# hpgmg/hpgmg

Measured on AMD Instinct MI355X. Metric: DOF/s (fine-grid) for FMG F-cycle, higher is better.
Workload: dtype f64

## Files before the change

### hpgmg_amd/csrc/host/operators_hip.c

```c
#include "plugin_internal.h"

void hp_do_restriction(level_type *Lc, int id_c, level_type *Lf, int id_f, int type) {
  TICK(Lf, restriction_total, "restriction");
  communicator_type *S = &Lf->restriction[type], *R = &Lc->restriction[type];
  backend_t *Bc = hp_backend_of(Lc), *Bf = hp_backend_of(Lf);
  HIP_OK(hpgmg_hip_restrict_blocks(&Bc->dev, id_c, &Bf->dev, id_f, hp_mirror(Lf, S->blocks[0], S->num_blocks[0]), S->num_blocks[0], type));
  hp_transport_phase(R, S, (Lf->tag << 4) | 0x5);
  HIP_OK(hpgmg_hip_restrict_blocks(&Bc->dev, id_c, &Bf->dev, id_f, hp_mirror(Lf, S->blocks[1], S->num_blocks[1]), S->num_blocks[1], type));
  HIP_OK(hpgmg_hip_copy_blocks(&Bc->dev, id_c, hp_mirror(Lc, R->blocks[2], R->num_blocks[2]), R->num_blocks[2]));
  TOCK();
}

int hpgmg_restrict_zero_fused(level_type *Lc, int id_c, level_type *Lf, int id_f, int zero_id) {
  communicator_type *S = &Lf->restriction[RESTRICT_CELL], *R = &Lc->restriction[RESTRICT_CELL];
  if (!Lf->active || !Lc->active || Lc->num_my_boxes < 1 || zero_id == id_c) return 0;
  if (S->num_sends || R->num_recvs || S->num_blocks[0] || R->num_blocks[2] || S->num_blocks[1] < 1) return 0;
  TICK(Lf, restriction_total, "restriction + zero_vector");
  backend_t *Bc = hp_backend_of(Lc), *Bf = hp_backend_of(Lf);
  HIP_OK(hpgmg_hip_restrict_cell_and_zero(&Bc->dev, id_c, &Bf->dev, id_f, hp_mirror(Lf, S->blocks[1], S->num_blocks[1]), S->num_blocks[1], zero_id));
  TOCK();
  return 1;
}

static const int *restrict_map_of(level_type *Lf, backend_t *Bf);
const int *hp_restrict_map_of(level_type *Lf, backend_t *Bf) { return restrict_map_of(Lf, Bf); }
static const int *restrict_map_of(level_type *Lf, backend_t *Bf) {
  communicator_type *S = &Lf->restriction[RESTRICT_CELL];
  if (!Bf->d_restrict_map) {
    int *map = (int *)malloc((size_t)Lf->num_my_boxes * 4 * sizeof(int)), n, b;
    for (b = 0; b < 4 * Lf->num_my_boxes; b++) map[b] = -1;
    for (n = 0; n < S->num_blocks[1]; n++) {
      const blockCopy_type *e = &S->blocks[1][n];
      if (e->read.box < 0 || e->write.box < 0 || map[4 * e->read.box] >= 0) continue;
      map[4 * e->read.box] = e->write.box;
      map[4 * e->read.box + 1] = e->write.i - e->read.i / 2; map[4 * e->read.box + 2] = e->write.j - e->read.j / 2; map[4 * e->read.box + 3] = e->write.k - e->read.k / 2;
    }
    for (b = 0; b < Lf->num_my_boxes; b++) if (map[4 * b] < 0) { free(map); return NULL; }
    Bf->d_restrict_map = (int *)hpgmg_hip_malloc((size_t)Lf->num_my_boxes * 4 * sizeof(int));
    if (!Bf->d_restrict_map) { fprintf(stderr, "hpgmg: device allocation failed: %s\n", hpgmg_hip_last_error()); abort(); }
    HIP_OK(hpgmg_hip_memcpy_h2d(Bf->d_restrict_map, map, (size_t)Lf->num_my_boxes * 4 * sizeof(int)));
    free(map);
  }
  return Bf->d_restrict_map;
}
static long long fused_residuals_remote = 0;
long long hpgmg_fused_residuals_remote(void) { return fused_residuals_remote; }
static int fused_residual_on(void) {
  return (int)hp_switch(SW_FUSED_RESIDUAL);
}
#define FUSED_LAUNCH(READY, CALL) do {                                                                          \
    if ((READY) == 2) {                                                                                          \
      hpgmg_hip_set_tile_part(1); HIP_OK(CALL); hp_overlap_end(); hpgmg_hip_set_tile_part(2); HIP_OK(CALL); hpgmg_hip_set_tile_part(0); \
    } else HIP_OK(CALL); } while (0)
static int fused_residual_operand_form(level_type *L, backend_t *B, int x_id, int restrict_form);
static int fused_residual_operand(level_type *L, backend_t *B, int x_id) { return fused_residual_operand_form(L, B, x_id, 0); }
static int fused_residual_operand_form(level_type *L, backend_t *B, int x_id, int restrict_form) {
// ... 72 lines not shown
  const int many = (T && T->size > 1);
  if (!fused_residual_on() || !hp_switch(SW_DEFER_NORM) || !L->active || !Lc->active || F_id == R_id) return 0;
  if (many) {
    const int nb = L->boxes_in.i * L->boxes_in.j * L->boxes_in.k;
    int q;
    if (Lc->boxes_in.i != L->boxes_in.i || Lc->boxes_in.j != L->boxes_in.j || Lc->boxes_in.k != L->boxes_in.k) return 0;
    for (q = 0; q < nb; q++) if (L->rank_of_box[q] != Lc->rank_of_box[q]) return 0;
  }
  int local_ok = (L->num_my_boxes >= 1 && Lc->num_my_boxes >= 1 && !S->num_sends && !R->num_recvs && !S->num_blocks[0] && !R->num_blocks[2] && S->num_blocks[1] >= 1);
  backend_t *Bc = Lc->num_my_boxes >= 1 ? hp_backend_of(Lc) : NULL, *B = L->num_my_boxes >= 1 ? hp_backend_of(L) : NULL;
  if (local_ok && ((L->box_dim & 1) || !(B->dev.flags & 1) || (L->box_jStride & 1) || (L->box_kStride & 1) || (L->box_volume & 1) || L->box_dim < 16 || !restrict_map_of(L, B))) local_ok = 0;
  if (!local_ok && !many) return 0;
  if (local_ok) {
    TICK(L, blas1, "norm(F) + R = F + restriction (fused, norm deferred)");
    HIP_OK(hpgmg_hip_norm_copy_restrict_deferred(&B->dev, F_id, R_id, &Bc->dev, R_id, B->d_restrict_map));
    TOCK();
    deferred_on_device = 1;
  } else {
    double v = 0.0;
    if (B) { TICK(L, blas1, "norm(F), this rank's part (reduction deferred)"); HIP_OK(hpgmg_hip_norm_max(&B->dev, F_id, &v)); TOCK(); }
    hp_do_scale_vector(L, R_id, 1.0, F_id);
    hp_do_restriction(Lc, R_id, L, R_id, RESTRICT_CELL);
    deferred_host_value = v; deferred_on_device = 0;
  }
  deferred_norm_level = L;
  return 1;
}
double hpgmg_norm_deferred_fetch(level_type *L) {
  double v = deferred_host_value;
  if (deferred_norm_level != L) { fprintf(stderr, "hpgmg: no deferred norm is pending on this level\n"); abort(); }
  deferred_norm_level = NULL;
  if (deferred_on_device) HIP_OK(hpgmg_hip_deferred_fetch(&v));
  return hp_allreduce_scalar(L, v, HPGMG_REDUCE_MAX);
}
int hpgmg_residual_norm_fused(level_type *L, int res_id, int x_id, int rhs_id, double a, double b, double *norm_out) {
  hpgmg_config cfg;
  hpgmg_get_config(&cfg);
  if (cfg.op != HPGMG_OP_7PT && res_id >= 0) return 0;
  if (!L->active || L->num_my_boxes < 1) return 0;
  backend_t *B = hp_backend_of(L);
  const int ready = fused_residual_operand(L, B, x_id);
  if (!ready) return 0;
  double v = 0.0;
  { TICK(L, residual, "residual + norm (fused)");
    FUSED_LAUNCH(ready, hpgmg_hip_residual_norm(hp_stencil_dev(B), hp_variant(), res_id, x_id, rhs_id, a, b, 1.0 / (L->h * L->h), &v));
    TOCK(); }
  *norm_out = hp_allreduce_scalar(L, v, HPGMG_REDUCE_MAX);
  return 1;
}


static void interpolation_lists(level_type *Lf, int id_f, double prescale, level_type *Lc, int id_c, int order, int tagbits) {
  TICK(Lf, interpolation_total, "interpolation");
  communicator_type *S = &Lc->interpolation, *R = &Lf->interpolation;
  backend_t *Bc = hp_backend_of(Lc), *Bf = hp_backend_of(Lf);
  HIP_OK(hpgmg_hip_interpolate_blocks(&Bf->dev, id_f, 0.0, &Bc->dev, id_c, hp_mirror(Lc, S->blocks[0], S->num_blocks[0]), S->num_blocks[0], order));
  hp_transport_phase(R, S, (Lf->tag << 4) | tagbits);
  HIP_OK(hpgmg_hip_interpolate_blocks(&Bf->dev, id_f, prescale, &Bc->dev, id_c, hp_mirror(Lc, S->blocks[1], S->num_blocks[1]), S->num_blocks[1], order));
  HIP_OK(hpgmg_hip_increment_blocks(&Bf->dev, id_f, prescale, hp_mirror(Lf, R->blocks[2], R->num_blocks[2]), R->num_blocks[2]));
  TOCK();
}
void hp_do_interpolation_vcycle(level_type *Lf, int id_f, double prescale, level_type *Lc, int id_c) {
  hpgmg_config c; hpgmg_get_config(&c);
  if (c.op == HPGMG_OP_27PT) {
    if (!hp_exchange_and_bcs_one_launch(Lc, id_c, STENCIL_SHAPE_BOX, 12, 1)) { exchange_boundary(Lc, id_c, STENCIL_SHAPE_BOX); apply_BCs_p2(Lc, id_c, STENCIL_SHAPE_BOX); }
    interpolation_lists(Lf, id_f, prescale, Lc, id_c, 2, 0x7);
    return;
  }
  if (c.op == HPGMG_OP_FV2 || c.op == HPGMG_OP_FV4) {
    if (!hp_exchange_and_bcs_one_launch(Lc, id_c, STENCIL_SHAPE_BOX, 2, 1)) { exchange_boundary(Lc, id_c, STENCIL_SHAPE_BOX); apply_BCs_v2(Lc, id_c, STENCIL_SHAPE_BOX); }
    interpolation_lists(Lf, id_f, prescale, Lc, id_c, 3, 0x7);
    return;
  }
  if (c.op != HPGMG_OP_7PT) hp_no_kernel("interpolation_vcycle for this operator");
  interpolation_lists(Lf, id_f, prescale, Lc, id_c, 0, 0x6);
}
static int interp_all_local(level_type *Lf, level_type *Lc) {
  communicator_type *S = &Lc->interpolation, *R = &Lf->interpolation;
  int n;
  if (Lc->num_my_boxes < 1 || S->num_sends || R->num_recvs || S->num_blocks[0] || R->num_blocks[2] || S->num_blocks[1] < 1) return 0;
  for (n = 0; n < S->num_blocks[1]; n++) if (S->blocks[1][n].read.box < 0 || S->blocks[1][n].write.box < 0) return 0;
  return 1;
}
static long long zero_interp_fused = 0;
long long hpgmg_zero_interp_fused(void) { return zero_interp_fused; }
int hpgmg_zero_interpolation_fcycle_fused(level_type *Lf, int id_f, level_type *Lc, int id_c) {
  hpgmg_config c; hpgmg_get_config(&c);
  if (!hp_switch(SW_FUSED_RESIDUAL) || !hp_ghost_free_mode() || !Lf->active || !Lc->active || Lf->num_my_boxes < 1) return 0;
  if (!interp_all_local(Lf, Lc) || !hp_backend_of(Lf)->all_faces_local) return 0;
  zero_interp_fused++;
  if (c.op == HPGMG_OP_7PT) {
    if (!hp_exchange_and_bcs_one_launch(Lc, id_c, STENCIL_SHAPE_BOX, 1, 1)) { exchange_boundary(Lc, id_c, STENCIL_SHAPE_BOX); apply_BCs_p1(Lc, id_c, STENCIL_SHAPE_BOX); }
    interpolation_lists(Lf, id_f, 0.0, Lc, id_c, 17, 0x7);
  } else if (c.op == HPGMG_OP_27PT) {
    if (!hp_exchange_and_bcs_one_launch(Lc, id_c, STENCIL_SHAPE_BOX, 12, 1)) { exchange_boundary(Lc, id_c, STENCIL_SHAPE_BOX); apply_BCs_p2(Lc, id_c, STENCIL_SHAPE_BOX); }
    interpolation_lists(Lf, id_f, 0.0, Lc, id_c, 18, 0x7);
  } else if (c.op == HPGMG_OP_FV2) {
    if (!hp_exchange_and_bcs_one_launch(Lc, id_c, STENCIL_SHAPE_BOX, 2, 1)) { exchange_boundary(Lc, id_c, STENCIL_SHAPE_BOX); apply_BCs_v2(Lc, id_c, STENCIL_SHAPE_BOX); }
    interpolation_lists(Lf, id_f, 0.0, Lc, id_c, 19, 0x7);
  } else {
    if (!hp_exchange_and_bcs_one_launch(Lc, id_c, STENCIL_SHAPE_BOX, 4, 1)) { exchange_boundary(Lc, id_c, STENCIL_SHAPE_BOX); apply_BCs_v4(Lc, id_c, STENCIL_SHAPE_BOX); }
    interpolation_lists(Lf, id_f, 0.0, Lc, id_c, 20, 0x7);
  }
  return 1;
}
void interpolation_fcycle(level_type *Lf, int id_f, double prescale, level_type *Lc, int id_c) {
  hpgmg_config c; hpgmg_get_config(&c);
  if (c.op == HPGMG_OP_27PT || c.op == HPGMG_OP_FV2) { hp_do_interpolation_vcycle(Lf, id_f, prescale, Lc, id_c); return; }
  if (c.op == HPGMG_OP_FV4) {
    if (!hp_exchange_and_bcs_one_launch(Lc, id_c, STENCIL_SHAPE_BOX, 4, 1)) { exchange_boundary(Lc, id_c, STENCIL_SHAPE_BOX); apply_BCs_v4(Lc, id_c, STENCIL_SHAPE_BOX); }
    interpolation_lists(Lf, id_f, prescale, Lc, id_c, 4, 0x7);
    return;
  }
  if (c.op != HPGMG_OP_7PT) hp_no_kernel("interpolation_fcycle for this operator");
  if (!hp_exchange_and_bcs_one_launch(Lc, id_c, STENCIL_SHAPE_BOX, 1, 1)) { exchange_boundary(Lc, id_c, STENCIL_SHAPE_BOX); apply_BCs_p1(Lc, id_c, STENCIL_SHAPE_BOX); }
  interpolation_lists(Lf, id_f, prescale, Lc, id_c, 1, 0x7);
}

void hp_do_zero_vector(level_type *L, int id) { BLAS1(hpgmg_hip_fill(&hp_backend_of(L)->dev, id, 0.0)); }
void init_vector(level_type *L, int id, double s) { BLAS1(hpgmg_hip_fill(&hp_backend_of(L)->dev, id, s)); }
void hp_do_add_vectors(level_type *L, int c, double sa, int a, double sb, int b) { BLAS1(hpgmg_hip_axpby(&hp_backend_of(L)->dev, c, sa, a, sb, b)); }
void hp_do_mul_vectors(level_type *L, int c, double s, int a, int b) { BLAS1(hpgmg_hip_mul(&hp_backend_of(L)->dev, c, s, a, b)); }
void invert_vector(level_type *L, int c, double s, int a) { BLAS1(hpgmg_hip_invert(&hp_backend_of(L)->dev, c, s, a)); }
void hp_do_scale_vector(level_type *L, int c, double s, int a) { BLAS1(hpgmg_hip_scale(&hp_backend_of(L)->dev, c, s, a)); }
void shift_vector(level_type *L, int c, int a, double shift) { BLAS1(hpgmg_hip_shift(&hp_backend_of(L)->dev, c, a, shift)); }
void color_vector(level_type *L, int id, int colors, int ic, int jc, int kc) { BLAS1(hpgmg_hip_color(&hp_backend_of(L)->dev, id, colors, ic, jc, kc)); }
void random_vector(level_type *L, int id) { BLAS1(hpgmg_hip_random(&hp_backend_of(L)->dev, id)); }

static int attempt_open = 0, attempt_failed = 0;
static long long brick_failures = 0;
long long hpgmg_brick_failures(void) { return brick_failures; }
static const char *brick_failure_text = "hpgmg: an exchange inside a brick launch gave up after 2 s -- not all its workgroups were running (other processes' launches of this kind on "
                                        "the same GPU?).  Results since then are void.";
void hpgmg_solve_attempt_begin(void) {
  const hpgmg_transport *T = hpgmg_get_transport();
  attempt_open = !(T && T->size > 1);
  attempt_failed = 0;
}
static void brick_failure_noted(void) {
  attempt_failed = 1;
  brick_failures++;
  hp_switch_set(SW_BRICK_VISITS, 0);
  if (hpgmg_hip_brick_visit_error_clear()) { fprintf(stderr, "hpgmg: %s\n", hpgmg_hip_last_error()); abort(); }
}
int hpgmg_solve_attempt_end(void) {
  hp_lazy_flush();
  if (attempt_open && !attempt_failed && hpgmg_hip_brick_visit_error()) { if (hpgmg_hip_sync()) abort(); brick_failure_noted(); }
  attempt_open = 0;
  if (attempt_failed) {
    fprintf(stderr, "%s  Brick launches are off from here on (HPGMG_BRICK_VISITS=0); the solve is repeated launch by launch.\n", brick_failure_text);
    attempt_failed = 0;
    return 1;
  }
  return 0;
}
double hp_allreduce_scalar(level_type *L, double v, int op) { hp_allreduce_values(L, &v, 1, op); return v; }
void hp_allreduce_values(level_type *L, double *v, int n, int op) {
  const hpgmg_transport *T = hpgmg_get_transport();
  if (hpgmg_hip_brick_visit_error()) {
    if (!attempt_open) { fprintf(stderr, "%s  HPGMG_BRICK_VISITS=0 runs these levels launch by launch.\n", brick_failure_text); abort(); }
    if (!attempt_failed) brick_failure_noted();
  }
  if (T && T->size > 1) {
    hpgmg_level_ext *X = hpgmg_level_ext_get(L);
    if (X->num_active_ranks > 1) { const double t0 = hp_now(); T->allreduce(T->ctx, v, n, op, X->active_ranks, X->num_active_ranks); L->timers.collectives += hp_now() - t0; }
  }
}
double hp_do_dot(level_type *L, int a, int b) { double v; BLAS1(hpgmg_hip_dot(&hp_backend_of(L)->dev, a, b, &v)); return hp_allreduce_scalar(L, v, HPGMG_REDUCE_SUM); }
double hp_do_norm(level_type *L, int a) {
  double v; BLAS1(hpgmg_hip_norm_max(&hp_backend_of(L)->dev, a, &v)); return hp_allreduce_scalar(L, v, HPGMG_REDUCE_MAX); }
double mean(level_type *L, int a) {
  double v; BLAS1(hpgmg_hip_sum(&hp_backend_of(L)->dev, a, &v));
  v = hp_allreduce_scalar(L, v, HPGMG_REDUCE_SUM);
  return v / (double)((double)L->dim.i * (double)L->dim.j * (double)L->dim.k);
}
double error(level_type *L, int a, int b) { add_vectors(L, VECTOR_TEMP, 1.0, a, -1.0, b); return norm(L, VECTOR_TEMP); }
```

### hpgmg_amd/csrc/host/plugin_dense.c

```c
#include "plugin_internal.h"
#include "hpgmg_boundary_math.h"

static double *dense_stage(backend_t *B, size_t n) {
  if (B->dense_stage_len < n) {
    if (B->dense_stage) hpgmg_hip_free(B->dense_stage);
    B->dense_stage = (double *)hpgmg_hip_malloc(n * sizeof(double));
    B->dense_stage_len = B->dense_stage ? n : 0;
    if (!B->dense_stage) { fprintf(stderr, "hpgmg: dense arrays: no device memory for a %zu-double staging buffer\n", n); abort(); }
  }
  return B->dense_stage;
}
static const double *dense_source(level_type *L, int id, const double *src, int where, size_t len) {
  if (L->num_ranks != 1 || id < 0 || id >= L->numVectors || !src) return NULL;
  if (where == HPGMG_WHERE_PLUGIN) return src;
  if (where != HPGMG_WHERE_HOST) return NULL;
  double *stage = dense_stage(hp_backend_of(L), len);
  HIP_OK(hpgmg_hip_memcpy_h2d(stage, src, len * sizeof(double)));
  return stage;
}
static void dense_extents(const level_type *L, int layout, size_t n[3]) {
  const int high = L->boundary_condition.type == BC_DIRICHLET;
  n[0] = (size_t)dense_extent(L->dim.i, high && layout == HPGMG_DENSE_FACE_I);
  n[1] = (size_t)dense_extent(L->dim.j, high && layout == HPGMG_DENSE_FACE_J);
  n[2] = (size_t)dense_extent(L->dim.k, high && layout == HPGMG_DENSE_FACE_K);
}

int hpgmg_dense_pack(level_type *L, int id, const double *src, int where, int layout, int check) {
  size_t n[3];
  int status = 0;
  if (layout < HPGMG_DENSE_CELL || layout > HPGMG_DENSE_FACE_K) return -1;
  dense_extents(L, layout, n);
  if (!(src = dense_source(L, id, src, where, n[0] * n[1] * n[2]))) return -1;
  HIP_OK(hpgmg_hip_dense_pack(&hp_backend_of(L)->dev, id, src, (int)n[0], (int)n[1], (int)n[2], check, &status));
  return status;
}

int hpgmg_dense_unpack(level_type *L, int id, double *dst, int where) {
  if (L->num_ranks != 1 || id < 0 || id >= L->numVectors || !dst) return -1;
  if (where != HPGMG_WHERE_HOST && where != HPGMG_WHERE_PLUGIN) return -1;
  backend_t *B = hp_backend_of(L);
  const size_t n = (size_t)L->dim.i * L->dim.j * L->dim.k;
  if (where == HPGMG_WHERE_PLUGIN) { HIP_OK(hpgmg_hip_dense_unpack(&B->dev, id, dst)); return 0; }
  double *stage = dense_stage(B, n);
  HIP_OK(hpgmg_hip_dense_unpack(&B->dev, id, stage));
  HIP_OK(hpgmg_hip_memcpy_d2h(dst, stage, n * sizeof(double)));
  return 0;
}

int hpgmg_dense_unpack_flux(level_type *L, int x_id, const double *g, double b, int mask, const double *wall, const double *kappa,
                            double *flux_i, double *flux_j, double *flux_k, int where) {
  int status = 0;
  if (L->num_ranks != 1 || x_id < 0 || x_id >= L->numVectors || !flux_i || !flux_j || !flux_k) return -1;
  if (where != HPGMG_WHERE_HOST && where != HPGMG_WHERE_PLUGIN) return -1;
  if (mask < 0 || mask > 63 || (mask && !wall) || L->dim.i != L->dim.j || L->dim.i != L->dim.k || L->box_ghosts < 1) return -1;
  if (L->boundary_condition.type != BC_DIRICHLET && (g || mask)) return -1;
  backend_t *B = hp_backend_of(L);
  const double wq = bnd_weight_neumann(b, L->h);
  if (where == HPGMG_WHERE_PLUGIN) {
    HIP_OK(hpgmg_hip_dense_unpack_flux(&B->dev, x_id, g, b, wq, L->h, mask, wall, mask ? kappa : NULL, flux_i, flux_j, flux_k, &status));
    return status;
  }
  size_t n[3];
  dense_extents(L, HPGMG_DENSE_FACE_I, n);
  const size_t len = n[0] * n[1] * n[2];
  double *stage = dense_stage(B, 3 * len);
  HIP_OK(hpgmg_hip_dense_unpack_flux(&B->dev, x_id, g, b, wq, L->h, mask, wall, mask ? kappa : NULL, stage, stage + len, stage + 2 * len, &status));
  HIP_OK(hpgmg_hip_memcpy_d2h(flux_i, stage, len * sizeof(double)));
  HIP_OK(hpgmg_hip_memcpy_d2h(flux_j, stage + len, len * sizeof(double)));
  HIP_OK(hpgmg_hip_memcpy_d2h(flux_k, stage + 2 * len, len * sizeof(double)));
  return status;
}

int hpgmg_dense_pack_walls(level_type *L, int id, const double *src, int where, int layout, int check, int mask, double *wall) {
  size_t n[3];
  int status = 0;
  if (layout < HPGMG_DENSE_FACE_I || layout > HPGMG_DENSE_FACE_K || !wall) return -1;
  if (mask < 0 || mask > 63 || L->boundary_condition.type != BC_DIRICHLET || L->dim.i != L->dim.j || L->dim.i != L->dim.k) return -1;
  dense_extents(L, layout, n);
  if (!(src = dense_source(L, id, src, where, n[0] * n[1] * n[2]))) return -1;
  HIP_OK(hpgmg_hip_dense_pack_walls(&hp_backend_of(L)->dev, id, src, layout - HPGMG_DENSE_FACE_I, check, mask, wall, &status));
  return status;
}

int hpgmg_dense_pack_lifted_robin(level_type *L, int id, const double *f, int where, const double *g, double b, int mask, const double *wall, const double *kappa) {
  int status = 0;
  if (!g || L->boundary_condition.type != BC_DIRICHLET || mask < 0 || mask > 63 || (mask && !wall)) return -1;
  if (!(f = dense_source(L, id, f, where, (size_t)L->dim.i * L->dim.j * L->dim.k))) return -1;
  HIP_OK(hpgmg_hip_dense_pack_lifted_robin(&hp_backend_of(L)->dev, id, f, g, bnd_weight(b, L->h), mask, wall, bnd_weight_neumann(b, L->h),
                                           mask ? kappa : NULL, L->h, &status));
  return status;
}
int hpgmg_dense_pack_lifted_faces(level_type *L, int id, const double *f, int where, const double *g, double b, int mask, const double *wall) {
  return hpgmg_dense_pack_lifted_robin(L, id, f, where, g, b, mask, wall, NULL);
}
int hpgmg_dense_pack_lifted(level_type *L, int id, const double *f, int where, const double *g, double b) {
  return hpgmg_dense_pack_lifted_faces(L, id, f, where, g, b, 0, NULL);
}

int hpgmg_boundary_flux_robin(level_type *L, double *phi, const double *g, double b, int mask, const double *wall, const double *kappa) {
  int status = 0;
  if (mask < 0 || mask > 63 || (mask && !wall)) return -1;
  HIP_OK(hpgmg_hip_boundary_flux_robin(&hp_backend_of(L)->dev, phi, g, bnd_weight(b, L->h), mask, wall, bnd_weight_neumann(b, L->h), mask ? kappa : NULL, L->h,
                                       &status));
  return status;
}
int hpgmg_boundary_flux_faces(level_type *L, double *phi, const double *g, double b, int mask, const double *wall) {
  return hpgmg_boundary_flux_robin(L, phi, g, b, mask, wall, NULL);
}
int hpgmg_boundary_flux(level_type *L, double *phi, const double *g, double b) { return hpgmg_boundary_flux_faces(L, phi, g, b, 0, NULL); }

void hpgmg_boundary_restrict(level_type *Lc, double *g_c, level_type *Lf, const double *g_f) {
  (void)Lf;
  HIP_OK(hpgmg_hip_boundary_restrict(g_c, g_f, Lc->dim.i));
}

void hpgmg_boundary_lift(level_type *L, int id, const double *phi, const double *phi_fine, double sign) {
  HIP_OK(hpgmg_hip_boundary_lift(&hp_backend_of(L)->dev, id, phi, phi_fine, sign));
}

void hpgmg_boundary_interp(level_type *Lf, int id, level_type *Lc, const double *g_c) {
  HIP_OK(hpgmg_hip_boundary_interp(&hp_backend_of(Lf)->dev, id, g_c, Lc->dim.i));
}

void hpgmg_boundary_interp_robin(level_type *Lf, int id, level_type *Lc, const double *g_c, int mask, const double *kappa_c) {
  int nb = Lc->dim.i / Lc->box_dim, bx;
  if (Lc->num_my_boxes != nb * nb * nb) nb = 0;
  for (bx = 0; nb && bx < Lc->num_my_boxes; bx++) {
    const box_type *X = &Lc->my_boxes[bx];
    if (X->low.i != (bx % nb) * Lc->box_dim || X->low.j != ((bx / nb) % nb) * Lc->box_dim || X->low.k != (bx / (nb * nb)) * Lc->box_dim) nb = 0;
  }
  HIP_OK(hpgmg_hip_boundary_interp_robin(&hp_backend_of(Lf)->dev, id, &hp_backend_of(Lc)->dev, nb, g_c, Lc->h, mask, mask ? kappa_c : NULL));
}
void hpgmg_boundary_interp_faces(level_type *Lf, int id, level_type *Lc, const double *g_c, int mask) {
  hpgmg_boundary_interp_robin(Lf, id, Lc, g_c, mask, NULL);
}

int hpgmg_boundary_check_kappa(level_type *L, const double *kappa, int where, int robin_mask, int *any_positive) {
  int status = 0;
  if (any_positive) *any_positive = 0;
  if (robin_mask < 0 || robin_mask > 63 || L->dim.i != L->dim.j || L->dim.i != L->dim.k) return -1;
  if (!(kappa = dense_source(L, 0, kappa, where, (size_t)6 * L->dim.i * L->dim.i))) return -1;
  HIP_OK(hpgmg_hip_boundary_check_kappa(kappa, L->dim.i, robin_mask, &status));
  if (any_positive) *any_positive = (status & BND_KAPPA_POSITIVE) != 0;
  return status & (HPGMG_DENSE_NOT_FINITE | HPGMG_DENSE_OUT_OF_RANGE);
}
void hpgmg_boundary_store_walls(level_type *L, const double *wall, const double *kappa, int mask) {
  if (!mask || !wall) return;
  HIP_OK(hpgmg_hip_boundary_store_walls(&hp_backend_of(L)->dev, wall, kappa, L->h, mask));
}
```

### hpgmg_amd/csrc/host/plugin_ghosts.c

```c
#include "plugin_internal.h"

void hp_transport_phase(const communicator_type *recv_side, const communicator_type *send_side, int tag) {
  const hpgmg_transport *T = hpgmg_get_transport();
  int nr = recv_side ? recv_side->num_recvs : 0, ns = send_side ? send_side->num_sends : 0;
  if (nr + ns == 0) return;
  if (!T) { fprintf(stderr, "hpgmg: level needs %d messages but no transport is set\n", nr + ns); abort(); }
  T->sendrecv(T->ctx, nr, nr ? recv_side->recv_buffers : NULL, nr ? recv_side->recv_sizes : NULL, nr ? recv_side->recv_ranks : NULL,
              ns, ns ? send_side->send_buffers : NULL, ns ? send_side->send_sizes : NULL, ns ? send_side->send_ranks : NULL, tag);
}

void exchange_boundary(level_type *L, int id, int shape) {
  TICK(L, ghostZone_total, "exchange_boundary");
  if (shape >= STENCIL_MAX_SHAPES) shape = STENCIL_SHAPE_BOX;
  communicator_type *C = &L->exchange_ghosts[shape];
  backend_t *B = hp_backend_of(L);
  HIP_OK(hpgmg_hip_copy_blocks(&B->dev, id, hp_mirror(L, C->blocks[0], C->num_blocks[0]), C->num_blocks[0]));
  hp_transport_phase(C, C, (L->tag << 4) | shape);
  HIP_OK(hpgmg_hip_copy_blocks(&B->dev, id, hp_mirror(L, C->blocks[1], C->num_blocks[1]), C->num_blocks[1]));
  HIP_OK(hpgmg_hip_copy_blocks(&B->dev, id, hp_mirror(L, C->blocks[2], C->num_blocks[2]), C->num_blocks[2]));
  TOCK();
}

int hp_ghost_free_mode(void) { return (int)hp_switch(SW_GHOST_FREE); }
void hpgmg_set_ghost_free(int on) { hp_switch_set(SW_GHOST_FREE, on ? 1 : 0); hpgmg_hip_set_ghost_free(on ? 1 : 0); }
int hp_exchange_and_bcs_one_launch(level_type *L, int id, int shape, int order, int with_copies) {
  if (!hp_switch(SW_ONE_LAUNCH_GHOSTS) || !hp_ghost_free_mode() || L->num_my_boxes < 1 || L->boundary_condition.type == BC_PERIODIC) return 0;
  if (order == 1 && L->box_ghosts != 1) return 0;
  if (order == 12 && !(L->box_dim >= 2 && L->box_ghosts == 1)) return 0;
  if (order == 2 && !(L->box_dim >= 2)) return 0;
  if (order == 4 && !(L->box_dim >= 4)) return 0;
  communicator_type *C = &L->exchange_ghosts[shape];
  if (C->num_sends + C->num_recvs > 0 || C->num_blocks[0] || C->num_blocks[2]) return 0;
  backend_t *B = hp_backend_of(L);
  int n = 0;
  const hpgmg_hip_bc_entry *e = hp_bc_entries(L, shape, &n);
  if (!B->bc_sources_local[shape]) return 0;
  TICK(L, ghostZone_total, "exchange_boundary + apply_BCs (one launch)");
  HIP_OK(hpgmg_hip_exchange_and_bc(&B->dev, id, with_copies ? hp_mirror(L, C->blocks[1], C->num_blocks[1]) : NULL, with_copies ? C->num_blocks[1] : 0, e, n, order));
  TOCK();
  return 1;
}
int hp_ghosts_for_stencil(level_type *L, int id, int out_id) {
  const int shape = stencil_get_shape();
  hpgmg_config c;
  hpgmg_get_config(&c);
  const int fuse = hp_ghost_free_mode() && c.op == HPGMG_OP_7PT && shape == STENCIL_SHAPE_STAR;
  hpgmg_hip_set_ghost_free(fuse);
  hpgmg_hip_set_tile_ghost_free(0);
  if (fuse) {
    communicator_type *C = &L->exchange_ghosts[shape];
    if (C->num_sends + C->num_recvs > 0) {
      TICK(L, ghostZone_total, "exchange_boundary (remote faces)");
      backend_t *B = hp_backend_of(L);
      HIP_OK(hpgmg_hip_copy_blocks(&B->dev, id, hp_mirror(L, C->blocks[0], C->num_blocks[0]), C->num_blocks[0]));
      hp_transport_phase(C, C, (L->tag << 4) | shape);
      HIP_OK(hpgmg_hip_copy_blocks(&B->dev, id, hp_mirror(L, C->blocks[2], C->num_blocks[2]), C->num_blocks[2]));
      TOCK();
    }
    return 0;
  }
  if (hp_ghost_free_mode() && (c.op == HPGMG_OP_27PT || c.op == HPGMG_OP_FV4) && L->num_my_boxes > 0) {
    backend_t *B = hp_backend_of(L);
    if (B->all_faces_local && hpgmg_hip_tile_kernel_applies(&B->dev, hp_variant(), id != out_id)) {
      hpgmg_hip_set_tile_ghost_free(1);
      if (!hp_exchange_and_bcs_one_launch(L, id, shape, c.op == HPGMG_OP_27PT ? 12 : 4, 0)) apply_BCs(L, id, shape);
// ... 6 lines not shown
  }
  {
    int order = 0;
    if (c.op == HPGMG_OP_27PT) order = 12; else if (c.op == HPGMG_OP_FV2) order = 2; else if (c.op == HPGMG_OP_FV4) order = 4;
    if (order && hp_exchange_and_bcs_one_launch(L, id, shape, order, 1)) return 0;
  }
  exchange_boundary(L, id, shape);
  apply_BCs(L, id, shape);
  return 0;
}

void *hp_comm_stream = NULL, *hp_ev_packed = NULL, *hp_ev_landed = NULL;
long long hp_overlap_count = 0;
long long hpgmg_overlap_count(void) { return hp_overlap_count; }
void hpgmg_set_overlap(int on) { hp_switch_set(SW_OVERLAP, on ? 1 : 0); }
int hp_overlap_enabled(void) { return (int)hp_switch(SW_OVERLAP); }
void hp_overlap_counted(void) { hp_overlap_count++; }
int hp_overlap_begin(level_type *L, int id) {
  const int shape = stencil_get_shape();
  const hpgmg_transport *T = hpgmg_get_transport();
  hpgmg_config c;
  if (!hp_overlap_enabled() || !T || T->size < 2) return 0;
  hpgmg_get_config(&c);
  if (!(hp_ghost_free_mode() && c.op == HPGMG_OP_7PT && shape == STENCIL_SHAPE_STAR) || L->box_dim < 8) return 0;
  communicator_type *C = &L->exchange_ghosts[shape];
  if (C->num_sends + C->num_recvs == 0 || L->num_my_boxes < 1) return 0;
  if (!hp_comm_stream) {
    hp_comm_stream = hpgmg_hip_stream_create(); hp_ev_packed = hpgmg_hip_event_create(); hp_ev_landed = hpgmg_hip_event_create();
    if (!hp_comm_stream || !hp_ev_packed || !hp_ev_landed) { fprintf(stderr, "hpgmg: cannot create the exchange stream\n"); abort(); }
  }
  const double t0 = (hpgmg_get_timer_mode() == TIMERS_DEVICE) ? 0.0 : hp_now();
  backend_t *B = hp_backend_of(L);
  void *launch_stream = hpgmg_hip_get_stream();
  hpgmg_hip_set_ghost_free(1);
  HIP_OK(hpgmg_hip_copy_blocks(&B->dev, id, hp_mirror(L, C->blocks[0], C->num_blocks[0]), C->num_blocks[0]));
  const blockCopy_type *unpack = hp_mirror(L, C->blocks[2], C->num_blocks[2]);
  HIP_OK(hpgmg_hip_event_record(hp_ev_packed));
  hpgmg_hip_set_stream(hp_comm_stream);
  HIP_OK(hpgmg_hip_stream_wait_event(hp_ev_packed));
  hp_transport_phase(C, C, (L->tag << 4) | shape);
  HIP_OK(hpgmg_hip_copy_blocks(&B->dev, id, unpack, C->num_blocks[2]));
  HIP_OK(hpgmg_hip_event_record(hp_ev_landed));
  hpgmg_hip_set_stream(launch_stream);
  if (hpgmg_get_timer_mode() != TIMERS_DEVICE) L->timers.ghostZone_total += hp_now() - t0;
  hp_overlap_count++;
  return 1;
}
void hp_overlap_end(void) { HIP_OK(hpgmg_hip_stream_wait_event(hp_ev_landed)); }

void apply_BCs_p1(level_type *L, int x_id, int shape) {
  if (shape >= STENCIL_MAX_SHAPES) shape = STENCIL_SHAPE_BOX;
  if (L->boundary_condition.type == BC_PERIODIC) return;
  TICK(L, boundary_conditions, "apply_BCs_p1");
  backend_t *B = hp_backend_of(L);
  const int n = L->boundary_condition.num_blocks[shape];
  HIP_OK(hpgmg_hip_apply_bc_p1(&B->dev, x_id, hp_mirror(L, L->boundary_condition.blocks[shape], n), n));
  TOCK();
}
void hp_no_kernel(const char *what) { fprintf(stderr, "hpgmg: %s has no HIP kernel yet\n", what); abort(); }
void apply_BCs_p2(level_type *L, int x_id, int shape) {
  if (shape >= STENCIL_MAX_SHAPES) shape = STENCIL_SHAPE_BOX;
  if (L->boundary_condition.type == BC_PERIODIC) return;
  if (L->box_dim < 2) { apply_BCs_p1(L, x_id, shape); return; }
  TICK(L, boundary_conditions, "apply_BCs_p2");
  backend_t *B = hp_backend_of(L);
  int n = L->boundary_condition.num_blocks[shape];
  if (L->box_ghosts == 1) { const hpgmg_hip_bc_entry *e = hp_bc_entries(L, shape, &n); HIP_OK(hpgmg_hip_apply_bc_fv(&B->dev, x_id, e, n, 12)); }
  else HIP_OK(hpgmg_hip_apply_bc_p2(&B->dev, x_id, hp_mirror(L, L->boundary_condition.blocks[shape], n), n));
  TOCK();
}
void apply_BCs_v1(level_type *L, int x_id, int shape) { apply_BCs_p1(L, x_id, shape); }
int hp_bc_entry_from_block(const level_type *L, int box, const int bpos[3], const int lo[3], const int len[3], int subtype,
                           int (*find)(void *, int), void *ctx, hpgmg_hip_bc_entry *o) {
  const int strides[3] = {1, L->box_jStride, L->box_kStride};
  const int d[3] = {subtype % 3 - 1, (subtype % 9) / 3 - 1, subtype / 9 - 1};
  int ax, nf = 0, local = 1;
  o->box = box; o->nn = 0; o->base = 0; o->len0 = o->len1 = 1; o->fs0 = o->fs1 = 0;
  o->zbase = lo[0] * strides[0] + lo[1] * strides[1] + lo[2] * strides[2]; o->zi = len[0]; o->zj = len[1]; o->zk = len[2];
  int nbr[3] = {0, 0, 0};
  for (ax = 0; ax < 3; ax++) {
    if (d[ax]) { o->base += (d[ax] < 0 ? -1 : L->box_dim) * strides[ax]; o->step[o->nn++] = -d[ax] * strides[ax]; }
    else {
      if (nf == 0) { o->base += lo[ax] * strides[ax]; o->len0 = len[ax]; o->fs0 = strides[ax]; nf++; }
      else if (nf == 1) { o->base += lo[ax] * strides[ax]; o->len1 = len[ax]; o->fs1 = strides[ax]; nf++; }
      if (lo[ax] < 0) nbr[ax] = -1; else if (lo[ax] >= L->box_dim) nbr[ax] = 1;
    }
  }
  o->src_box = o->box; o->src_base = o->base;
  if (nbr[0] || nbr[1] || nbr[2]) {
    const int ni = bpos[0] + nbr[0], nj = bpos[1] + nbr[1], nk = bpos[2] + nbr[2];
    int src = -1;
    if (ni >= 0 && nj >= 0 && nk >= 0 && ni < L->boxes_in.i && nj < L->boxes_in.j && nk < L->boxes_in.k) src = find(ctx, ni + L->boxes_in.i * (nj + L->boxes_in.j * nk));
    if (src >= 0) { o->src_box = src; for (ax = 0; ax < 3; ax++) o->src_base -= nbr[ax] * L->box_dim * strides[ax]; }
    else local = 0;
  }
  return local;
}
static int find_own_box(void *ctx, int gid) {
  const level_type *L = (const level_type *)ctx;
  int q;
  if (L->rank_of_box[gid] != L->my_rank) return -1;
  for (q = 0; q < L->num_my_boxes; q++) if (L->my_boxes[q].global_box_id == gid) return q;
  return -1;
}
static hpgmg_hip_bc_entry *bc_entries_host(level_type *L, int shape, int k_only, int *n_out, int *all_local_out) {
  const int n = L->boundary_condition.num_blocks[shape];
// ... 18 lines not shown
  hpgmg_hip_bc_entry *d = (hpgmg_hip_bc_entry *)hpgmg_hip_malloc((size_t)(n > 0 ? n : 1) * sizeof *h);
  if (!d) { fprintf(stderr, "hpgmg: device allocation failed: %s\n", hpgmg_hip_last_error()); abort(); }
  if (n > 0) HIP_OK(hpgmg_hip_memcpy_h2d(d, h, (size_t)n * sizeof *h));
  free(h);
  return d;
}
const hpgmg_hip_bc_entry *hp_bc_entries(level_type *L, int shape, int *n_out) {
  backend_t *B = hp_backend_of(L);
  const int n = L->boundary_condition.num_blocks[shape];
  *n_out = n;
  if (n <= 0) return NULL;
  if (B->d_bc[shape] && B->n_bc[shape] == n) return B->d_bc[shape];
  if (B->d_bc[shape]) hpgmg_hip_free(B->d_bc[shape]);
  int m = 0, all_local = 1;
  hpgmg_hip_bc_entry *h = bc_entries_host(L, shape, 0, &m, &all_local);
  B->bc_sources_local[shape] = all_local;
  B->d_bc[shape] = bc_entries_upload(h, n);
  B->n_bc[shape] = n;
  return B->d_bc[shape];
}
const hpgmg_hip_bc_entry *hp_bc_entries_k(level_type *L, int *n_out, int *all_local_out) {
  backend_t *B = hp_backend_of(L);
  if (B->n_bc_k < 0) {
    int m = 0;
    hpgmg_hip_bc_entry *h = bc_entries_host(L, stencil_get_shape(), 1, &m, &B->bc_k_local);
    B->d_bc_k = bc_entries_upload(h, m);
    B->n_bc_k = m;
  }
  *n_out = B->n_bc_k; *all_local_out = B->bc_k_local;
  return B->d_bc_k;
}
void apply_BCs_v2(level_type *L, int x_id, int shape) {
  if (shape >= STENCIL_MAX_SHAPES) shape = STENCIL_SHAPE_BOX;
  if (L->boundary_condition.type == BC_PERIODIC) return;
  if (L->box_dim < 2) { apply_BCs_v1(L, x_id, shape); return; }
  TICK(L, boundary_conditions, "apply_BCs_v2");
  int n = L->boundary_condition.num_blocks[shape];
  { const hpgmg_hip_bc_entry *e = hp_bc_entries(L, shape, &n); HIP_OK(hpgmg_hip_apply_bc_fv(&hp_backend_of(L)->dev, x_id, e, n, 2)); }
  TOCK();
}
void apply_BCs_v4(level_type *L, int x_id, int shape) {
  if (shape >= STENCIL_MAX_SHAPES) shape = STENCIL_SHAPE_BOX;
  if (L->boundary_condition.type == BC_PERIODIC) return;
  if (L->box_ghosts < 2) { fprintf(stderr, "called quartic BC's with only 1 ghost zone!!!\n"); abort(); }
  if (L->box_dim < 4) { apply_BCs_v2(L, x_id, shape); return; }
  TICK(L, boundary_conditions, "apply_BCs_v4");
  int n = L->boundary_condition.num_blocks[shape];
  { const hpgmg_hip_bc_entry *e = hp_bc_entries(L, shape, &n); HIP_OK(hpgmg_hip_apply_bc_fv(&hp_backend_of(L)->dev, x_id, e, n, 4)); }
  TOCK();
}
void extrapolate_betas(level_type *L) {
  if (L->boundary_condition.type == BC_PERIODIC) return;
  TICK(L, boundary_conditions, "extrapolate_betas");
  const int n = L->boundary_condition.num_blocks[STENCIL_SHAPE_BOX];
  HIP_OK(hpgmg_hip_extrapolate_betas(&hp_backend_of(L)->dev, hp_mirror(L, L->boundary_condition.blocks[STENCIL_SHAPE_BOX], n), n));
  TOCK();
}
void rebuild_operator_blackbox(level_type *L, double a, double b, int colors) {
  hp_coef32_invalidate(L);
  if (L->dim.i < colors) colors = L->dim.i;
  if (L->dim.j < colors) colors = L->dim.j;
  if (L->dim.k < colors) colors = L->dim.k;
  if (L->my_rank == 0 && hpgmg_verbose) { fprintf(stdout, "  calculating D^{-1} exactly for level h=%e using %3d colors...  ", L->h, colors * colors * colors); fflush(stdout); }
  const int x_id = VECTOR_TEMP, Aii_id = VECTOR_DINV, sum_id = (hpgmg_vectors_reserved() > VECTOR_L1INV) ? VECTOR_L1INV : VECTOR_E;
  const double h2inv = 1.0 / (L->h * L->h);
  int ic, jc, kc;
  hp_do_zero_vector(L, Aii_id);
  hp_do_zero_vector(L, sum_id);
  for (kc = 0; kc < colors; kc++) for (jc = 0; jc < colors; jc++) for (ic = 0; ic < colors; ic++) {
    color_vector(L, x_id, colors, ic, jc, kc);
    exchange_boundary(L, x_id, stencil_get_shape());
    apply_BCs(L, x_id, stencil_get_shape());
    HIP_OK(hpgmg_hip_blackbox_accumulate(&hp_backend_of(L)->dev, hp_variant(), x_id, Aii_id, sum_id, a, b, h2inv));
  }
  double lambda = -1e9;
  HIP_OK(hpgmg_hip_blackbox_finalize(&hp_backend_of(L)->dev, Aii_id, sum_id, a, b, h2inv, &lambda));
  if (L->my_rank == 0 && hpgmg_verbose) fprintf(stdout, "done\n");
  { const hpgmg_transport *T = hpgmg_get_transport();
    if (T && T->size > 1) { int r, *all = (int *)malloc((size_t)T->size * sizeof(int)); for (r = 0; r < T->size; r++) all[r] = r;
      T->allreduce(T->ctx, &lambda, 1, HPGMG_REDUCE_MAX, all, T->size); free(all); } }
  { hpgmg_config cfg; hpgmg_get_config(&cfg);
    if (cfg.smoother == HPGMG_SMOOTH_CHEBY && L->my_rank == 0 && hpgmg_verbose) { fprintf(stdout, "  estimating  lambda_max... <%1.15e\n", lambda); fflush(stdout); } }
  L->dominant_eigenvalue_of_DinvA = lambda;
}
void apply_BCs(level_type *L, int x_id, int shape) {
  hpgmg_config c;
  hpgmg_get_config(&c);
  switch (c.op) {
    case HPGMG_OP_7PT:  apply_BCs_p1(L, x_id, shape); break;
    case HPGMG_OP_27PT: apply_BCs_p2(L, x_id, shape); break;
    case HPGMG_OP_FV2:  apply_BCs_v2(L, x_id, shape); break;
    default:            apply_BCs_v4(L, x_id, shape); break;
  }
}
```

### hpgmg_amd/csrc/host/plugin_internal.h

```cpp
#ifndef HPGMG_PLUGIN_INTERNAL_H
#define HPGMG_PLUGIN_INTERNAL_H
#include <stdio.h>
#include <stdlib.h>
#include <string.h>
#include <math.h>
#include <time.h>
#include <stdint.h>
#include "hpgmg_level.h"
#include "hpgmg_operators.h"
#include "hpgmg_mg.h"
#include "hpgmg_hip.h"

int hpgmg_smooth_sweeps(void);
int hpgmg_gsrb_out_of_place(void);

#define HP_INTERNAL __attribute__((visibility("hidden")))

enum { TIMERS_HOST = 0, TIMERS_DEVICE = 1, TIMERS_SYNC = 2 };
#define TICK(L, FIELD, WHAT) const hpgmg_tick tick_ = hpgmg_tick_begin((L), &(L)->timers.FIELD, WHAT)
#define TOCK() hpgmg_tick_end(tick_)
HP_INTERNAL void hp_lazy_flush(void);
#define HIP_OK(call) do { hp_lazy_flush(); int e_ = (call); if (e_) { fprintf(stderr, "hpgmg: %s failed (%d): %s\n", #call, e_, hpgmg_hip_last_error()); abort(); } } while (0)

#define MAX_LISTS 32
typedef struct {
  hpgmg_hip_level dev;
  double **d_box_base;  int *d_box_low;  int *d_box_nbr;  int all_faces_local;
  double  *seen_v0;     int seen_nv, seen_boxes;
  struct { const blockCopy_type *host; int n; blockCopy_type *dev; } lists[MAX_LISTS];
  int num_lists;
  hpgmg_hip_bc_entry *d_bc[STENCIL_MAX_SHAPES]; int n_bc[STENCIL_MAX_SHAPES];
  int *d_fv4_special; int n_fv4_special;
  hpgmg_hip_bc_entry *d_bc_k; int n_bc_k, bc_k_local;
  int bc_sources_local[STENCIL_MAX_SHAPES];
  int *krylov_pinned;
  double *dense_stage; size_t dense_stage_len;
  double *pair_scratch; double **d_pair_base;
  float *coef32; float **d_coef32_base; int coef32_valid;
  int lexicographic;
  int *d_restrict_map;
  struct pair_halo *halo;
  int halo_state;
  struct halo_images *img;
  int img_state;
  int img_active;
} backend_t;

enum { HALO_FIRST = 0, HALO_NEXT = 1, HALO_COEF = 2, HALO_PLANS = 3 };
typedef struct {
  int n_send, n_recv;
  hpgmg_hip_halo_entry *d_send, *d_recv;
  int n_sp, n_rp;
  int *sp_rank, *rp_rank, *sp_size, *rp_size;
  double **sp_ptr, **rp_ptr;
} halo_plan;
typedef struct pair_halo {
  int brick[3], rem[6];
  halo_plan plan[HALO_PLANS];
  double *sendbuf, *recvbuf, *deep, *deep_beta;
  int coef_valid;
} pair_halo;

enum { IMG_PLAN_COEF = 6, IMG_PLANS = 7 };
typedef struct {
  int n_send, n_recv;
  hpgmg_hip_halo_entry *d_send, *d_recv;
  int n_sp, n_rp;
  int *sp_rank, *rp_rank, *sp_size, *rp_size;
  long long *sp_off, *rp_off;
  int built;
} image_plan;
typedef struct halo_images {
  int n_real, n_img, n_all;
  int *gid;
  int *h_nbr;
  int lo[3], n[3];
  int *brick_lo, *brick_n;
  int depth_max;
  double *storage, *scratch;
  double **d_box_base, **d_pair_base; int *d_box_low, *d_box_nbr;
  hpgmg_hip_level dev, dev_all;
  image_plan plan[IMG_PLANS];
  double *sendbuf, *recvbuf; size_t send_cap, recv_cap;
  double **ptr_tmp; int ptr_cap;
  hpgmg_hip_bc_entry *d_bc; int n_bc, n_bc_own;
  hpgmg_hip_bc_entry *d_bc_k; int n_bc_k;
  int *d_special; int n_special;
  int coef_valid, shape;
  double *seen_v0; int seen_nv;
} halo_images;

typedef enum { SW_GHOST_FREE = 0, SW_ONE_LAUNCH_GHOSTS, SW_OVERLAP, SW_PAIR_REMOTE, SW_IMAGES, SW_FUSED_SWEEPS, SW_PAIR_MIN_CELLS, SW_FUSED_RESIDUAL, SW_FUSED_TAIL,
               SW_FUSED_FTAIL, SW_FUSED_BOTTOM, SW_SMALL_FUSED, SW_SMALL_VTAIL, SW_SMALL_27PT_GSRB, SW_SMALL_OPS, SW_LAZY, SW_LAZY_REPORT, SW_TEMP_SCRATCH,
               SW_FV4_NO_EXACT_RB, SW_GRAPH, SW_SMOOTHER_PRECISION, SW_DEFER_NORM, SW_BRICK_VISITS, SW_BRICK_SIZE, SW_BRICK_MIN_DIM, SW_BRICK_FSTEP, SW_BRICK_CHAIN, SW_BRICK_WIDE, SW_BRICK_WIDE_MAX_DIM, SW_BRICK_WIDE_TAIL_DIM, SW_FTAIL_MAX_DIM, SW_COUNT } hp_switch_id;
HP_INTERNAL long long hp_switch(hp_switch_id id);
HP_INTERNAL void hp_switch_set(hp_switch_id id, long long value);

HP_INTERNAL backend_t *hp_backend_of(level_type *L);
HP_INTERNAL const blockCopy_type *hp_mirror(level_type *owner, const blockCopy_type *host, int n);
HP_INTERNAL int  hp_variant(void);
HP_INTERNAL int  hp_ghost_free_mode(void);
HP_INTERNAL int  hp_box_rank_at(const level_type *L, int bi, int bj, int bk);
HP_INTERNAL void hp_ensure_pair_scratch(level_type *L, backend_t *B);
HP_INTERNAL int  hp_bc_entry_from_block(const level_type *L, int box, const int bpos[3], const int lo[3], const int len[3], int subtype,
                                        int (*find)(void *, int), void *ctx, hpgmg_hip_bc_entry *o);
HP_INTERNAL int  hp_images_ready(level_type *L, backend_t *B);
HP_INTERNAL void hp_images_refresh(level_type *L, backend_t *B, int scr, int id, int depth, int rhs_id, int bc_order);
HP_INTERNAL int  hp_images_refresh_begin(level_type *L, backend_t *B, int scr, int id, int depth, int rhs_id, int bc_order);
HP_INTERNAL void hp_images_refresh_end(void);
HP_INTERNAL int  hp_overlap_enabled(void);
HP_INTERNAL void hp_overlap_counted(void);
HP_INTERNAL void hp_images_bcs(level_type *L, backend_t *B, int scr, int id, int bc_order, int part);
HP_INTERNAL const int *hp_images_fv4_special(level_type *L, backend_t *B, int *n_out);
HP_INTERNAL const hpgmg_hip_bc_entry *hp_images_bc_k(level_type *L, backend_t *B, int *n_out);
HP_INTERNAL void hp_images_release(backend_t *B);
HP_INTERNAL void hp_images_invalidate_coefficients(backend_t *B);
extern HP_INTERNAL long long hp_images_exchanges;
static inline const hpgmg_hip_level *hp_stencil_dev(backend_t *B) { return (B->img && B->img_active) ? &B->img->dev : &B->dev; }


extern HP_INTERNAL void *hp_comm_stream, *hp_ev_packed, *hp_ev_landed;
extern HP_INTERNAL long long hp_overlap_count;
HP_INTERNAL double hp_now(void);
HP_INTERNAL void hp_transport_phase(const communicator_type *recv_side, const communicator_type *send_side, int tag);
HP_INTERNAL int hp_exchange_and_bcs_one_launch(level_type *L, int id, int shape, int order, int with_copies);
HP_INTERNAL int hp_ghosts_for_stencil(level_type *L, int id, int out_id);
HP_INTERNAL int hp_overlap_begin(level_type *L, int id);
HP_INTERNAL void hp_overlap_end(void);
HP_INTERNAL void hp_no_kernel(const char *what);
HP_INTERNAL const hpgmg_hip_bc_entry *hp_bc_entries(level_type *L, int shape, int *n_out);
HP_INTERNAL const hpgmg_hip_bc_entry *hp_bc_entries_k(level_type *L, int *n_out, int *all_local_out);
HP_INTERNAL int hp_vcycle_legs_fused(level_type **levels, int n, int e_id, int R_id, double a, double b, int leg);
HP_INTERNAL void hp_coef32_invalidate(level_type *L);
HP_INTERNAL int hp_interp_smooth_fused(level_type *Lf, int e_id, int R_id, level_type *Lc, double a, double b, int exact_state);
HP_INTERNAL void hp_do_smooth(level_type *L, int x_id, int rhs_id, double a, double b, int temp_dead);
HP_INTERNAL void hp_do_residual(level_type *L, int res_id, int x_id, int rhs_id, double a, double b);
HP_INTERNAL void hp_do_apply_op(level_type *L, int Ax_id, int x_id, double a, double b);
HP_INTERNAL int hp_pair_halo_ready(level_type *L, backend_t *B);
HP_INTERNAL int hp_pair_halo_begin(level_type *L, backend_t *B, int first, int x0_scr, int x0_id, int xm1_scr, int xm1_id, int rhs_id);
HP_INTERNAL void hp_do_restriction(level_type *Lc, int id_c, level_type *Lf, int id_f, int type);
HP_INTERNAL int hp_residual_restrict_zero_fused(level_type *Lc, int id_c, level_type *Lf, int res_id, int x_id, int rhs_id, double a, double b, int zero_id);
HP_INTERNAL int hp_norm_scale_restrict_fused(level_type *L, int F_id, int R_id, level_type *Lc, double *norm_out);
HP_INTERNAL void hp_do_interpolation_vcycle(level_type *Lf, int id_f, double prescale, level_type *Lc, int id_c);
HP_INTERNAL void hp_do_zero_vector(level_type *L, int id);
HP_INTERNAL void hp_do_add_vectors(level_type *L, int c, double sa, int a, double sb, int b);
HP_INTERNAL void hp_do_mul_vectors(level_type *L, int c, double s, int a, int b);
HP_INTERNAL void hp_do_scale_vector(level_type *L, int c, double s, int a);
HP_INTERNAL double hp_allreduce_scalar(level_type *L, double v, int op);
HP_INTERNAL void hp_allreduce_values(level_type *L, double *v, int n, int op);
HP_INTERNAL double hp_do_dot(level_type *L, int a, int b);
HP_INTERNAL double hp_do_norm(level_type *L, int a);
HP_INTERNAL void hp_small_ops_forget(void);
HP_INTERNAL const int *hp_restrict_map_of(level_type *Lf, backend_t *Bf);

#define BLAS1(call) do { TICK(L, blas1, "BLAS1"); HIP_OK(call); TOCK(); } while (0)
#define STENCIL_WITH_GHOSTS(L, id, out_id, TIMER, CALL) do {                                                     \
    hp_backend_of(L)->img_active = 0;                                                                    \
    if (hp_overlap_begin(L, id)) {                                                                          \
      TICK(L, TIMER, #TIMER " (overlapped with the halo exchange)");                                     \
      hpgmg_hip_set_defer_mode(1); HIP_OK(CALL);                                                         \
      hp_overlap_end();                                                                                     \
      hpgmg_hip_set_defer_mode(2); HIP_OK(CALL); hpgmg_hip_set_defer_mode(0);                            \
      TOCK();                                                                                            \
    } else {                                                                                             \
      const int two_parts_ = hp_ghosts_for_stencil(L, id, out_id);    \
      TICK(L, TIMER, #TIMER);                                                                            \
      if (two_parts_) {                                                                                  \
        hpgmg_hip_set_tile_part(1); HIP_OK(CALL);                                                        \
        hp_images_refresh_end();                                                                         \
        hpgmg_hip_set_tile_part(2); HIP_OK(CALL); hpgmg_hip_set_tile_part(0);                            \
      } else HIP_OK(CALL);                                                                               \
      TOCK();                                                                                            \
    } } while (0)
#define PAIR_REMOTE_LAUNCH(OVERLAPPED, DISCARD_X1, CALL) do {                                                   \
    pair_halo *H_ = B->halo;                                                                                   \
    if (OVERLAPPED) {                                                                                          \
      hpgmg_hip_pair_set_halo(H_->brick, H_->rem, H_->deep, H_->deep_beta); hpgmg_hip_set_tile_part(1);        \
      if (DISCARD_X1) hpgmg_hip_pair_discard_x1();                                                             \
      HIP_OK(CALL);                                                                                            \
      hp_overlap_end();                                                                                           \
      hpgmg_hip_pair_set_halo(H_->brick, H_->rem, H_->deep, H_->deep_beta); hpgmg_hip_set_tile_part(2);        \
      if (DISCARD_X1) hpgmg_hip_pair_discard_x1();                                                             \
      HIP_OK(CALL);                                                                                            \
      hpgmg_hip_set_tile_part(0);                                                                              \
    } else {                                                                                                   \
      hpgmg_hip_pair_set_halo(H_->brick, H_->rem, H_->deep, H_->deep_beta);                                    \
// ... 6 lines not shown
```

### hpgmg_amd/csrc/host/plugin_problem.c

```c
#include "plugin_internal.h"

static void eval_beta(double x, double y, double z, double *B, double *Bx, double *By, double *Bz) {
  const double Bmin = 1.0, Bmax = 10.0, c2 = (Bmax - Bmin) / 2, c1 = (Bmax + Bmin) / 2, c3 = 10.0;
  const double xc = 0.50, yc = 0.50, zc = 0.50;
  double r2 = pow((x - xc), 2) + pow((y - yc), 2) + pow((z - zc), 2);
  double r2x = 2.0 * (x - xc), r2y = 2.0 * (y - yc), r2z = 2.0 * (z - zc);
  double r = pow(r2, 0.5);
  double rx = 0.5 * r2x * pow(r2, -0.5), ry = 0.5 * r2y * pow(r2, -0.5), rz = 0.5 * r2z * pow(r2, -0.5);
  *B  = c1 + c2 * tanh(c3 * (r - 0.25));
  *Bx = c2 * c3 * rx * (1 - pow(tanh(c3 * (r - 0.25)), 2));
  *By = c2 * c3 * ry * (1 - pow(tanh(c3 * (r - 0.25)), 2));
  *Bz = c2 * c3 * rz * (1 - pow(tanh(c3 * (r - 0.25)), 2));
}
static void eval_poly(double t, double shift, double *P, double *Pt, double *Ptt) {
  *P   =  2.0 * pow(t, 6) -   6.0 * pow(t, 5) +  5.0 * pow(t, 4) - 1.0 * pow(t, 2) + shift;
  *Pt  = 12.0 * pow(t, 5) -  30.0 * pow(t, 4) + 20.0 * pow(t, 3) - 2.0 * t;
  *Ptt = 60.0 * pow(t, 4) - 120.0 * pow(t, 3) + 60.0 * pow(t, 2) - 2.0;
}
#ifndef M_PI
#define M_PI 3.14159265358979323846
#endif
static double fv_beta(double x, double y, double z, double h, int add_Bxx, int add_Byy, int add_Bzz) {
  const double b = 0.25, a = 2.0 * M_PI;
  double B   = 1.0 + b * sin(a * x) * sin(a * y) * sin(a * z);
// ... 80 lines not shown
    }
    hpgmg_vector_upload(B->vectors[VECTOR_BETA_I], stage + 0 * vol, vol);
    hpgmg_vector_upload(B->vectors[VECTOR_BETA_J], stage + 1 * vol, vol);
    hpgmg_vector_upload(B->vectors[VECTOR_BETA_K], stage + 2 * vol, vol);
    if (cfg.helmholtz) hpgmg_vector_upload(B->vectors[VECTOR_ALPHA], stage + 3 * vol, vol);
    hpgmg_vector_upload(B->vectors[VECTOR_F], stage + 4 * vol, vol);
  }
  free(stage);
}

void rebuild_operator(level_type *L, level_type *from, double a, double b) {
  hp_coef32_invalidate(L);
  hpgmg_config cfg;
  hpgmg_get_config(&cfg);
  if (cfg.op != HPGMG_OP_7PT) {
    if (from) {
      if (cfg.helmholtz) hp_do_restriction(L, VECTOR_ALPHA, from, VECTOR_ALPHA, RESTRICT_CELL);
      hp_do_restriction(L, VECTOR_BETA_I, from, VECTOR_BETA_I, RESTRICT_FACE_I);
      hp_do_restriction(L, VECTOR_BETA_J, from, VECTOR_BETA_J, RESTRICT_FACE_J);
      hp_do_restriction(L, VECTOR_BETA_K, from, VECTOR_BETA_K, RESTRICT_FACE_K);
    }
    if (cfg.op == HPGMG_OP_FV4) extrapolate_betas(L);
    if (cfg.helmholtz) exchange_boundary(L, VECTOR_ALPHA, STENCIL_SHAPE_BOX);
    exchange_boundary(L, VECTOR_BETA_I, STENCIL_SHAPE_BOX);
    exchange_boundary(L, VECTOR_BETA_J, STENCIL_SHAPE_BOX);
    exchange_boundary(L, VECTOR_BETA_K, STENCIL_SHAPE_BOX);
    rebuild_operator_blackbox(L, a, b, cfg.op == HPGMG_OP_FV4 ? 4 : 2);
    exchange_boundary(L, VECTOR_DINV, STENCIL_SHAPE_BOX);
    return;
  }
  if (cfg.op != HPGMG_OP_7PT) hp_no_kernel("rebuild_operator for this operator");
  if (L->my_rank == 0 && hpgmg_verbose) { fprintf(stdout, "  rebuilding operator for level...  h=%e  ", L->h); fflush(stdout); }
  if (from) {
    if (cfg.helmholtz) hp_do_restriction(L, VECTOR_ALPHA, from, VECTOR_ALPHA, RESTRICT_CELL);
    hp_do_restriction(L, VECTOR_BETA_I, from, VECTOR_BETA_I, RESTRICT_FACE_I);
    hp_do_restriction(L, VECTOR_BETA_J, from, VECTOR_BETA_J, RESTRICT_FACE_J);
    hp_do_restriction(L, VECTOR_BETA_K, from, VECTOR_BETA_K, RESTRICT_FACE_K);
  }
  if (cfg.helmholtz) exchange_boundary(L, VECTOR_ALPHA, STENCIL_SHAPE_BOX);
  exchange_boundary(L, VECTOR_BETA_I, STENCIL_SHAPE_BOX);
  exchange_boundary(L, VECTOR_BETA_J, STENCIL_SHAPE_BOX);
  exchange_boundary(L, VECTOR_BETA_K, STENCIL_SHAPE_BOX);

  double lambda = -1e9;
  BLAS1(hpgmg_hip_rebuild_7pt(&hp_backend_of(L)->dev, cfg.variable_coeff, cfg.helmholtz ? VECTOR_ALPHA : -1,
                              cfg.helmholtz ? VECTOR_L1INV : -1, a, b, 1.0 / (L->h * L->h), &lambda));
  { const hpgmg_transport *T = hpgmg_get_transport();
    if (T && T->size > 1) { int r, *all = (int *)malloc((size_t)T->size * sizeof(int)); for (r = 0; r < T->size; r++) all[r] = r;
      T->allreduce(T->ctx, &lambda, 1, HPGMG_REDUCE_MAX, all, T->size); free(all); } }
  if (L->my_rank == 0 && hpgmg_verbose) fprintf(stdout, "eigenvalue_max<%e\n", lambda);
  L->dominant_eigenvalue_of_DinvA = lambda;
  exchange_boundary(L, VECTOR_DINV, STENCIL_SHAPE_BOX);
  if (cfg.helmholtz) exchange_boundary(L, VECTOR_L1INV, STENCIL_SHAPE_BOX);
}
```

### hpgmg_amd/csrc/host/plugin_runtime.c

```c
#include "plugin_internal.h"

static int timer_mode = -1;
void hpgmg_set_timer_mode(int mode) { timer_mode = (mode >= 0 && mode <= 2) ? mode : 0; }
void hpgmg_set_sync_timers(int on) { timer_mode = on ? TIMERS_SYNC : TIMERS_HOST; }
int hpgmg_get_timer_mode(void) {
  if (timer_mode < 0) {
    const char *e = getenv("HPGMG_TIMERS"), *s = getenv("HPGMG_SYNC_TIMERS");
    timer_mode = TIMERS_HOST;
    if (e && !strcmp(e, "device")) timer_mode = TIMERS_DEVICE;
    if ((e && !strcmp(e, "sync")) || (s && s[0] == '1')) timer_mode = TIMERS_SYNC;
  }
  return timer_mode;
}
double hp_now(void) {
  struct timespec ts;
  if (hpgmg_get_timer_mode() == TIMERS_SYNC) hpgmg_hip_sync();
  clock_gettime(CLOCK_MONOTONIC, &ts);
  return (double)ts.tv_sec + 1e-9 * (double)ts.tv_nsec;
}
hpgmg_tick hpgmg_tick_begin(level_type *L, double *acc, const char *what) {
  hpgmg_tick t;
  t.acc = acc; t.slot = -1; t.t0 = 0.0; t.range = 0;
  if (hpgmg_hip_range_enabled()) {
    char label[96];
    snprintf(label, sizeof label, "%d^3 %s", L ? L->dim.i : 0, what);
    hpgmg_hip_range_push(label);
    t.range = 1;
  }
  if (hpgmg_get_timer_mode() == TIMERS_DEVICE) { t.slot = hpgmg_hip_timer_begin(acc); if (t.slot < 0) t.acc = NULL; }
  else t.t0 = hp_now();
  return t;
}
void hpgmg_tick_end(hpgmg_tick t) {
  if (hpgmg_get_timer_mode() == TIMERS_DEVICE) hpgmg_hip_timer_end(t.slot);
  else if (t.acc) *t.acc += hp_now() - t.t0;
  if (t.range) hpgmg_hip_range_pop();
}
void hpgmg_timers_settle(void) { hpgmg_hip_timer_flush(); }

const char *hpgmg_backend_name(void) { return "hip"; }
double *hpgmg_vector_alloc(size_t n) {
  double *p = (double *)hpgmg_hip_malloc(n * sizeof(double));
  if (!p) { fprintf(stderr, "hpgmg: device allocation of %zu doubles failed: %s\n", n, hpgmg_hip_last_error()); abort(); }
  return p;
}
void hpgmg_vector_free(double *p) { hp_lazy_flush(); hpgmg_hip_graph_reset(); hpgmg_hip_free(p); }
void hpgmg_vector_copy(double *d, const double *s, size_t n) { HIP_OK(hpgmg_hip_memcpy_d2d(d, s, n * sizeof(double))); }
void hpgmg_vector_upload(double *d, const double *s, size_t n) { HIP_OK(hpgmg_hip_memcpy_h2d(d, s, n * sizeof(double))); }
void hpgmg_vector_download(double *d, const double *s, size_t n) { HIP_OK(hpgmg_hip_memcpy_d2h(d, s, n * sizeof(double))); }

int hpgmg_transport_init_rccl(const char *id128, int rank, int size) {
  hpgmg_transport t;
  int e = hpgmg_hip_rccl_init(id128, rank, size);
  if (e) return e;
  t.rank = rank; t.size = size; t.ctx = NULL;
  t.sendrecv = hpgmg_hip_rccl_sendrecv;
  t.allreduce = hpgmg_hip_rccl_allreduce;
  t.prepare_subset = hpgmg_hip_rccl_prepare_subset;
  hpgmg_set_transport(&t);
  return 0;
}
void hpgmg_transport_finalize_rccl(void) { hpgmg_set_transport(NULL); hpgmg_hip_rccl_finalize(); }
int hpgmg_transport_init_ipc(const char *name, int rank, int size) {
  hpgmg_transport t;
  int e = hpgmg_hip_ipc_init(name, rank, size);
  if (e) return e;
  t.rank = rank; t.size = size; t.ctx = NULL;
  t.sendrecv = hpgmg_hip_ipc_sendrecv;
  t.allreduce = hpgmg_hip_ipc_allreduce;
  t.prepare_subset = NULL;
  hpgmg_set_transport(&t);
  return 0;
}
void hpgmg_transport_finalize_ipc(void) { hpgmg_set_transport(NULL); hpgmg_hip_ipc_finalize(); }

void hpgmg_set_graphs(int on) { hp_switch_set(SW_GRAPH, on ? 1 : 0); }
void hpgmg_segment_begin(long long key) {
  hp_lazy_flush();
  if (!hp_switch(SW_GRAPH) || hpgmg_get_timer_mode() == TIMERS_SYNC) return;
  { extern int hpgmg_gather_dim; const hpgmg_transport *T = hpgmg_get_transport(); if (T && T->size > 1 && hpgmg_gather_dim < 64) return; }
  if (hpgmg_hip_graph_begin(key) < 0) { fprintf(stderr, "hpgmg: graph segment failed: %s\n", hpgmg_hip_last_error()); abort(); }
}
void hpgmg_segment_end(void) { HIP_OK(hpgmg_hip_graph_end()); }


backend_t *hp_backend_of(level_type *L) {
  hpgmg_level_ext *X = hpgmg_level_ext_get(L);
  backend_t *B = (backend_t *)X->backend;
  if (!B) { B = (backend_t *)calloc(1, sizeof(*B)); X->backend = B; B->lexicographic = -1; B->n_bc_k = -1; B->n_fv4_special = -1; }
  double *v0 = L->num_my_boxes ? L->my_boxes[0].vectors[0] : NULL;
  if (B->seen_v0 != v0 || B->seen_nv != L->numVectors || B->seen_boxes != L->num_my_boxes || !B->d_box_low) {
    int b, n = L->num_my_boxes > 0 ? L->num_my_boxes : 1;
    double **base = (double **)calloc((size_t)n, sizeof(double *));
    int *low = (int *)calloc((size_t)n * 3, sizeof(int));
    for (b = 0; b < L->num_my_boxes; b++) {
      base[b] = L->my_boxes[b].vectors[0];
      low[3 * b] = L->my_boxes[b].low.i; low[3 * b + 1] = L->my_boxes[b].low.j; low[3 * b + 2] = L->my_boxes[b].low.k;
    }
    int *nbr = (int *)calloc((size_t)n * 6, sizeof(int));
    B->all_faces_local = 1;
    for (b = 0; b < L->num_my_boxes; b++) {
// ... 22 lines not shown
    B->d_box_low = (int *)hpgmg_hip_malloc((size_t)n * 3 * sizeof(int));
    B->d_box_nbr = (int *)hpgmg_hip_malloc((size_t)n * 6 * sizeof(int));
    if (!B->d_box_base || !B->d_box_low || !B->d_box_nbr) { fprintf(stderr, "hpgmg: device allocation failed: %s\n", hpgmg_hip_last_error()); abort(); }
    HIP_OK(hpgmg_hip_memcpy_h2d(B->d_box_base, base, (size_t)n * sizeof(double *)));
    HIP_OK(hpgmg_hip_memcpy_h2d(B->d_box_low, low, (size_t)n * 3 * sizeof(int)));
    HIP_OK(hpgmg_hip_memcpy_h2d(B->d_box_nbr, nbr, (size_t)n * 6 * sizeof(int)));
    free(base); free(low); free(nbr);
    B->seen_v0 = v0; B->seen_nv = L->numVectors; B->seen_boxes = L->num_my_boxes;
  }
  B->dev.box_base = (double *const *)B->d_box_base;
  B->dev.box_low = B->d_box_low;
  B->dev.num_boxes = L->num_my_boxes;
  B->dev.dim = L->box_dim;       B->dev.ghosts = L->box_ghosts;
  B->dev.jStride = L->box_jStride; B->dev.kStride = L->box_kStride; B->dev.volume = L->box_volume;
  B->dev.dim_i = L->dim.i; B->dev.dim_j = L->dim.j; B->dev.dim_k = L->dim.k;
  B->dev.periodic = (L->boundary_condition.type == BC_PERIODIC);
  B->dev.box_nbr = B->d_box_nbr;
  {
    int b, ok = (L->box_jStride % 2 == 0) && (L->box_kStride % 2 == 0) && (L->box_volume % 2 == 0);
    const size_t first = (size_t)L->box_ghosts * (size_t)(1 + L->box_jStride + L->box_kStride);
    for (b = 0; ok && b < L->num_my_boxes; b++) if (((uintptr_t)(L->my_boxes[b].vectors[0] + first)) % 16) ok = 0;
    B->dev.flags = ok ? 1 : 0;
    B->dev.box_stride = 0;
    if (L->num_my_boxes > 1) {
      const long long d = (long long)(L->my_boxes[1].vectors[0] - L->my_boxes[0].vectors[0]);
      for (b = 1; b < L->num_my_boxes && (long long)(L->my_boxes[b].vectors[0] - L->my_boxes[b - 1].vectors[0]) == d; b++) ;
      if (b == L->num_my_boxes && d > 0) B->dev.box_stride = d;
    } }
  return B;
}

const blockCopy_type *hp_mirror(level_type *owner, const blockCopy_type *host, int n) {
  int s;
  if (n <= 0 || !host) return NULL;
  backend_t *B = hp_backend_of(owner);
  for (s = 0; s < B->num_lists; s++) if (B->lists[s].host == host && B->lists[s].n == n) return B->lists[s].dev;
  if (B->num_lists == MAX_LISTS) { fprintf(stderr, "hpgmg: too many block lists on one level\n"); abort(); }
  blockCopy_type *d = (blockCopy_type *)hpgmg_hip_malloc((size_t)n * sizeof(blockCopy_type));
  if (!d) { fprintf(stderr, "hpgmg: device allocation failed: %s\n", hpgmg_hip_last_error()); abort(); }
  HIP_OK(hpgmg_hip_memcpy_h2d(d, host, (size_t)n * sizeof(blockCopy_type)));
  B->lists[B->num_lists].host = host; B->lists[B->num_lists].n = n; B->lists[B->num_lists].dev = d;
  B->num_lists++;
  return d;
}

void hpgmg_level_release(level_type *L) {
  hp_lazy_flush();
  hp_small_ops_forget();
  hpgmg_hip_graph_reset();
  hpgmg_hip_timer_forget(&L->timers, &L->timers + 1);
  hpgmg_level_ext *X = hpgmg_level_ext_get(L);
  backend_t *B = (backend_t *)X->backend;
  int s;
  if (!B) return;
  hpgmg_hip_pair_packed_forget(&B->dev);
  hp_images_release(B);
  for (s = 0; s < B->num_lists; s++) hpgmg_hip_free(B->lists[s].dev);
  for (s = 0; s < STENCIL_MAX_SHAPES; s++) if (B->d_bc[s]) hpgmg_hip_free(B->d_bc[s]);
  if (B->d_bc_k) hpgmg_hip_free(B->d_bc_k);
  if (B->d_fv4_special) hpgmg_hip_free(B->d_fv4_special);
  if (B->d_box_base) hpgmg_hip_free(B->d_box_base);
  if (B->d_box_low) hpgmg_hip_free(B->d_box_low);
  if (B->d_box_nbr) hpgmg_hip_free(B->d_box_nbr);
  if (B->krylov_pinned) hpgmg_hip_host_free(B->krylov_pinned);
  if (B->dense_stage) hpgmg_hip_free(B->dense_stage);
  if (B->pair_scratch) hpgmg_hip_free(B->pair_scratch);
  if (B->coef32) hpgmg_hip_free(B->coef32);
  if (B->d_coef32_base) hpgmg_hip_free(B->d_coef32_base);
  if (B->d_pair_base) hpgmg_hip_free(B->d_pair_base);
  if (B->d_restrict_map) hpgmg_hip_free(B->d_restrict_map);
  if (B->halo) {
    int q;
    for (q = 0; q < HALO_PLANS; q++) {
      halo_plan *P = &B->halo->plan[q];
      if (P->d_send) hpgmg_hip_free(P->d_send);
      if (P->d_recv) hpgmg_hip_free(P->d_recv);
      free(P->sp_rank); free(P->rp_rank); free(P->sp_size); free(P->rp_size); free(P->sp_ptr); free(P->rp_ptr);
    }
    if (B->halo->sendbuf) hpgmg_hip_free(B->halo->sendbuf);
    if (B->halo->recvbuf) hpgmg_hip_free(B->halo->recvbuf);
    if (B->halo->deep) hpgmg_hip_free(B->halo->deep);
    if (B->halo->deep_beta) hpgmg_hip_free(B->halo->deep_beta);
    free(B->halo);
  }
  free(B);
  X->backend = NULL;
}

int hp_variant(void) {
  hpgmg_config c;
  hpgmg_get_config(&c);
  if (c.op == HPGMG_OP_7PT || c.op == HPGMG_OP_FV2)
    return !c.variable_coeff ? HPGMG_HIP_7PT_CC : (c.helmholtz ? HPGMG_HIP_7PT_VC_HELMHOLTZ : HPGMG_HIP_7PT_VC_POISSON);
  if (c.op == HPGMG_OP_27PT) return HPGMG_HIP_27PT_CC;
  if (c.op == HPGMG_OP_FV4 && c.variable_coeff) return c.helmholtz ? HPGMG_HIP_FV4_VC_HELMHOLTZ : HPGMG_HIP_FV4_VC_POISSON;
  fprintf(stderr, "hpgmg: operator %d has no HIP kernels yet\n", c.op);
  abort();
}
```

### hpgmg_amd/csrc/host/plugin_smooth.c

```c
#include "plugin_internal.h"

static void cheby_coefficients(const level_type *L, int degree, double *c1, double *c2) {
  double beta = 1.000 * L->dominant_eigenvalue_of_DinvA, alpha = 0.125000 * beta;
  double theta = 0.5 * (beta + alpha), delta = 0.5 * (beta - alpha), sigma = theta / delta, rho_n = 1 / sigma;
  int s;
  c1[0] = 0.0; c2[0] = 1 / theta;
  for (s = 1; s < degree; s++) { double rho_nm1 = rho_n; rho_n = 1.0 / (2.0 * sigma - rho_nm1); c1[s] = rho_n * rho_nm1; c2[s] = rho_n * 2.0 / delta; }
}

void hpgmg_level_sync_counters(level_type *L) {
  hpgmg_hip_timer_flush();
  hpgmg_level_ext *X = hpgmg_level_ext_get(L);
  backend_t *B = (backend_t *)X->backend;
  if (!B || !B->krylov_pinned) return;
  HIP_OK(hpgmg_hip_sync());
  L->Krylov_iterations += *B->krylov_pinned;
  *B->krylov_pinned = 0;
}

int hpgmg_vcycle_legs_fused(level_type **levels, int n, int e_id, int R_id, double a, double b, int leg) { hp_lazy_flush(); return hp_vcycle_legs_fused(levels, n, e_id, R_id, a, b, leg); }
static int bottom_solve_fused_impl(level_type *L, int e_id, int R_id, double a, double b, double want, int ask_only);
static level_type *tail_books_on = NULL;
static int tail_follows_bricks = 0;
static long long small_vtails = 0;
// ... 219 lines not shown
        if (L->numVectors < hpgmg_vectors_reserved() + IterativeSolver_NumVectors()) return 0;
        L->must_subtract_mean = 0;
        if (!B->krylov_pinned) B->krylov_pinned = (int *)hpgmg_hip_host_malloc(64);
        if (!B->krylov_pinned) return 0;
      }
    }
    dev[l] = &B->dev;
    h2inv[l] = 1.0 / (L->h * L->h);
  }
  if (leg == HPGMG_LEG_FCYCLE_TAIL_ASK || probe) return 1;
  TICK(tail_books_on ? tail_books_on : levels[0], smooth, leg == 3 ? "bottom solve (device BiCGStab)" : (leg == 4 ? "fused F-cycle tail" : "fused V-cycle tail"));
  HIP_OK(hpgmg_hip_vcycle_tail(n, dev, h2inv, c1, c2, sweeps, hp_variant(), cfg.smoother, e_id, R_id, a, b, leg,
                               hpgmg_vectors_reserved(), MG_DEFAULT_BOTTOM_NORM, with_bottom ? hp_backend_of(levels[n - 1])->krylov_pinned : NULL));
  TOCK();
  return 1;
}

static int boxes_lexicographic(level_type *L) {
  backend_t *B = hp_backend_of(L);
  if (B->lexicographic < 0) {
    int bx, ok = (L->num_my_boxes == L->boxes_in.i * L->boxes_in.j * L->boxes_in.k);
    for (bx = 0; ok && bx < L->num_my_boxes; bx++) {
      const box_type *X = &L->my_boxes[bx];
      if (X->low.i != (bx % L->boxes_in.i) * L->box_dim || X->low.j != ((bx / L->boxes_in.i) % L->boxes_in.j) * L->box_dim ||
          X->low.k != (bx / (L->boxes_in.i * L->boxes_in.j)) * L->box_dim) ok = 0;
    }
    B->lexicographic = ok;
  }
  return B->lexicographic;
}

void hpgmg_set_smoother_precision(int bits) { hp_switch_set(SW_SMOOTHER_PRECISION, (bits == 32) ? 32 : 64); }
int hpgmg_get_smoother_precision(void) {
  return hp_switch(SW_SMOOTHER_PRECISION) == 32 ? 32 : 64;
}
static const float *const *coef32_of(level_type *L) {
  backend_t *B = hp_backend_of(L);
  if (hpgmg_get_smoother_precision() != 32) return NULL;
  if (!B->coef32) {
    int bx;
    float **base = (float **)calloc((size_t)L->num_my_boxes, sizeof(float *));
    B->coef32 = (float *)hpgmg_hip_malloc(((size_t)L->num_my_boxes * 5 * (size_t)L->box_volume + 4) * sizeof(float));
    B->d_coef32_base = (float **)hpgmg_hip_malloc((size_t)L->num_my_boxes * sizeof(float *));
    if (!B->coef32 || !B->d_coef32_base) { fprintf(stderr, "hpgmg: no memory for the fp32 coefficient copies\n"); abort(); }
    const size_t pad = ((uintptr_t)L->my_boxes[0].vectors[0] % 16) / sizeof(double);
    for (bx = 0; bx < L->num_my_boxes; bx++) base[bx] = B->coef32 + pad + (size_t)bx * 5 * (size_t)L->box_volume;
    HIP_OK(hpgmg_hip_memcpy_h2d(B->d_coef32_base, base, (size_t)L->num_my_boxes * sizeof(float *)));
    free(base);
    B->coef32_valid = 0;
  }
  if (!B->coef32_valid) { HIP_OK(hpgmg_hip_coef32_refresh(&B->dev, (float *const *)B->d_coef32_base, L->numVectors)); B->coef32_valid = 1; }
  return (const float *const *)B->d_coef32_base;
}
void hp_coef32_invalidate(level_type *L) { backend_t *B = hp_backend_of(L); B->coef32_valid = 0; if (B->halo) B->halo->coef_valid = 0; hp_images_invalidate_coefficients(B); hpgmg_hip_pair_packed_invalidate(&B->dev); }

static long long pair_remote_smooths = 0, fp32_pair_smooths = 0;
long long hpgmg_pair_remote_smooths(void) { return pair_remote_smooths; }
long long hpgmg_fp32_pair_smooths(void) { hp_lazy_flush(); return fp32_pair_smooths; }

void hp_ensure_pair_scratch(level_type *L, backend_t *B) {
  if (!B->pair_scratch) {
    int bx;
    double **base = (double **)calloc((size_t)L->num_my_boxes, sizeof(double *));
    B->pair_scratch = (double *)hpgmg_hip_malloc(((size_t)L->num_my_boxes * 2 * (size_t)L->box_volume + 2) * sizeof(double));
    B->d_pair_base = (double **)hpgmg_hip_malloc((size_t)L->num_my_boxes * sizeof(double *));
    if (!B->pair_scratch || !B->d_pair_base) { fprintf(stderr, "hpgmg: no memory for the sweep-pair scratch vectors\n"); abort(); }
    const size_t pad = ((uintptr_t)L->my_boxes[0].vectors[0] % 16) / sizeof(double);
    for (bx = 0; bx < L->num_my_boxes; bx++) base[bx] = B->pair_scratch + pad + (size_t)bx * 2 * (size_t)L->box_volume;
    HIP_OK(hpgmg_hip_memcpy_h2d(B->d_pair_base, base, (size_t)L->num_my_boxes * sizeof(double *)));
    free(base);
  }
}
void hpgmg_set_fused_sweeps(int on) { hp_switch_set(SW_FUSED_SWEEPS, on ? 1 : 0); }
void hpgmg_set_pair_min_cells(long long cells) { hp_switch_set(SW_PAIR_MIN_CELLS, cells > 0 ? cells : 2000000); }
static int pair_kernel_ready(level_type *L, int x_id, int rhs_id, int sweeps) {
  hpgmg_config cfg;
  hpgmg_get_config(&cfg);
  backend_t *B = hp_backend_of(L);
  if (!hp_switch(SW_FUSED_SWEEPS) || sweeps != 4 || cfg.op != HPGMG_OP_7PT || !hp_ghost_free_mode() || stencil_get_shape() != STENCIL_SHAPE_STAR) return 0;
  if (L->boundary_condition.type != BC_DIRICHLET || x_id == VECTOR_TEMP || rhs_id == VECTOR_TEMP) return 0;
  if (B->all_faces_local) { if (!hpgmg_hip_smooth_cheby_pair_supported(&B->dev, hp_variant()) || !boxes_lexicographic(L)) return 0; }
  else if (!hp_pair_halo_ready(L, B)) return 0;
  {
    if ((long long)L->dim.i * L->dim.j * L->dim.k < hp_switch(SW_PAIR_MIN_CELLS)) return 0;
  }
  hp_ensure_pair_scratch(L, B);
  hpgmg_hip_set_ghost_free(1);
  return 1;
}


static long long interp_folded_remote = 0;
long long hpgmg_interp_folded_remote(void) { return interp_folded_remote; }
static int first_pair_folded(const hpgmg_hip_level *fold_Lc, backend_t *B, int v, int x_id, int rhs_id, double a, double b, double h2inv, const double *c1, const double *c2) {
  hpgmg_hip_pair_fold_interpolation(fold_Lc, x_id, 1.0);
  return hpgmg_hip_smooth_cheby_pair(&B->dev, v, (double *const *)B->d_pair_base, NULL, 0, x_id, 0, VECTOR_TEMP, 1, 0, 1, 1, rhs_id, a, b, h2inv, c1[0], c2[0], c1[1], c2[1]);
}
static int smooth_cheby_pairs_fold(level_type *L, int x_id, int rhs_id, double a, double b, const double *c1, const double *c2, int sweeps, int temp_dead, const hpgmg_hip_level *fold_Lc) {
  if (!pair_kernel_ready(L, x_id, rhs_id, sweeps)) return 0;
  backend_t *B = hp_backend_of(L);
  const double h2inv = 1.0 / (L->h * L->h);
  const int v = hp_variant();
  const int remote = !B->all_faces_local;
  const float *const *c32 = remote ? NULL : coef32_of(L);
  int over = 0;
  if (c32) fp32_pair_smooths++;
  if (remote) {
    pair_remote_smooths++;
    if (fold_Lc) { hpgmg_hip_pair_halo_fold_interpolation(fold_Lc, x_id, 1.0); interp_folded_remote++; }
    over = hp_pair_halo_begin(L, B, 1, 0, x_id, 0, VECTOR_TEMP, rhs_id);
  }
  { TICK(L, smooth, "smooth (Chebyshev sweeps 1+2)");
    if (remote && fold_Lc) PAIR_REMOTE_LAUNCH(over, 0, first_pair_folded(fold_Lc, B, v, x_id, rhs_id, a, b, h2inv, c1, c2));
    else if (remote) PAIR_REMOTE_LAUNCH(over, 0, hpgmg_hip_smooth_cheby_pair(&B->dev, v, (double *const *)B->d_pair_base, c32, 0, x_id, 0, VECTOR_TEMP, 1, 0, 1, 1, rhs_id, a, b, h2inv, c1[0], c2[0], c1[1], c2[1]));
    else HIP_OK(hpgmg_hip_smooth_cheby_pair(&B->dev, v, (double *const *)B->d_pair_base, c32, 0, x_id, 0, VECTOR_TEMP, 1, 0, 1, 1, rhs_id, a, b, h2inv, c1[0], c2[0], c1[1], c2[1]));
    TOCK(); }
  if (remote) over = hp_pair_halo_begin(L, B, 0, 1, 1, 1, 0, rhs_id);
  { TICK(L, smooth, "smooth (Chebyshev sweeps 3+4)");
    if (remote) PAIR_REMOTE_LAUNCH(over, temp_dead, hpgmg_hip_smooth_cheby_pair(&B->dev, v, (double *const *)B->d_pair_base, c32, 1, 1, 1, 0, 0, VECTOR_TEMP, 0, x_id, rhs_id, a, b, h2inv, c1[2], c2[2], c1[3], c2[3]));
    else {
      if (temp_dead) hpgmg_hip_pair_discard_x1();
      HIP_OK(hpgmg_hip_smooth_cheby_pair(&B->dev, v, (double *const *)B->d_pair_base, c32, 1, 1, 1, 0, 0, VECTOR_TEMP, 0, x_id, rhs_id, a, b, h2inv, c1[2], c2[2], c1[3], c2[3]));
    }
    TOCK(); }
  return 1;
}
static int smooth_cheby_pairs(level_type *L, int x_id, int rhs_id, double a, double b, const double *c1, const double *c2, int sweeps, int temp_dead) {
  return smooth_cheby_pairs_fold(L, x_id, rhs_id, a, b, c1, c2, sweeps, temp_dead, NULL);
}
static int smooth_gsrb_pairs(level_type *L, int x_id, int rhs_id, double a, double b, int sweeps) {
  if (hpgmg_gsrb_out_of_place() || !pair_kernel_ready(L, x_id, rhs_id, sweeps)) return 0;
  backend_t *B = hp_backend_of(L);
  const double h2inv = 1.0 / (L->h * L->h);
  const int v = hp_variant();
  const int remote = !B->all_faces_local;
  int over = 0;
  if (remote) { pair_remote_smooths++; over = hp_pair_halo_begin(L, B, 1, 0, x_id, 0, x_id, rhs_id); }
  { TICK(L, smooth, "smooth (GSRB half sweeps 1+2)");
    if (remote) PAIR_REMOTE_LAUNCH(over, 0, hpgmg_hip_smooth_gsrb_pair(&B->dev, v, (double *const *)B->d_pair_base, NULL, 0, x_id, 0, 1, 1, rhs_id, a, b, h2inv, 0));
    else HIP_OK(hpgmg_hip_smooth_gsrb_pair(&B->dev, v, (double *const *)B->d_pair_base, NULL, 0, x_id, 0, 1, 1, rhs_id, a, b, h2inv, 0));
    TOCK(); }
  if (remote) over = hp_pair_halo_begin(L, B, 0, 1, 1, 1, 1, rhs_id);
  { TICK(L, smooth, "smooth (GSRB half sweeps 3+4)");
    if (remote) PAIR_REMOTE_LAUNCH(over, 0, hpgmg_hip_smooth_gsrb_pair(&B->dev, v, (double *const *)B->d_pair_base, NULL, 1, 1, 0, 0, x_id, rhs_id, a, b, h2inv, 2));
    else HIP_OK(hpgmg_hip_smooth_gsrb_pair(&B->dev, v, (double *const *)B->d_pair_base, NULL, 1, 1, 0, 0, x_id, rhs_id, a, b, h2inv, 2));
    TOCK(); }
  return 1;
}

int hpgmg_interp_smooth_fused(level_type *Lf, int e_id, int R_id, level_type *Lc, double a, double b) { hp_lazy_flush(); return hp_interp_smooth_fused(Lf, e_id, R_id, Lc, a, b, 0); }
static long long interp_folded_single = 0;
long long hpgmg_interp_folded_single(void) { return interp_folded_single; }
static int interp_smooth_fused_single(level_type *Lf, int e_id, int R_id, level_type *Lc, double a, double b) {
  hpgmg_config cfg;
  hpgmg_get_config(&cfg);
  const int sweeps = hpgmg_smooth_sweeps(), v = hp_variant();
  communicator_type *S = &Lc->interpolation, *Rv = &Lf->interpolation;
  if (!hp_switch(SW_FUSED_RESIDUAL) || cfg.op != HPGMG_OP_7PT || cfg.smoother != HPGMG_SMOOTH_CHEBY || !Lf->active || !Lc->active || sweeps < 2) return 0;
  if (Lf->num_my_boxes < 1 || Lc->num_my_boxes < 1 || !hp_ghost_free_mode() || Lf->boundary_condition.type != BC_DIRICHLET) return 0;
  if (S->num_sends || Rv->num_recvs || S->num_blocks[0] || Rv->num_blocks[2]) return 0;
  if (e_id == VECTOR_TEMP || R_id == VECTOR_TEMP || Lf->dominant_eigenvalue_of_DinvA <= 0.0) return 0;
  backend_t *B = hp_backend_of(Lf), *Bc = hp_backend_of(Lc);
  if (!B->all_faces_local || stencil_get_shape() != STENCIL_SHAPE_STAR) return 0;
  hpgmg_hip_set_ghost_free(1);
  if (!hpgmg_hip_smooth_cheby_fold_supported(&B->dev, v)) return 0;
  const int *map = hp_restrict_map_of(Lf, B);
  if (!map) return 0;
  double c1[16], c2[16];
  const double h2inv = 1.0 / (Lf->h * Lf->h);
  int s;
  cheby_coefficients(Lf, sweeps, c1, c2);
  B->img_active = 0;
  for (s = 0; s < sweeps; s++) {
    const int src = (s & 1) ? VECTOR_TEMP : e_id, dst = (s & 1) ? e_id : VECTOR_TEMP;
    TICK(Lf, smooth, s < 2 ? "smooth (Chebyshev sweep, interpolation folded in)" : "smooth");
    if (s < 2) hpgmg_hip_stencil_fold_interpolation(&Bc->dev, e_id, map, s + 1);
    HIP_OK(hpgmg_hip_smooth_cheby(&B->dev, v, src, dst, R_id, a, b, h2inv, c1[s], c2[s]));
    TOCK();
  }
  interp_folded_single++;
  return 1;
}
int hp_interp_smooth_fused(level_type *Lf, int e_id, int R_id, level_type *Lc, double a, double b, int exact_state) {
  hpgmg_config cfg;
  hpgmg_get_config(&cfg);
  const int sweeps = hpgmg_smooth_sweeps();
  communicator_type *S = &Lc->interpolation, *Rv = &Lf->interpolation;
  if (cfg.op != HPGMG_OP_7PT || !Lf->active || !Lc->active) return 0;
  if (cfg.smoother != HPGMG_SMOOTH_CHEBY && !(cfg.smoother == HPGMG_SMOOTH_GSRB && !hpgmg_gsrb_out_of_place())) return 0;
  if (S->num_sends || Rv->num_recvs || S->num_blocks[0] || Rv->num_blocks[2]) return 0;
  const int remote = !hp_backend_of(Lf)->all_faces_local;
  int parents_in_place = (Lc->num_my_boxes == Lf->num_my_boxes), bx;
  for (bx = 0; parents_in_place && bx < Lf->num_my_boxes; bx++)
    parents_in_place = (2 * Lc->my_boxes[bx].low.i == Lf->my_boxes[bx].low.i && 2 * Lc->my_boxes[bx].low.j == Lf->my_boxes[bx].low.j && 2 * Lc->my_boxes[bx].low.k == Lf->my_boxes[bx].low.k);
  if ((remote && Lf->box_dim % 128 != 0) || Lc->box_dim * 2 != Lf->box_dim || !parents_in_place ||       (!remote && !boxes_lexicographic(Lc)) ||
      (remote && (cfg.smoother != HPGMG_SMOOTH_CHEBY || !hp_switch(SW_PAIR_REMOTE))) ||
      !pair_kernel_ready(Lf, e_id, R_id, sweeps))
    return interp_smooth_fused_single(Lf, e_id, R_id, Lc, a, b);
// ... 256 lines not shown
```

### hpgmg_amd/csrc/host/plugin_switches.c

```c
#include "plugin_internal.h"

enum { K_ON = 0, K_OFF = 1, K_INT = 2, K_TRI = 3 };
static struct { const char *env; int kind; long long dflt; const char *what; long long value; int known; } table[SW_COUNT] = {
  [SW_GHOST_FREE]        = { "HPGMG_GHOST_FREE", K_ON, 1, "stencil launches read neighbouring boxes and the Dirichlet rule themselves; 0: the reference's exchange + boundary + stencil launches" },
  [SW_ONE_LAUNCH_GHOSTS] = { "HPGMG_ONE_LAUNCH_GHOSTS", K_ON, 1, "27-pt / fv2 / fv4: box-to-box ghost copies and boundary conditions as one launch" },
  [SW_OVERLAP]           = { "HPGMG_OVERLAP", K_ON, 1, "N > 1: halo exchanges on a second stream under the part of the stencil launch that does not need them" },
  [SW_PAIR_REMOTE]       = { "HPGMG_PAIR_REMOTE", K_ON, 1, "N > 1, 7-pt: sweep pairs across rank boundaries (two-deep halo, one exchange per pair); 0: one exchange per sweep" },
  [SW_IMAGES]            = { "HPGMG_IMAGES", K_ON, 1, "N > 1, 27-pt / fv4: images of the neighbouring ranks' boxes (one-pass red + black kernels keep running); 0: exchange_boundary per half sweep" },
  [SW_FUSED_SWEEPS]      = { "HPGMG_FUSED_SWEEPS", K_ON, 1, "7-pt: two smoother sweeps per pass on bandwidth-bound levels" },
  [SW_PAIR_MIN_CELLS]    = { "HPGMG_PAIR_MIN_CELLS", K_INT, 2000000, "7-pt: smallest level (cells) that takes the sweep-pair kernel (2 M: the 128^3 level too, since the kernel picks its launch shape per launch -- 16 workgroup rows of 10 waves x 16 chunks = 256 workgroups there: config 2 2.70 vs 2.74 ms; with 16 waves it lost, 3.02 vs 2.92: profiles/r06k_ab_pair_min.txt, r06n_ab_pair_min.txt)" },
  [SW_FUSED_RESIDUAL]    = { "HPGMG_FUSED_RESIDUAL", K_ON, 1, "residual + restriction (+ zero_vector), residual + norm, norm + copy + restriction as one pass each" },
  [SW_FUSED_TAIL]        = { "HPGMG_FUSED_TAIL", K_ON, 1, "7-pt: the V-cycle below the brick levels (<= 8^3; <= 16^3 without them) as one single-workgroup launch" },
  [SW_FUSED_FTAIL]       = { "HPGMG_FUSED_FTAIL", K_ON, 1, "7-pt: the F-cycle's own work below 32^3 as one launch" },
  [SW_FUSED_BOTTOM]      = { "HPGMG_FUSED_BOTTOM", K_ON, 1, "BiCGStab bottom solve on the device; 0: driven from the host (host/solvers.c) through the operators" },
  [SW_SMALL_FUSED]       = { "HPGMG_SMALL_FUSED", K_TRI, 2, "27-pt / fv2 / fv4: smooth() of a one-box level as one launch on an LDS image (2, default); 0 off" },
  [SW_SMALL_VTAIL]       = { "HPGMG_SMALL_VTAIL", K_TRI, 2, "27-pt / fv2 / fv4: the V-cycle below a one-box level as one launch: 2 on except for 27-pt GSRB (default), 1 on, 0 off" },
  [SW_SMALL_27PT_GSRB]   = { "HPGMG_TUNE_SMALL_27PT_GSRB", K_OFF, 0, "27-pt GSRB: the one-launch small-level smooth() instead of the one-workgroup-per-box red + black kernel" },
  [SW_SMALL_OPS]         = { "HPGMG_SMALL_OPS", K_ON, 1, "BLAS-1 / operator calls of a host-driven Krylov solver on a small one-box level go out with the scalar that follows them" },
  [SW_LAZY]              = { "HPGMG_LAZY", K_ON, 1, "void operators are postponed while they follow MGVCycle's call order and issued fused (the reference's own driver, INTEGRATION.md Route B)" },
  [SW_LAZY_REPORT]       = { "HPGMG_LAZY_REPORT", K_OFF, 0, "print what the operator queue did when the process ends" },
  [SW_TEMP_SCRATCH]      = { "HPGMG_TEMP_SCRATCH", K_ON, 1, "inside a cycle VECTOR_TEMP is scratch after smooth(): in-cycle smoother forms; 0: the exact state of smooth() everywhere" },
  [SW_FV4_NO_EXACT_RB]   = { "HPGMG_TUNE_FV4_NO_EXACT_RB", K_OFF, 0, "fv4: the exported smooth() as six half sweeps (no red + black passes)" },
  [SW_GRAPH]             = { "HPGMG_GRAPH", K_OFF, 0, "capture / replay the launch-bound segments as hipGraphs (measured slower with a full stream)" },
  [SW_DEFER_NORM]        = { "HPGMG_DEFER_NORM", K_ON, 1, "FMGSolve: norm(F) of the opening pass is collected at the end, where it is used, instead of waited for at the start" },
  [SW_BRICK_VISITS]     = { "HPGMG_BRICK_VISITS", K_ON, 1, "7-pt: the 64^3 / 32^3 / 16^3 levels of a V-cycle leg as one launch of 8^3 bricks that trade faces, residuals and corrections inside the launch; 0 when other processes run such launches on the same GPU" },
  [SW_BRICK_SIZE]       = { "HPGMG_TUNE_BRICK", K_INT, 8, "side of those bricks: 8 (512 lanes, one cell each) or 16 (1024 lanes, four cells each)" },
  [SW_BRICK_MIN_DIM]    = { "HPGMG_TUNE_BRICK_MIN", K_INT, 16, "smallest level (cells per side) visited as bricks; the levels below it are the single-workgroup tail's" },
  [SW_BRICK_FSTEP]      = { "HPGMG_TUNE_BRICK_FSTEP", K_ON, 1, "FMGSolve: interpolation_fcycle onto a brick level rides in the first launch of the V-cycle that follows it" },
  [SW_BRICK_CHAIN]      = { "HPGMG_TUNE_BRICK_CHAIN", K_INT, 1, "consecutive brick levels of a V-cycle leg in ONE launch (what passes between the levels passes inside it); 0: one launch per level visit" },
  [SW_BRICK_WIDE]       = { "HPGMG_BRICK_WIDE", K_ON, 1, "27-pt / fv4: the same for the operators with wide stencils (kernels/brick_wide.hip: halo of the stencil's radius, apply_BCs_p2 / _v4 on the LDS image)" },
  [SW_BRICK_WIDE_MAX_DIM] = { "HPGMG_TUNE_BRICK_WIDE_MAX", K_INT, 64, "largest level (cells per side) the 27-pt / fv4 plugins visit as bricks (measured: fv4 `7 64` 29.71 / 29.91 / 30.15 ms with 64 / 32 / 16, 27-pt 12.27 / 12.51 / 12.52)" },
  [SW_BRICK_WIDE_TAIL_DIM] = { "HPGMG_TUNE_BRICK_WIDE_TAIL", K_INT, 1, "27-pt / fv4: the largest one-box level left to the single-workgroup tail (1: the 8^3, 4^3 (and 27-pt: 2^3) levels are visited as ONE brick each and only the bottom solve is left; 2 / 4 / 8: the tail starts there)" },
  [SW_FTAIL_MAX_DIM]    = { "HPGMG_TUNE_FTAIL_MAX", K_INT, 8, "7-pt: the largest level (cells per side) the single-launch F-cycle tail starts from (8: the 16^3 step of the climb is a brick launch each way, eight CUs instead of one: config 1 0.320 vs 0.328 ms with 16, config 2 the same within noise; profiles/r06i_ab_ftail.txt)" },
  [SW_SMOOTHER_PRECISION]= { "HPGMG_SMOOTHER_PRECISION", K_INT, 64, "32: fp32 coefficient streams in the Chebyshev sweep pairs (BASELINE config 5: within 2e-4 of the fp64 norms, and bit-exact against the CPU oracle's fp32 mode, which rounds the same coefficients); 64: bit-exact" },
};

long long hp_switch(hp_switch_id id) {
  if (!table[id].known) {
    const char *e = getenv(table[id].env);
    long long v = table[id].dflt;
    switch (table[id].kind) {
      case K_ON:  v = !(e && e[0] == '0'); break;
      case K_OFF: v = (e && e[0] == '1'); break;
      case K_INT: if (e && *e) v = atoll(e); break;
      default:    v = (e && e[0] == '0') ? 0 : ((e && e[0] == '1') ? 1 : table[id].dflt); break;
    }
    table[id].value = v; table[id].known = 1;
  }
  return table[id].value;
}
void hp_switch_set(hp_switch_id id, long long value) { table[id].value = value; table[id].known = 1; }

void hpgmg_print_switches(void) {
  int q;
  for (q = 0; q < SW_COUNT; q++) fprintf(stderr, "  %-28s = %-8lld (default %lld)  %s\n", table[q].env, hp_switch((hp_switch_id)q), table[q].dflt, table[q].what);
}
__attribute__((constructor)) static void switches_report(void) { const char *e = getenv("HPGMG_SWITCHES"); if (e && e[0] == '1') hpgmg_print_switches(); }
```

### hpgmg_amd/csrc/kernels/cheby_pair.hpp

```cpp
#pragma once
#include "common.hpp"
#include "stencil_math.hpp"

namespace hpgmg {

struct VecRef { int scratch, id; };
struct PairArgs {
  VecRef x0, xm1, out1, out2;
  int rhs_id;
  double a, b, h2inv, c1a, c2a, c1b, c2b;
  int sweep_a;
  int keep_x1;
  hpgmg_hip_level Lc; int coarse_id; double prescale;
  double *const *scr_base;
  const float *const *c32_base;
  int nbi, nbj;
  int Di, Dj, Dk;
  int rem[6];
  const double *deep;
  const double *deep_beta;
  int tiles_i, slabs_j, chunks_k, KC, per_xcd, total_blocks;
  int edge_blocks, edge_per_xcd;
  double *edge_coef;
  const int *order;
};

__device__ __forceinline__ double *pair_vec(const hpgmg_hip_level &L, const PairArgs &A, VecRef r, int box) {
  double *base = r.scratch ? A.scr_base[box] : L.box_base[box];
  return base + (size_t)r.id * (size_t)L.volume + (size_t)L.ghosts * (size_t)(1 + L.jStride + L.kStride);
}
struct LaneShift { long long lvl, scr, c32; };
__device__ __forceinline__ long long shift_of(const LaneShift &s, VecRef r) { return r.scratch ? s.scr : s.lvl; }

struct alignas(16) p2 { double x, y; };
typedef double __attribute__((ext_vector_type(2))) d2v;
typedef const d2v __attribute__((address_space(1))) *gd2cptr;
typedef d2v __attribute__((address_space(1))) *gd2ptr;
__device__ __forceinline__ p2 pld(const double *p) { const d2v v = *(gd2cptr)as_global(p); return p2{v.x, v.y}; }
__device__ __forceinline__ void pst(double *p, p2 v) { d2v w; w.x = v.x; w.y = v.y; *(gd2ptr)as_global(p) = w; }
__device__ __forceinline__ double gld1(const double *p) { return *as_global(p); }
__device__ __forceinline__ p2 pneg(p2 v) { return p2{-v.x, -v.y}; }
__device__ __forceinline__ int uni(int v) { return __builtin_amdgcn_readfirstlane(v); }

enum { C32_DINV = 0, C32_ALPHA, C32_BETA_I, C32_BETA_J, C32_BETA_K, C32_COUNT };
template <bool C32> struct CoefStream {
  const double *p64; const float *p32;
  __device__ __forceinline__ CoefStream(const hpgmg_hip_level &L, const PairArgs &A, int box, int vec_id, int slot, const LaneShift &sh = LaneShift{0, 0, 0}) {
    const size_t first = (size_t)L.ghosts * (size_t)(1 + L.jStride + L.kStride);
    if (C32) { p32 = A.c32_base[box] + (size_t)slot * (size_t)L.volume + first + sh.c32; p64 = nullptr; }
    else     { p64 = L.box_base[box] + (size_t)vec_id * (size_t)L.volume + first + sh.lvl; p32 = nullptr; }
  }
  __device__ __forceinline__ p2 pair(int off) const {
    if (C32) { typedef float __attribute__((ext_vector_type(2))) f2v; const f2v f = *(const f2v __attribute__((address_space(1))) *)(p32 + off); return p2{(double)f.x, (double)f.y}; }
    return pld(p64 + off);
  }
  __device__ __forceinline__ double one(int off) const { return C32 ? (double)*(const float __attribute__((address_space(1))) *)(p32 + off) : gld1(p64 + off); }
};

template <int V> struct PlaneCoef { p2 rhs, dinv, al, bi, bjlo, bjhi, bk0, bk1; double bir; };

enum { PAIR_CHEBY = 0, PAIR_GSRB = 1 };
template <int V, int SM>
__device__ __forceinline__ p2 pair_update(p2 c, double left, double right, p2 jm, p2 jp, p2 km, p2 kp, p2 old,
                                          const PlaneCoef<V> &q, double a, double b, double h2inv, double c1, double c2, bool first_is_swept) {
  const double Ax0 = apply_op_7pt<V>(c.x, left, c.y, jm.x, jp.x, km.x, kp.x, q.bi.x, q.bi.y, q.bjlo.x, q.bjhi.x, q.bk0.x, q.bk1.x, q.al.x, a, b, h2inv);
  const double Ax1 = apply_op_7pt<V>(c.y, c.x, right, jm.y, jp.y, km.y, kp.y, q.bi.y, q.bir, q.bjlo.y, q.bjhi.y, q.bk0.y, q.bk1.y, q.al.y, a, b, h2inv);
  p2 o;
  if (SM == PAIR_CHEBY) {
    o.x = c.x + c1 * (c.x - old.x) + c2 * q.dinv.x * (q.rhs.x - Ax0);
    o.y = c.y + c1 * (c.y - old.y) + c2 * q.dinv.y * (q.rhs.y - Ax1);
  } else {
    const double nx = c.x + q.dinv.x * (q.rhs.x - Ax0), ny = c.y + q.dinv.y * (q.rhs.y - Ax1);
    o.x = first_is_swept ? nx : c.x;
    o.y = first_is_swept ? c.y : ny;
  }
  return o;
}

constexpr int kPairMaxBoxes = 1024;
template <int V, int NW, bool C32, int SM, bool NARROW, bool INTERP, bool REMOTE = false>
__global__ __launch_bounds__(64 * NW) void cheby_pair_kernel(const hpgmg_hip_level L_in, const PairArgs A_in) {
  static_assert(!(REMOTE && C32) && !(REMOTE && NARROW && INTERP), "the multi-rank variant is built for fp64 coefficients; with narrow boxes the interpolation is not folded in");
  constexpr bool kVC = (V != HPGMG_HIP_7PT_CC);
  constexpr bool kHelm = (V == HPGMG_HIP_7PT_VC_HELMHOLTZ);
  constexpr int NR = NW - 2;
  extern __shared__ p2 pair_lds[];
  p2 (*slabX0)[NW][64] = reinterpret_cast<p2 (*)[NW][64]>(pair_lds);
  p2 (*slabX1)[NW][64] = reinterpret_cast<p2 (*)[NW][64]>(pair_lds + 2 * NW * 64);
  p2 (*slabBJ)[NW][64] = reinterpret_cast<p2 (*)[NW][64]>(pair_lds + 4 * NW * 64);
  __shared__ double *sTabLvl[kPairMaxBoxes];
  __shared__ double *sTabScr[kPairMaxBoxes];
  __shared__ const float *sTabC32[C32 ? kPairMaxBoxes : 1];
  __shared__ double *sTabCrs[INTERP ? kPairMaxBoxes : 1];
  hpgmg_hip_level L = L_in;
  PairArgs A = A_in;
  {
    const int nt = 64 * NW, tid0 = (int)threadIdx.y * 64 + (int)threadIdx.x;
    for (int bx = tid0; bx < L_in.num_boxes; bx += nt) {
      sTabLvl[bx] = L_in.box_base[bx];
      sTabScr[bx] = A_in.scr_base ? A_in.scr_base[bx] : nullptr;
      if (C32) sTabC32[bx] = A_in.c32_base[bx];
      if (INTERP) sTabCrs[bx] = A_in.Lc.box_base[bx];
    }
    L.box_base = sTabLvl; A.scr_base = sTabScr;
    if (C32) A.c32_base = sTabC32;
    if (INTERP) A.Lc.box_base = sTabCrs;
    __syncthreads();
  }

  int logical = xcd_logical_block((int)blockIdx.x, A.per_xcd);
  if (REMOTE && A.order) logical = A.order[logical];
  if (logical >= A.total_blocks) return;
  int t = logical;
  const int ti = t % A.tiles_i; t /= A.tiles_i;
  const int sj = t % A.slabs_j; t /= A.slabs_j;
  const int ck = t;

  const int lane = (int)threadIdx.x, w = uni((int)threadIdx.y);
  const int bd = L.dim, jS = L.jStride, kS = L.kStride;
  const int gi0 = ti * 128, R = sj * NR, K0 = ck * A.KC;
  const int NRs = (R + NR <= A.Dj) ? NR : A.Dj - R;
  const int KCs = (K0 + A.KC <= A.Dk) ? A.KC : A.Dk - K0;
  const int gj = R - 1 + w;
  const int jlo = (REMOTE && A.rem[2]) ? -1 : 0, jhi = (REMOTE && A.rem[3]) ? A.Dj + 1 : A.Dj;
  const int klo = (REMOTE && A.rem[4]) ? -1 : 0, khi = (REMOTE && A.rem[5]) ? A.Dk + 1 : A.Dk;
  auto x0row = [&](int r) { return r >= ((REMOTE && A.rem[2]) ? -2 : 0) && r < ((REMOTE && A.rem[3]) ? A.Dj + 2 : A.Dj); };
  auto x0plane = [&](int g) { return g >= ((REMOTE && A.rem[4]) ? -2 : 0) && g < ((REMOTE && A.rem[5]) ? A.Dk + 2 : A.Dk); };
  const bool row_x1 = (gj >= jlo && gj < jhi && w <= NRs + 1);
  const bool row_out = (w >= 1 && w <= NRs);
  const int lanes_per_box = NARROW ? bd / 2 : 64, hop = NARROW ? lane / lanes_per_box : 0;
  const int bi_ = gi0 / bd, li = NARROW ? 2 * (lane - hop * lanes_per_box) : gi0 - bi_ * bd + 2 * lane;
  LaneShift sh = {0, 0, 0};
  if (NARROW) { sh.lvl = (long long)hop * L.box_stride; sh.scr = (long long)hop * 2 * L.volume; sh.c32 = (long long)hop * C32_COUNT * L.volume; }
  const int gjc = row_x1 ? gj : 0;
  const int nbj_ = A.Dj / bd, nbk_ = A.Dk / bd;
  auto jbox = [&](int r) { return !REMOTE ? r / bd : (r < 0 ? 0 : (r >= A.Dj ? nbj_ - 1 : r / bd)); };
  auto kbox = [&](int g) { return !REMOTE ? g / bd : (g < 0 ? 0 : (g >= A.Dk ? nbk_ - 1 : g / bd)); };
  const int bj_ = jbox(gjc), lj = gjc - bj_ * bd;
// ... 31 lines not shown
  auto x0_row = [&](int bj, int l_j, int gk) -> p2 {
    if (REMOTE && (gk < -1 || gk > A.Dk)) {
      if (l_j < 0 || l_j >= bd) return p2{0, 0};
      const int box = box_of(bi_, bj, gk) + hop;
      return pld(A.deep + (((size_t)box * 6 + (gk < 0 ? 4 : 5)) * bd + l_j) * bd + li);
    }
    return x0_pair(box_of(bi_, bj, gk), li, l_j, gk);
  };
  auto far_row = [&](int gk) -> p2 {
    if (REMOTE && far_deep) {
      if (gk < 0 || gk >= A.Dk) return p2{0, 0};
      const int box = box_of(bi_, bjf, gk) + hop;
      return pld(A.deep + (((size_t)box * 6 + (gjf < 0 ? 2 : 3)) * bd + (gk - kbox(gk) * bd)) * bd + li);
    }
    return REMOTE ? x0_row(bjf, ljf, gk) : x0_pair(box_of(bi_, bjf, gk), li, ljf, gk);
  };

  const int P0 = K0 - 1, P1 = K0 + KCs;
  auto in_dom = [&](int gk) { return gk >= klo && gk < khi; };

  p2 x0m = {0, 0}, x0c = {0, 0}, x0p = {0, 0};
  p2 x1m2 = {0, 0}, x1m1 = {0, 0}, x1c = {0, 0};
  p2 far_c = {0, 0}, far_n = {0, 0};
  p2 bj_c = {0, 0}, bj_n = {0, 0};
  PlaneCoef<V> qc = {}, qp = {};

  const int pstart = in_dom(P0) ? P0 : P0 + 1;
  if (row_x1) {
    const int box = box_of(bi_, bj_, pstart), off = row_off + plane_off(pstart);
    x0c = REMOTE ? x0_row(bj_, lj, pstart) : x0_pair(box, li, lj, pstart);
    if (kVC) bj_c = CoefStream<C32>(L, A, box, VECTOR_BETA_J, C32_BETA_J, sh).pair(off);
    if (x0plane(pstart - 1)) x0m = REMOTE ? x0_row(bj_, lj, pstart - 1) : x0_pair(box_of(bi_, bj_, pstart - 1), li, lj, pstart - 1);
    if (far_lo || far_hi) far_c = far_row(pstart);
    slabX0[pstart & 1][w][lane] = x0c;
    slabBJ[pstart & 1][w][lane] = bj_c;
  }
  __syncthreads();

#ifdef HPGMG_EXP_TIMELINE
  unsigned long long *tl = (unsigned long long *)A.deep;
  const bool probe = !REMOTE && tl && logical == 0 && w == 1 && lane == 0;
  int tl_n = 0;
#define TL_MARK() do { if (probe && tl_n < 4000) tl[tl_n++] = __builtin_amdgcn_s_memrealtime(); } while (0)
#else
#define TL_MARK() do { } while (0)
#endif
  for (int p = pstart; p <= P1 && p < khi; p++) {
    const int box = box_of(bi_, bj_, p), off = row_off + plane_off(p);
    TL_MARK();
    const bool have_next = in_dom(p + 1) && (p + 1 <= P1);
    const bool above_in = x0plane(p + 1);
    const bool ghost_plane = REMOTE && (p < 0 || p >= A.Dk);
    if (row_x1) {
      if (above_in) {
        const int bn = box_of(bi_, bj_, p + 1), offn = row_off + plane_off(p + 1);
        x0p = REMOTE ? x0_row(bj_, lj, p + 1) : x0_pair(bn, li, lj, p + 1);
        if (have_next) {
          if (kVC) bj_n = CoefStream<C32>(L, A, bn, VECTOR_BETA_J, C32_BETA_J, sh).pair(offn);
          if (far_lo || far_hi) far_n = far_row(p + 1);
        }
      }
      qc.rhs = pld(vec_origin(L, box, A.rhs_id) + sh.lvl + off);
      qc.dinv = CoefStream<C32>(L, A, box, VECTOR_DINV, C32_DINV, sh).pair(off);
      if (kHelm) qc.al = CoefStream<C32>(L, A, box, VECTOR_ALPHA, C32_ALPHA, sh).pair(off);
      if (kVC) {
        const CoefStream<C32> bis(L, A, box, VECTOR_BETA_I, C32_BETA_I, sh), bks(L, A, box, VECTOR_BETA_K, C32_BETA_K, sh);
        qc.bi = bis.pair(off);
        qc.bir = __shfl_down(qc.bi.x, 1, 64);
        if (lane == 63) qc.bir = bis.one(off + 2);
        if (p == pstart || (p % bd) == 0) qc.bk0 = bks.pair(off); else qc.bk0 = qp.bk1;
        if (REMOTE && p >= A.Dk) qc.bk1 = ghost_row ? p2{0, 0} : pld(A.deep_beta + (((size_t)(box + hop) * 3 + 2) * bd + lj) * bd + li);
        else qc.bk1 = bks.pair(off + kS);
        qc.bjlo = bj_c;
        if (REMOTE && gj >= A.Dj) qc.bjhi = ghost_plane ? p2{0, 0} : pld(A.deep_beta + (((size_t)(box + hop) * 3 + 1) * bd + (p - kbox(p) * bd)) * bd + li);
        else if (w == NRs + 1 || gj + 1 >= jhi || ((lj + 1) == bd)) qc.bjhi = CoefStream<C32>(L, A, box, VECTOR_BETA_J, C32_BETA_J, sh).pair(off + jS);
        else qc.bjhi = slabBJ[p & 1][w + 1][lane];
      }
      p2 xm1 = x0c;
      if (SM == PAIR_CHEBY && A.c1a != 0.0) xm1 = pld(pair_vec(L, A, A.xm1, box) + shift_of(sh, A.xm1) + off);
#ifdef HPGMG_EXP_TIMELINE
      if (probe) { asm volatile("s_waitcnt vmcnt(0)" ::: "memory"); }
      TL_MARK();
#endif

      p2 jm, jp;
      if (!x0row(gj - 1)) jm = pneg(x0c); else if (w == 0) jm = far_c; else jm = slabX0[p & 1][w - 1][lane];
      if (!x0row(gj + 1)) jp = pneg(x0c); else if (w == NRs + 1) jp = far_c; else jp = slabX0[p & 1][w + 1][lane];
      const p2 km = x0plane(p - 1) ? x0m : pneg(x0c);
      const p2 kp = above_in ? x0p : pneg(x0c);
      double left = __shfl_up(x0c.y, 1, 64), right = __shfl_down(x0c.x, 1, 64);
      if (lane == 0)  left  = (left_dom && !left_ghost)   ? -x0c.x : x0_one(box_of(biL, bj_, p), liL, lj, p);
      if (lane == 63) right = (right_dom && !right_ghost) ? -x0c.y : x0_one(box_of(biR, bj_, p), liR, lj, p);
      if (!(ghost_row && ghost_plane))
        x1c = pair_update<V, SM>(x0c, left, right, jm, jp, km, kp, xm1, qc, A.a, A.b, A.h2inv, A.c1a, A.c2a, ((gj ^ p ^ A.sweep_a) & 1) == 0);
    }
#ifdef HPGMG_EXP_TIMELINE
    if (probe) { asm volatile("" :: "v"(x1c.x)); }
    TL_MARK();
#endif

    const int q = p - 1;
    if (row_out && q >= K0) {
      const int boxq = box_of(bi_, bj_, q), offq = row_off + plane_off(q);
      p2 jm, jp;
      if (gj - 1 < jlo) jm = pneg(x1m1); else jm = slabX1[q & 1][w - 1][lane];
      if (gj + 1 >= jhi) jp = pneg(x1m1); else jp = slabX1[q & 1][w + 1][lane];
      const p2 km = in_dom(q - 1) ? x1m2 : pneg(x1m1);
      const p2 kp = x1c;
      double left = __shfl_up(x1m1.y, 1, 64), right = __shfl_down(x1m1.x, 1, 64);
      if (lane == 0)  left  = (left_dom && !left_ghost)   ? -x1m1.x : gld1(pair_vec(L, A, A.out1, box_of(biL, bj_, q)) + (liL + lj * jS + plane_off(q)));
      if (lane == 63) right = (right_dom && !right_ghost) ? -x1m1.y : gld1(pair_vec(L, A, A.out1, box_of(biR, bj_, q)) + (liR + lj * jS + plane_off(q)));
      const p2 x2 = pair_update<V, SM>(x1m1, left, right, jm, jp, km, kp, x0m, qp, A.a, A.b, A.h2inv, A.c1b, A.c2b, ((gj ^ q ^ (A.sweep_a + 1)) & 1) == 0);
      pst(pair_vec(L, A, A.out2, boxq) + shift_of(sh, A.out2) + offq, x2);
    }
    if (SM == PAIR_CHEBY && A.keep_x1 && row_out && p >= K0 && p < K0 + KCs) pst(pair_vec(L, A, A.out1, box) + shift_of(sh, A.out1) + off, x1c);

    TL_MARK();
    if (row_x1) {
      slabX1[p & 1][w][lane] = x1c;
      if (have_next) { slabX0[(p + 1) & 1][w][lane] = x0p; slabBJ[(p + 1) & 1][w][lane] = bj_n; }
    }
    __syncthreads();
    TL_MARK();
    x0m = x0c; x0c = x0p; x1m2 = x1m1; x1m1 = x1c; far_c = far_n; bj_c = bj_n; qp = qc;
  }
#ifdef HPGMG_EXP_TIMELINE
  if (probe) tl[4095] = (unsigned long long)tl_n;
#endif
#undef TL_MARK

  if (P1 >= khi && row_out) {
    const int q = A.Dk - 1;
// ... 98 lines not shown
```

### hpgmg_amd/csrc/kernels/pair.hip

```cpp
#include "stencil_direct.hpp"
#include "cheby_pair.hpp"

namespace hpgmg {
struct HaloRefs { VecRef x0, xm1; int rhs_id; double *const *scr_base; int fold; hpgmg_hip_level Lc; int coarse_id; double prescale; };
__device__ __forceinline__ double *halo_vec(const hpgmg_hip_level &L, const HaloRefs &R, int vec, int box) {
  const size_t first = (size_t)L.ghosts * (size_t)(1 + L.jStride + L.kStride);
  if (vec >= 16) return L.box_base[box] + (size_t)(vec - 16) * (size_t)L.volume + first;
  if (vec == 2) return L.box_base[box] + (size_t)R.rhs_id * (size_t)L.volume + first;
  const VecRef r = (vec == 0) ? R.x0 : R.xm1;
  return (r.scratch ? R.scr_base[box] : L.box_base[box]) + (size_t)r.id * (size_t)L.volume + first;
}
template <bool kUnpack>
__global__ __launch_bounds__(256) void pair_halo_kernel(const hpgmg_hip_level L, const HaloRefs R, const hpgmg_hip_halo_entry *__restrict__ list,
                                                        double *buf, double *deep, double *deep_beta) {
  const hpgmg_hip_halo_entry e = list[blockIdx.x];
  const int n = e.ni * e.nj * e.nk, jS = L.jStride, kS = L.kStride;
  double *v = halo_vec(L, R, e.vec, e.box) + e.i + e.j * jS + e.k * kS;
  double *b = buf + e.off;
  double *plane = nullptr;
  if (kUnpack && e.deep >= 8) plane = deep_beta + ((size_t)e.box * 3 + (e.deep - 8)) * (size_t)L.dim * L.dim;
  else if (kUnpack && e.deep >= 0) plane = deep + ((size_t)e.box * 6 + e.deep) * (size_t)L.dim * L.dim;
  for (int t = blockIdx.y * 256 + threadIdx.x; t < n; t += gridDim.y * 256) {
    const int ti = t % e.ni, tj = (t / e.ni) % e.nj, tk = t / (e.ni * e.nj);
    if (!kUnpack) {
      double val = v[ti + tj * jS + tk * kS];
      if (R.fold && e.vec == 0) {
        const int ci = e.i + ti, cj = e.j + tj, ck = e.k + tk;
        val = R.prescale * val + vec_origin(R.Lc, e.box, R.coarse_id)[(ci >> 1) + (cj >> 1) * R.Lc.jStride + (ck >> 1) * R.Lc.kStride];
      }
      b[t] = val;
    }
    else if (plane) plane[t] = b[t];
    else v[ti + tj * jS + tk * kS] = b[t];
  }
}
#ifdef HPGMG_EXP_TIMELINE
double *g_exp_timeline = nullptr;
#endif
}
using namespace hpgmg;

extern "C" {
int hpgmg_hip_graph_flush(void);

static int pair_supported_dims(const hpgmg_hip_level *L, int variant, int Di, int Dj, int Dk) {
  if (variant != HPGMG_HIP_7PT_VC_HELMHOLTZ && variant != HPGMG_HIP_7PT_VC_POISSON && variant != HPGMG_HIP_7PT_CC) return 0;
  if (L->num_boxes <= 0 || L->num_boxes > kPairMaxBoxes || L->periodic || !(L->flags & 1) || L->ghosts < 1 || Di % 128 != 0) return 0;
  if (L->dim % 128 != 0 && !(128 % L->dim == 0 && L->dim >= 16 && (L->box_stride > 0 || L->num_boxes == 1))) return 0;
  if (L->jStride % 2 || L->kStride % 2 || L->volume % 2) return 0;
  if (Di % L->dim || Dj % L->dim || Dk % L->dim) return 0;
  if ((long long)(Di / L->dim) * (Dj / L->dim) * (Dk / L->dim) != L->num_boxes) return 0;
  return 1;
}
int hpgmg_hip_smooth_cheby_pair_supported(const hpgmg_hip_level *L, int variant) { return pair_supported_dims(L, variant, L->dim_i, L->dim_j, L->dim_k); }
int hpgmg_hip_smooth_cheby_pair_supported_brick(const hpgmg_hip_level *L, int variant, int nbi, int nbj, int nbk) {
  return pair_supported_dims(L, variant, nbi * L->dim, nbj * L->dim, nbk * L->dim);
}
int hpgmg_hip_coef32_refresh(const hpgmg_hip_level *L, float *const *c32_base, int num_vectors) {
  HPGMG_SKIP_IF_REPLAY();
  if (L->num_boxes <= 0) return 0;
  hipLaunchKernelGGL(coef32_convert_kernel, dim3(512, L->num_boxes), dim3(256), 0, g_stream, *L, c32_base, num_vectors);
  HPGMG_LAUNCH_CHECK("coef32_convert_kernel");
  return 0;
}
static bool g_pair_halo_set = false;
static int g_pair_rem[6], g_pair_brick[3];
static const double *g_pair_deep = nullptr, *g_pair_deep_beta = nullptr;
static long long g_pair_launches = 0, g_pair_remote_launches = 0;
static int g_pair_discard_x1 = 0;
static const hpgmg_hip_level *g_pair_interp_level = nullptr;
static int g_pair_interp_id = 0;
static double g_pair_interp_prescale = 1.0;
struct EdgePack { const void *key; int variant, Di, Dj, Dk; double *buf; bool valid; };
static std::vector<EdgePack> g_edge_packs;
extern "C" void hpgmg_hip_pair_packed_invalidate(const hpgmg_hip_level *L) { for (EdgePack &e : g_edge_packs) if (!L || e.key == (const void *)L->box_base) e.valid = false; }
extern "C" void hpgmg_hip_pair_packed_forget(const hpgmg_hip_level *L) {
  for (size_t q = 0; q < g_edge_packs.size();) {
    if (!L || g_edge_packs[q].key == (const void *)L->box_base) { (void)hipStreamSynchronize(g_stream); (void)hipFree(g_edge_packs[q].buf); g_edge_packs.erase(g_edge_packs.begin() + (long)q); }
    else q++;
  }
}
static EdgePack *edge_pack_slot(const hpgmg_hip_level *L, int variant, const PairArgs &A) {
  static const int on = env_int("HPGMG_TUNE_PAIR_PACKED", 1);
  if (!on || A.tiles_i < 2 || variant == HPGMG_HIP_7PT_CC) return nullptr;
  for (EdgePack &e : g_edge_packs) if (e.key == (const void *)L->box_base && e.variant == variant && e.Di == A.Di && e.Dj == A.Dj && e.Dk == A.Dk) return &e;
  EdgePack e = { (const void *)L->box_base, variant, A.Di, A.Dj, A.Dk, nullptr, false };
  const size_t n = (size_t)2 * (A.tiles_i - 1) * A.Dk * A.Dj * 8;
  if (hipMalloc((void **)&e.buf, n * sizeof(double)) != hipSuccess) return nullptr;
  g_edge_packs.push_back(e);
  return &g_edge_packs.back();
}
struct PairOrder { int ti, sj, ck, rem[6], part; int *d_order; int grid, per_xcd, count; };
static std::vector<PairOrder> g_pair_orders;
static const PairOrder *pair_part_order(const PairArgs &A, int part) {
  for (const PairOrder &o : g_pair_orders)
    if (o.ti == A.tiles_i && o.sj == A.slabs_j && o.ck == A.chunks_k && o.part == part && memcmp(o.rem, A.rem, sizeof o.rem) == 0) return &o;
  PairOrder o = {}; o.ti = A.tiles_i; o.sj = A.slabs_j; o.ck = A.chunks_k; o.part = part; memcpy(o.rem, A.rem, sizeof o.rem);
  std::vector<int> sel;
  for (int l = 0; l < A.total_blocks; l++) {
    int t = l;
    const int ti = t % A.tiles_i; t /= A.tiles_i;
    const int sj = t % A.slabs_j; t /= A.slabs_j;
    const int ck = t;
    const bool later = (ti == 0 && A.rem[0]) || (ti == A.tiles_i - 1 && A.rem[1]) || (sj == 0 && A.rem[2]) || (sj == A.slabs_j - 1 && A.rem[3]) || (ck == 0 && A.rem[4]) || (ck == A.chunks_k - 1 && A.rem[5]);
    if (later == (part == 2)) sel.push_back(l);
  }
  o.count = (int)sel.size();
  if (o.count > 0) {
    o.per_xcd = (o.count + kXcds - 1) / kXcds; o.grid = o.per_xcd * kXcds;
    sel.resize((size_t)o.grid, A.total_blocks);
    if (hipMalloc((void **)&o.d_order, sel.size() * sizeof(int)) != hipSuccess) return nullptr;
    if (hipMemcpy(o.d_order, sel.data(), sel.size() * sizeof(int), hipMemcpyHostToDevice) != hipSuccess) { (void)hipFree(o.d_order); return nullptr; }
  }
  g_pair_orders.push_back(o);
  return &g_pair_orders.back();
}
static int smooth_pair(const hpgmg_hip_level *L, int variant, int gsrb, int sweep_a, double *const *scr_base, const float *const *c32_base,
                       int x0_scr, int x0_id, int xm1_scr, int xm1_id, int out1_scr, int out1_id, int out2_scr, int out2_id,
                       int rhs_id, double a, double b, double h2inv, double c1a, double c2a, double c1b, double c2b) {
  const bool remote = g_pair_halo_set;
  const int discard_x1 = g_pair_discard_x1;
  const hpgmg_hip_level *const interp_level = g_pair_interp_level;
  g_pair_halo_set = false; g_pair_discard_x1 = 0; g_pair_interp_level = nullptr;
  HPGMG_SKIP_IF_REPLAY();
  const int Di = remote ? g_pair_brick[0] * L->dim : L->dim_i, Dj = remote ? g_pair_brick[1] * L->dim : L->dim_j, Dk = remote ? g_pair_brick[2] * L->dim : L->dim_k;
  if (!pair_supported_dims(L, variant, Di, Dj, Dk)) return record_error(hipErrorInvalidValue, "smooth_cheby_pair: level not supported");
  if (remote && c32_base) return record_error(hipErrorInvalidValue, "smooth_cheby_pair: remote faces need fp64 coefficients");
  static const int tune_kc = env_int("HPGMG_TUNE_PAIR_KC", 0);
  static const int tune_nw = env_int("HPGMG_TUNE_PAIR_NW", 0);
  int nw = 16, kc = tune_kc;
  {
    const int slots = 256, cand[3] = {10, 12, 16}, step_cost[3] = {46, 51, 75};
    long long best_cost = -1;
    for (int ci = 0; ci < 3; ci++) {
      const int w = cand[ci];
      if (tune_nw > 0 && w != tune_nw) continue;
      if (tune_nw <= 0 && c32_base && w == 10) continue;
      const int per_plane = (Di / 128) * ((Dj + (w - 2) - 1) / (w - 2));
      auto steps = [&](int c) { const long long wgs = (long long)per_plane * ((Dk + c - 1) / c); return ((wgs + slots - 1) / slots) * (c + 2); };
      int k = tune_kc;
      if (k <= 0) {
        long long best = -1;
        for (int c = 8; c <= 64 && c <= Dk; c++) { const long long cost = steps(c); if (best < 0 || cost < best) { best = cost; k = c; } }
        for (int c = k + 1; c <= 64 && c <= Dk; c++) if (steps(c) * 100 <= best * 103) k = c;
      }
      const long long cost = steps(k) * step_cost[ci];
      if (best_cost < 0 || cost < best_cost) { best_cost = cost; nw = w; kc = k; }
    }
  }
  PairArgs A = {};
  A.x0 = VecRef{x0_scr, x0_id}; A.xm1 = VecRef{xm1_scr, xm1_id}; A.out1 = VecRef{out1_scr, out1_id}; A.out2 = VecRef{out2_scr, out2_id};
  A.rhs_id = rhs_id; A.a = a; A.b = b; A.h2inv = h2inv; A.c1a = c1a; A.c2a = c2a; A.c1b = c1b; A.c2b = c2b;
  A.scr_base = scr_base; A.c32_base = c32_base; A.sweep_a = sweep_a;
  A.keep_x1 = discard_x1 ? 0 : 1;
  const bool interp = (interp_level != nullptr);
  if (interp) {
    const hpgmg_hip_level *C = interp_level;
    if ((remote && L->dim % 128 != 0) || C->num_boxes != L->num_boxes || C->num_boxes > kPairMaxBoxes || 2 * C->dim != L->dim) return record_error(hipErrorInvalidValue, "smooth pair with interpolation: level pair not supported");
    A.Lc = *C; A.coarse_id = g_pair_interp_id; A.prescale = g_pair_interp_prescale;
  }
  A.nbi = Di / L->dim; A.nbj = Dj / L->dim;
  A.Di = Di; A.Dj = Dj; A.Dk = Dk;
  if (remote) { for (int d = 0; d < 6; d++) A.rem[d] = g_pair_rem[d]; A.deep = g_pair_deep; A.deep_beta = g_pair_deep_beta; }
#ifdef HPGMG_EXP_TIMELINE
  else A.deep = g_exp_timeline;
#endif
  A.tiles_i = A.Di / 128; A.slabs_j = (A.Dj + (nw - 2) - 1) / (nw - 2); A.KC = kc; A.chunks_k = (A.Dk + kc - 1) / kc;
  A.total_blocks = A.tiles_i * A.slabs_j * A.chunks_k;
  int grid = grid_for(A.total_blocks, &A.per_xcd);
  long long cells = (long long)A.Di * A.Dj * A.Dk;
  const long long whole_cells = cells;
  const int part = remote ? g_tile_part : 0;
  if (part) {
    const PairOrder *o = pair_part_order(A, part);
    if (!o) return record_error(hipErrorOutOfMemory, "smooth pair: dispatch list of a partial launch");
    if (o->count == 0) return 0;
    A.order = o->d_order; grid = o->grid; A.per_xcd = o->per_xcd;
    cells = cells * o->count / A.total_blocks;
  }
  const size_t lds = (size_t)nw * 6 * 64 * sizeof(p2);
  if (!remote && !c32_base) {
    EdgePack *pk = edge_pack_slot(L, variant, A);
    if (pk) {
      A.edge_coef = pk->buf;
      if (!pk->valid) {
        A.edge_blocks = ((A.Dj + 63) / 64) * A.Dk * 2 * (A.tiles_i - 1);
        const dim3 pgrid(grid_for(A.edge_blocks, &A.edge_per_xcd));
        if (variant == HPGMG_HIP_7PT_VC_HELMHOLTZ) hipLaunchKernelGGL((cheby_pair_edge_kernel<HPGMG_HIP_7PT_VC_HELMHOLTZ, false, PAIR_CHEBY, false, false, true>), pgrid, dim3(64), 0, g_stream, *L, A);
        else hipLaunchKernelGGL((cheby_pair_edge_kernel<HPGMG_HIP_7PT_VC_POISSON, false, PAIR_CHEBY, false, false, true>), pgrid, dim3(64), 0, g_stream, *L, A);
        HPGMG_LAUNCH_CHECK("cheby_pair_edge_kernel (packing)");
        pk->valid = true;
      }
    }
  }
  const int prof = profile_begin(whole_cells);
#define PAIR_NW_SWITCH(...) switch (nw) { case 10: { constexpr int NWC = 10; __VA_ARGS__ } break; case 12: { constexpr int NWC = 12; __VA_ARGS__ } break; default: { constexpr int NWC = 16; __VA_ARGS__ } break; }
#define PAIR_LAUNCH2(VAR, C32, SM, NARROW, INTERP) PAIR_NW_SWITCH( \
      static bool once = false; if (!once) { HPGMG_CHECK(hipFuncSetAttribute((const void *)cheby_pair_kernel<VAR, NWC, C32, SM, NARROW, INTERP>, hipFuncAttributeMaxDynamicSharedMemorySize, (int)((size_t)NWC * 6 * 64 * sizeof(p2)))); once = true; } \
      hipLaunchKernelGGL((cheby_pair_kernel<VAR, NWC, C32, SM, NARROW, INTERP>), dim3(grid), dim3(64, NWC), lds, g_stream, *L, A); )
#define PAIR_LAUNCH_REMOTE_IP(VAR, SM, NRW, IP) { \
      const int ecols = 2 * (A.tiles_i - 1) + (A.rem[0] ? 1 : 0) + (A.rem[1] ? 1 : 0); \
      A.edge_blocks = ((A.Dj + 63) / 64) * A.Dk * ecols; const int egrid_r = grid_for(A.edge_blocks, &A.edge_per_xcd); \
      if (ecols > 0) hipLaunchKernelGGL((cheby_pair_edge_kernel<VAR, false, SM, IP, true>), dim3(egrid_r), dim3(64), 0, g_stream, *L, A); \
      PAIR_NW_SWITCH( \
      static bool once = false; if (!once) { HPGMG_CHECK(hipFuncSetAttribute((const void *)cheby_pair_kernel<VAR, NWC, false, SM, NRW, IP, true>, hipFuncAttributeMaxDynamicSharedMemorySize, (int)((size_t)NWC * 6 * 64 * sizeof(p2)))); once = true; } \
      hipLaunchKernelGGL((cheby_pair_kernel<VAR, NWC, false, SM, NRW, IP, true>), dim3(grid), dim3(64, NWC), lds, g_stream, *L, A); ) }
#define PAIR_LAUNCH_REMOTE(VAR, SM) { if (L->dim % 128 != 0) PAIR_LAUNCH_REMOTE_IP(VAR, SM, true, false) else if (interp) PAIR_LAUNCH_REMOTE_IP(VAR, SM, false, true) else PAIR_LAUNCH_REMOTE_IP(VAR, SM, false, false) }
#define PAIR_LAUNCH(VAR, C32, SM) { \
      A.edge_blocks = ((A.Dj + 63) / 64) * A.Dk * 2 * (A.tiles_i - 1); const dim3 egrid(A.edge_blocks > 0 ? grid_for(A.edge_blocks, &A.edge_per_xcd) : 1); \
      if (remote) PAIR_LAUNCH_REMOTE(VAR, SM) \
      else if (interp) { \
        if (A.tiles_i > 1) hipLaunchKernelGGL((cheby_pair_edge_kernel<VAR, C32, SM, true>), egrid, dim3(64), 0, g_stream, *L, A); \
        if (L->dim % 128 == 0) PAIR_LAUNCH2(VAR, C32, SM, false, true) else PAIR_LAUNCH2(VAR, C32, SM, true, true) \
      } else { \
        if (A.tiles_i > 1) hipLaunchKernelGGL((cheby_pair_edge_kernel<VAR, C32, SM, false>), egrid, dim3(64), 0, g_stream, *L, A); \
        if (L->dim % 128 == 0) PAIR_LAUNCH2(VAR, C32, SM, false, false) else PAIR_LAUNCH2(VAR, C32, SM, true, false) \
      } }
#define PAIR_CASE(VAR) case VAR: \
    if (gsrb) { if (c32_base) PAIR_LAUNCH(VAR, true, PAIR_GSRB) else PAIR_LAUNCH(VAR, false, PAIR_GSRB) } \
    else      { if (c32_base) PAIR_LAUNCH(VAR, true, PAIR_CHEBY) else PAIR_LAUNCH(VAR, false, PAIR_CHEBY) } break;
  switch (variant) {
    PAIR_CASE(HPGMG_HIP_7PT_VC_HELMHOLTZ)
    PAIR_CASE(HPGMG_HIP_7PT_VC_POISSON)
    PAIR_CASE(HPGMG_HIP_7PT_CC)
    default: return record_error(hipErrorInvalidValue, "smooth_cheby_pair: variant");
  }
#undef PAIR_CASE
#undef PAIR_LAUNCH
#undef PAIR_LAUNCH2
#undef PAIR_NW_SWITCH
#undef PAIR_LAUNCH_REMOTE
#undef PAIR_LAUNCH_REMOTE_IP
  if (part != 1) { g_pair_launches++; if (remote) g_pair_remote_launches++; }
  profile_end(prof, 2 * cells, part == 1);
  HPGMG_LAUNCH_CHECK("cheby_pair_kernel");
  return 0;
}
int hpgmg_hip_smooth_cheby_pair(const hpgmg_hip_level *L, int variant, double *const *scr_base, const float *const *c32_base,
                                int x0_scr, int x0_id, int xm1_scr, int xm1_id, int out1_scr, int out1_id, int out2_scr, int out2_id,
                                int rhs_id, double a, double b, double h2inv, double c1a, double c2a, double c1b, double c2b) {
  return smooth_pair(L, variant, 0, 0, scr_base, c32_base, x0_scr, x0_id, xm1_scr, xm1_id, out1_scr, out1_id, out2_scr, out2_id, rhs_id, a, b, h2inv, c1a, c2a, c1b, c2b);
}
void hpgmg_hip_pair_fold_interpolation(const hpgmg_hip_level *Lc, int coarse_id, double prescale) {
  g_pair_interp_level = Lc; g_pair_interp_id = coarse_id; g_pair_interp_prescale = prescale;
}
void hpgmg_hip_pair_set_halo(const int brick_boxes[3], const int remote_face[6], const double *deep, const double *deep_beta) {
  for (int d = 0; d < 3; d++) g_pair_brick[d] = brick_boxes[d];
  for (int d = 0; d < 6; d++) g_pair_rem[d] = remote_face[d];
  g_pair_deep = deep; g_pair_deep_beta = deep_beta; g_pair_halo_set = true;
}
void hpgmg_hip_pair_discard_x1(void) { g_pair_discard_x1 = 1; }
#ifdef HPGMG_EXP_TIMELINE
void hpgmg_hip_exp_timeline(void *buf) { g_exp_timeline = (double *)buf; }
#endif
void hpgmg_hip_pair_launch_counts(long long out[2]) { out[0] = g_pair_launches; out[1] = g_pair_remote_launches; }

static const hpgmg_hip_level *g_halo_fold_level = nullptr;
static int g_halo_fold_id = 0;
static double g_halo_fold_prescale = 1.0;
static int pair_halo_move(bool unpack, const hpgmg_hip_level *L, double *const *scr_base, int x0_scr, int x0_id, int xm1_scr, int xm1_id, int rhs_id,
                          const hpgmg_hip_halo_entry *entries, int n, double *buf, double *deep, double *deep_beta) {
  const hpgmg_hip_level *fold = unpack ? nullptr : g_halo_fold_level;
  if (!unpack) g_halo_fold_level = nullptr;
  HPGMG_SKIP_IF_REPLAY();
  if (n <= 0) return 0;
  HaloRefs R = {}; R.x0 = VecRef{x0_scr, x0_id}; R.xm1 = VecRef{xm1_scr, xm1_id}; R.rhs_id = rhs_id; R.scr_base = scr_base;
  if (fold) { R.fold = 1; R.Lc = *fold; R.coarse_id = g_halo_fold_id; R.prescale = g_halo_fold_prescale; }
  const int slabs = (L->dim * L->dim + 4095) / 4096;
  if (unpack) hipLaunchKernelGGL((pair_halo_kernel<true>), dim3(n, slabs), dim3(256), 0, g_stream, *L, R, entries, buf, deep, deep_beta);
  else        hipLaunchKernelGGL((pair_halo_kernel<false>), dim3(n, slabs), dim3(256), 0, g_stream, *L, R, entries, buf, deep, deep_beta);
  HPGMG_LAUNCH_CHECK("pair_halo_kernel");
  return 0;
}
void hpgmg_hip_pair_halo_fold_interpolation(const hpgmg_hip_level *Lc, int coarse_id, double prescale) { g_halo_fold_level = Lc; g_halo_fold_id = coarse_id; g_halo_fold_prescale = prescale; }
int hpgmg_hip_pair_halo_pack(const hpgmg_hip_level *L, double *const *scr_base, int x0_scr, int x0_id, int xm1_scr, int xm1_id, int rhs_id,
                             const hpgmg_hip_halo_entry *entries, int n, double *sendbuf) {
  return pair_halo_move(false, L, scr_base, x0_scr, x0_id, xm1_scr, xm1_id, rhs_id, entries, n, sendbuf, nullptr, nullptr);
}
int hpgmg_hip_pair_halo_unpack(const hpgmg_hip_level *L, double *const *scr_base, int x0_scr, int x0_id, int xm1_scr, int xm1_id, int rhs_id,
                               const hpgmg_hip_halo_entry *entries, int n, double *recvbuf, double *deep, double *deep_beta) {
  return pair_halo_move(true, L, scr_base, x0_scr, x0_id, xm1_scr, xm1_id, rhs_id, entries, n, recvbuf, deep, deep_beta);
}

int hpgmg_hip_smooth_gsrb_pair(const hpgmg_hip_level *L, int variant, double *const *scr_base, const float *const *c32_base,
                               int x0_scr, int x0_id, int edge_scr_id, int out2_scr, int out2_id, int rhs_id,
                               double a, double b, double h2inv, int sweep) {
  return smooth_pair(L, variant, 1, sweep, scr_base, c32_base, x0_scr, x0_id, x0_scr, x0_id, 1, edge_scr_id, out2_scr, out2_id, rhs_id, a, b, h2inv, 0.0, 0.0, 0.0, 0.0);
}

}
```

### include/hpgmg_fv.h

```cpp
#ifndef HPGMG_FV_H
#define HPGMG_FV_H

#include "hpgmg_level.h"
#include "hpgmg_operators.h"
#include "hpgmg_mg.h"

#ifdef __cplusplus
extern "C" {
#endif

typedef struct hpgmg_solver {
  level_type level_h;
  mg_type    mg;
  double a, b, h;
  int boxes_in_i, box_dim;
  int my_rank, num_ranks;
} hpgmg_solver;

int hpgmg_choose_boxes_in_i(int log2_box_dim, int target_boxes_per_rank, int num_ranks);

hpgmg_solver *hpgmg_solver_create(int log2_box_dim, int target_boxes_per_rank, int bc, int my_rank, int num_ranks);
hpgmg_solver *hpgmg_solver_create_explicit(int boxes_in_i, int box_dim, int bc, int my_rank, int num_ranks);
void hpgmg_solver_destroy(hpgmg_solver *s);

// ... 29 lines not shown
int  hpgmg_user_solve(hpgmg_user_solver *s, int method, double rtol, const double *u0, int where, hpgmg_user_info *info);
int  hpgmg_user_set_max_iterations(hpgmg_user_solver *s, int n);
int  hpgmg_user_get_solution(hpgmg_user_solver *s, double *u, int where);
int  hpgmg_user_apply(hpgmg_user_solver *s, const double *x, double *y, int where);
int  hpgmg_user_set_rhs_dirichlet(hpgmg_user_solver *s, const double *f, const double *g, int where, double *mean_shift);
int  hpgmg_user_apply_dirichlet(hpgmg_user_solver *s, const double *x, const double *g, double *y, int where);
enum { HPGMG_FACE_DIRICHLET = 0, HPGMG_FACE_NEUMANN = 1, HPGMG_FACE_ROBIN = 3 };
int  hpgmg_user_create_faces(int n, int box_dim, const int face_bc[6], int op, int smoother, double a, double b, double h, hpgmg_user_solver **out);
int  hpgmg_user_set_coefficients_robin(hpgmg_user_solver *s, const double *alpha, const double *beta_i, const double *beta_j, const double *beta_k,
                                       const double *kappa, int where);
int  hpgmg_user_flux(hpgmg_user_solver *s, const double *u, const double *g, double *flux_i, double *flux_j, double *flux_k, int where);

enum { HPGMG_INFO_DIM = 0, HPGMG_INFO_BOX_DIM, HPGMG_INFO_GHOSTS, HPGMG_INFO_JSTRIDE, HPGMG_INFO_KSTRIDE,
       HPGMG_INFO_VOLUME, HPGMG_INFO_NUM_MY_BOXES, HPGMG_INFO_NUM_VECTORS, HPGMG_INFO_BOXES_IN_I,
       HPGMG_INFO_MY_RANK, HPGMG_INFO_NUM_RANKS, HPGMG_INFO_NUM_MY_BLOCKS, HPGMG_INFO_ACTIVE, HPGMG_INFO_COUNT };
void   hpgmg_level_info(const level_type *level, int out[HPGMG_INFO_COUNT]);
double hpgmg_level_h(const level_type *level);
double hpgmg_level_eigenvalue(const level_type *level);
int    hpgmg_level_must_subtract_mean(const level_type *level);
void   hpgmg_level_set_eigenvalue(level_type *level, double dominant_eigenvalue_of_DinvA);
void   hpgmg_level_box_low(const level_type *level, int box, int out[3]);
int    hpgmg_level_list_counts(const level_type *level, int which, int shape_or_type, int out[3]);
void   hpgmg_level_read_vector(level_type *level, int box, int id, double *host_out);
void   hpgmg_level_write_vector(level_type *level, int box, int id, const double *host_in);
level_type *hpgmg_level_create(int boxes_in_i, int box_dim, int ghosts, int numVectors, int bc, int my_rank, int num_ranks, double h);
void        hpgmg_level_destroy(level_type *level);
mg_type    *hpgmg_mg_create(level_type *fine, double a, double b, int minCoarseDim);
void        hpgmg_mg_destroy(mg_type *mg);
level_type *hpgmg_mg_level(mg_type *mg, int l);
int         hpgmg_mg_num_levels(const mg_type *mg);
void        hpgmg_set_verbose(int v);
int         hpgmg_transport_init_rccl(const char *id128, int rank, int size);
void        hpgmg_transport_finalize_rccl(void);
int         hpgmg_transport_init_ipc(const char *name, int rank, int size);
void        hpgmg_transport_finalize_ipc(void);
int         hpgmg_transport_selftest(char *msg, int msglen);
void        hpgmg_set_sync_timers(int on);
void        hpgmg_print_switches(void);
void        hpgmg_set_small_fused(int mode);
void        hpgmg_set_small_vtail(int on);
void        hpgmg_set_small_ops(int on);
long long   hpgmg_small_ops_groups(void);
long long   hpgmg_small_ops_prefetched(void);
void        hpgmg_set_fused_bottom(int on);
void        hpgmg_set_fused_tail(int on);
void        hpgmg_set_brick_visits(int on);
long long   hpgmg_brick_visits(void);
long long   hpgmg_brick_failures(void);
long long   hpgmg_brick_capacity_refusals(void);
void        hpgmg_set_brick_wide(int on);
void        hpgmg_set_brick_chains(int on);
long long   hpgmg_pair_remote_smooths(void);
long long   hpgmg_fp32_pair_smooths(void);
long long   hpgmg_fused_residuals_remote(void);
long long   hpgmg_fv4_rb_smooths(void);
long long   hpgmg_rb27_passes(void);
long long   hpgmg_image_exchanges(void);
void        hpgmg_level_timers(level_type *level, double out[9]);
void        hpgmg_set_gather_dim(int dim);
long long   hpgmg_overlap_count(void);
void        hpgmg_set_overlap(int on);
void        hpgmg_set_smoother_precision(int bits);
int         hpgmg_get_smoother_precision(void);
void        hpgmg_set_graphs(int on);
void        hpgmg_set_fused_sweeps(int on);
void        hpgmg_set_pair_min_cells(long long cells);
void        hpgmg_set_ghost_free(int on);
void        hpgmg_set_box_alignment(int jstride, int kstride, int volume, int base_bytes);

#ifdef __cplusplus
}
#endif
#endif
```

### include/hpgmg_hip.h

```cpp
#ifndef HPGMG_HIP_H
#define HPGMG_HIP_H

#include <stddef.h>
#include "hpgmg_level.h"

#ifdef __cplusplus
extern "C" {
#endif

typedef struct {
  double *const *box_base;
  const int *box_low;
  int num_boxes;
  int dim, ghosts, jStride, kStride, volume;
  int dim_i, dim_j, dim_k;
  int periodic;
  const int *box_nbr;
  int flags;
  long long box_stride;
} hpgmg_hip_level;

enum { HPGMG_HIP_7PT_VC_HELMHOLTZ = 0, HPGMG_HIP_7PT_VC_POISSON = 1, HPGMG_HIP_7PT_CC = 2,
       HPGMG_HIP_27PT_CC = 3, HPGMG_HIP_FV4_VC_HELMHOLTZ = 4, HPGMG_HIP_FV4_VC_POISSON = 5 };

// ... 43 lines not shown
                            double a, double b, double h2inv, double weight);
int hpgmg_hip_residual(const hpgmg_hip_level *L, int variant, int res_id, int x_id, int rhs_id,
                       double a, double b, double h2inv);
int hpgmg_hip_residual_fused_supported(const hpgmg_hip_level *L, int variant);
int  hpgmg_hip_residual_restrict_supported(const hpgmg_hip_level *L, int variant);
int hpgmg_hip_residual_restrict(const hpgmg_hip_level *L, int variant, int x_id, int rhs_id, double a, double b, double h2inv,
                                const hpgmg_hip_level *Lc, int coarse_id, const int *map, int zero_id);
int hpgmg_hip_residual_restrict_store(const hpgmg_hip_level *L, int variant, int res_id, int x_id, int rhs_id, double a, double b, double h2inv,
                                      const hpgmg_hip_level *Lc, int coarse_id, const int *map, int zero_id);
int hpgmg_hip_residual_norm(const hpgmg_hip_level *L, int variant, int res_id, int x_id, int rhs_id, double a, double b, double h2inv, double *norm_out);
int hpgmg_hip_small_level_max_cells(void);
int hpgmg_hip_small_level_op(const hpgmg_hip_level *L, int variant, int mode, int sweeps, int x_id, int rhs_id, int res_id, int out_of_place,
                             double a, double b, double h2inv, const double *c1, const double *c2,
                             const blockCopy_type *copy_list, int n_copy, const blockCopy_type *bc_list, int n_bc, int bc_kind, int zero_first);
int hpgmg_hip_bottom_bicgstab_max_cells(void);
int hpgmg_hip_bottom_bicgstab(const hpgmg_hip_level *L, int variant, int x_id, int rhs_id, int krylov_base, double a, double b, double h2inv, double want,
                              const blockCopy_type *bc_list, int n_bc, int bc_kind, int zero_first, int *krylov_iterations);
int hpgmg_hip_small_ops_max(void);
int hpgmg_hip_small_ops(const hpgmg_hip_level *L, int variant, int n, const int *kinds, const int *c, const int *a, const int *b, const double *sa, const double *sb,
                        const blockCopy_type *bc_list, int n_bc, int bc_kind, int zero_first, double op_a, double op_b, double h2inv, double *value_out, double *value2_out);
long long hpgmg_hip_small_ops_launch_count(void);
#define HPGMG_HIP_SMALL_TAIL_MAX_LEVELS 4
typedef struct {
  hpgmg_hip_level L;
  const blockCopy_type *bc_list, *ibc_list;
  int n_bc, bc_kind, zero_first, n_ibc, ibc_kind, ibc_zero_first;
  double h2inv, c1[8], c2[8];
} hpgmg_hip_small_tail_level;
typedef struct {
  int n, mode, sweeps, out_of_place, e_id, R_id, krylov_base, legs;
  double a, b, want;
  int *krylov_iterations;
  hpgmg_hip_small_tail_level lv[HPGMG_HIP_SMALL_TAIL_MAX_LEVELS];
} hpgmg_hip_small_tail_args;
long long hpgmg_hip_small_vtail_lds_doubles(const hpgmg_hip_small_tail_args *args);
long long hpgmg_hip_small_vtail_lds_limit(void);
int hpgmg_hip_small_vtail(const hpgmg_hip_small_tail_args *args, int variant);
long long hpgmg_hip_small_vtail_launch_count(void);
void hpgmg_hip_set_defer_mode(int mode);
void hpgmg_hip_set_tile_part(int part);
void hpgmg_hip_set_tile_ghost_free(int on);
void hpgmg_hip_set_27pt_tile32(int on);
int  hpgmg_hip_smooth_gsrb27_rb_supported(const hpgmg_hip_level *L);
int  hpgmg_hip_smooth_gsrb27_rb(const hpgmg_hip_level *L, int x_id, int out_id, int rhs_id, double a, double b, double h2inv, int sweep);
int  hpgmg_hip_smooth_gsrb27_rb_box_supported(const hpgmg_hip_level *L);
void hpgmg_hip_set_27pt_rb_box_maxdim(int dim);
int  hpgmg_hip_smooth_gsrb27_rb_box(const hpgmg_hip_level *L, int x_id, int out_id, int rhs_id, double a, double b, double h2inv, int sweep);
long long hpgmg_hip_rb27_launch_count(void);
int  hpgmg_hip_tile_kernel_applies(const hpgmg_hip_level *L, int variant, int out_of_place);

int hpgmg_hip_smooth_cheby_pair_supported(const hpgmg_hip_level *L, int variant);
int hpgmg_hip_smooth_cheby_pair(const hpgmg_hip_level *L, int variant, double *const *scr_base, const float *const *c32_base,
                                int x0_scr, int x0_id, int xm1_scr, int xm1_id, int out1_scr, int out1_id, int out2_scr, int out2_id,
                                int rhs_id, double a, double b, double h2inv, double c1a, double c2a, double c1b, double c2b);
int  hpgmg_hip_smooth_cheby_pair_supported_brick(const hpgmg_hip_level *L, int variant, int nbi, int nbj, int nbk);
void hpgmg_hip_pair_set_halo(const int brick_boxes[3], const int remote_face[6], const double *deep, const double *deep_beta);
void hpgmg_hip_pair_discard_x1(void);
void hpgmg_hip_pair_packed_invalidate(const hpgmg_hip_level *L);
void hpgmg_hip_pair_packed_forget(const hpgmg_hip_level *L);
void hpgmg_hip_pair_launch_counts(long long out[2]);
typedef struct { int box, vec, i, j, k, ni, nj, nk, deep, pad_; long long off; } hpgmg_hip_halo_entry;
void hpgmg_hip_pair_halo_fold_interpolation(const hpgmg_hip_level *Lc, int coarse_id, double prescale);
int  hpgmg_hip_pair_halo_pack(const hpgmg_hip_level *L, double *const *scr_base, int x0_scr, int x0_id, int xm1_scr, int xm1_id, int rhs_id,
                              const hpgmg_hip_halo_entry *entries, int n, double *sendbuf);
int  hpgmg_hip_pair_halo_unpack(const hpgmg_hip_level *L, double *const *scr_base, int x0_scr, int x0_id, int xm1_scr, int xm1_id, int rhs_id,
                                const hpgmg_hip_halo_entry *entries, int n, double *recvbuf, double *deep, double *deep_beta);
int hpgmg_hip_smooth_gsrb_pair(const hpgmg_hip_level *L, int variant, double *const *scr_base, const float *const *c32_base,
                               int x0_scr, int x0_id, int edge_scr_id, int out2_scr, int out2_id, int rhs_id,
                               double a, double b, double h2inv, int sweep);
void hpgmg_hip_pair_fold_interpolation(const hpgmg_hip_level *Lc, int coarse_id, double prescale);
int hpgmg_hip_coef32_refresh(const hpgmg_hip_level *L, float *const *c32_base, int num_vectors );

int hpgmg_hip_copy_blocks(const hpgmg_hip_level *L, int id, const blockCopy_type *blocks, int num_blocks);
int hpgmg_hip_increment_blocks(const hpgmg_hip_level *L, int id, double prescale, const blockCopy_type *blocks, int num_blocks);
int hpgmg_hip_apply_bc_p1(const hpgmg_hip_level *L, int id, const blockCopy_type *blocks, int num_blocks);
int hpgmg_hip_apply_bc_p2(const hpgmg_hip_level *L, int id, const blockCopy_type *blocks, int num_blocks);
int hpgmg_hip_apply_bc_v2(const hpgmg_hip_level *L, int id, const blockCopy_type *blocks, int num_blocks);
int hpgmg_hip_apply_bc_v4(const hpgmg_hip_level *L, int id, const blockCopy_type *blocks, int num_blocks);
int hpgmg_hip_extrapolate_betas(const hpgmg_hip_level *L, const blockCopy_type *blocks, int num_blocks);
typedef struct { int box, nn, base, len0, len1, fs0, fs1, step[3], src_box, src_base;
                 int zbase, zi, zj, zk;
} hpgmg_hip_bc_entry;
int hpgmg_hip_apply_bc_fv(const hpgmg_hip_level *L, int id, const hpgmg_hip_bc_entry *entries, int num_entries, int order);
int hpgmg_hip_exchange_and_bc(const hpgmg_hip_level *L, int id, const blockCopy_type *copies, int num_copies,
                              const hpgmg_hip_bc_entry *entries, int num_entries, int order);

int  hpgmg_hip_smooth_gsrb_fv4_rb_supported(const hpgmg_hip_level *L, int variant);
int  hpgmg_hip_fv4_rb_prepass(const hpgmg_hip_level *L, int variant, double *const *scr_base, int x_scratch, int x_id, int tg_id, int rhs_id,
                              double a, double b, double h2inv, int sweep, const hpgmg_hip_bc_entry *entries_k, int n_k,
                              const int *special_cells , int n_special);
int  hpgmg_hip_smooth_gsrb_fv4_rb(const hpgmg_hip_level *L, int variant, double *const *scr_base, int x_scratch, int x_id, int out_scratch, int out_id,
                                  int tg_id, int rhs_id, double a, double b, double h2inv, int sweep);
long long hpgmg_hip_rb_fv4_launch_count(void);
int hpgmg_hip_restrict_blocks(const hpgmg_hip_level *Lc, int id_c, const hpgmg_hip_level *Lf, int id_f,
                              const blockCopy_type *blocks, int num_blocks, int type);
int hpgmg_hip_restrict_cell_and_zero(const hpgmg_hip_level *Lc, int id_c, const hpgmg_hip_level *Lf, int id_f,
                                     const blockCopy_type *blocks, int num_blocks, int zero_id);
int hpgmg_hip_interpolate_blocks(const hpgmg_hip_level *Lf, int id_f, double prescale, const hpgmg_hip_level *Lc, int id_c,
                                 const blockCopy_type *blocks, int num_blocks, int order);

int hpgmg_hip_fill(const hpgmg_hip_level *L, int id, double interior_value);
int hpgmg_hip_axpby(const hpgmg_hip_level *L, int id_c, double sa, int id_a, double sb, int id_b);
int hpgmg_hip_mul(const hpgmg_hip_level *L, int id_c, double s, int id_a, int id_b);
int hpgmg_hip_invert(const hpgmg_hip_level *L, int id_c, double s, int id_a);
int hpgmg_hip_scale(const hpgmg_hip_level *L, int id_c, double s, int id_a);
int hpgmg_hip_shift(const hpgmg_hip_level *L, int id_c, int id_a, double shift);
int hpgmg_hip_color(const hpgmg_hip_level *L, int id, int colors, int ic, int jc, int kc);
int hpgmg_hip_random(const hpgmg_hip_level *L, int id);
int hpgmg_hip_norm_max(const hpgmg_hip_level *L, int id, double *out);
int hpgmg_hip_dot(const hpgmg_hip_level *L, int id_a, int id_b, double *out);
int hpgmg_hip_norm_copy_restrict(const hpgmg_hip_level *L, int f_id, int r_id, const hpgmg_hip_level *Lc, int rc_id, const int *map, double *norm_out);
int  hpgmg_hip_norm_copy_restrict_deferred(const hpgmg_hip_level *L, int f_id, int r_id, const hpgmg_hip_level *Lc, int rc_id, const int *restrict_map);
int  hpgmg_hip_deferred_fetch(double *out);
int hpgmg_hip_sum(const hpgmg_hip_level *L, int id, double *out);
int hpgmg_hip_gram(const hpgmg_hip_level *L, const int *id_A, int rows, const int *id_B, int cols, double *C_host);
int hpgmg_hip_pcg_supported(const hpgmg_hip_level *L, int variant);
int hpgmg_hip_pcg_apply_dot(const hpgmg_hip_level *L, int variant, int Ap_id, int p_id, double a, double b, double h2inv, double *dot);
int hpgmg_hip_pcg_update(const hpgmg_hip_level *L, int x_id, int r_id, int p_id, int Ap_id, double alpha, double *rmax);
int hpgmg_hip_pcg_dot(const hpgmg_hip_level *L, int a_id, int b_id, double *dot);
int hpgmg_hip_pcg_dot2(const hpgmg_hip_level *L, int a_id, int c_id, int b_id, double *ab, double *cb);

int hpgmg_hip_dense_pack(const hpgmg_hip_level *L, int id, const double *src, int ni, int nj, int nk, int check, int *status);
// ... 85 lines not shown
```

Measured before the change: 6.524 billion.

## Form Dinv inside the Chebyshev pair smoother instead of loading it

Adds a kernel template variant that recomputes the diagonal inverse from the beta coefficients on the fly, rather than streaming the stored Dinv vector. It applies only when Dinv is recorded as rebuilt with the same a, b and h2inv. To keep that record valid, every path that writes coefficient vectors (BLAS1 ops, exchanges, BCs, restriction, interpolation, copies, uploads) now clears it. The aim is to cut one memory stream per cell in a bandwidth-bound smoother, at the cost of extra arithmetic, more kernel instantiations and host-side bookkeeping that must catch every write. It is gated by a switch and excluded for the constant-coefficient 7pt variant, for fp32 coefficients, for remote halos and for NW=16.

Measured after the change: 6.664 billion (median of 6 runs). 2.2% higher.

```diff
diff --git a/hpgmg_amd/csrc/host/operators_hip.c b/hpgmg_amd/csrc/host/operators_hip.c
--- a/hpgmg_amd/csrc/host/operators_hip.c
+++ b/hpgmg_amd/csrc/host/operators_hip.c
@@ -2,6 +2,7 @@
 
 void hp_do_restriction(level_type *Lc, int id_c, level_type *Lf, int id_f, int type) {
   TICK(Lf, restriction_total, "restriction");
+  hp_coef_written(Lc, id_c);
   communicator_type *S = &Lf->restriction[type], *R = &Lc->restriction[type];
   backend_t *Bc = hp_backend_of(Lc), *Bf = hp_backend_of(Lf);
   HIP_OK(hpgmg_hip_restrict_blocks(&Bc->dev, id_c, &Bf->dev, id_f, hp_mirror(Lf, S->blocks[0], S->num_blocks[0]), S->num_blocks[0], type));
@@ -180,6 +181,7 @@
 
 static void interpolation_lists(level_type *Lf, int id_f, double prescale, level_type *Lc, int id_c, int order, int tagbits) {
   TICK(Lf, interpolation_total, "interpolation");
+  hp_coef_written(Lf, id_f);
   communicator_type *S = &Lc->interpolation, *R = &Lf->interpolation;
   backend_t *Bc = hp_backend_of(Lc), *Bf = hp_backend_of(Lf);
   HIP_OK(hpgmg_hip_interpolate_blocks(&Bf->dev, id_f, 0.0, &Bc->dev, id_c, hp_mirror(Lc, S->blocks[0], S->num_blocks[0]), S->num_blocks[0], order));
@@ -245,15 +247,15 @@
   interpolation_lists(Lf, id_f, prescale, Lc, id_c, 1, 0x7);
 }
 
-void hp_do_zero_vector(level_type *L, int id) { BLAS1(hpgmg_hip_fill(&hp_backend_of(L)->dev, id, 0.0)); }
-void init_vector(level_type *L, int id, double s) { BLAS1(hpgmg_hip_fill(&hp_backend_of(L)->dev, id, s)); }
-void hp_do_add_vectors(level_type *L, int c, double sa, int a, double sb, int b) { BLAS1(hpgmg_hip_axpby(&hp_backend_of(L)->dev, c, sa, a, sb, b)); }
-void hp_do_mul_vectors(level_type *L, int c, double s, int a, int b) { BLAS1(hpgmg_hip_mul(&hp_backend_of(L)->dev, c, s, a, b)); }
-void invert_vector(level_type *L, int c, double s, int a) { BLAS1(hpgmg_hip_invert(&hp_backend_of(L)->dev, c, s, a)); }
-void hp_do_scale_vector(level_type *L, int c, double s, int a) { BLAS1(hpgmg_hip_scale(&hp_backend_of(L)->dev, c, s, a)); }
-void shift_vector(level_type *L, int c, int a, double shift) { BLAS1(hpgmg_hip_shift(&hp_backend_of(L)->dev, c, a, shift)); }
-void color_vector(level_type *L, int id, int colors, int ic, int jc, int kc) { BLAS1(hpgmg_hip_color(&hp_backend_of(L)->dev, id, colors, ic, jc, kc)); }
-void random_vector(level_type *L, int id) { BLAS1(hpgmg_hip_random(&hp_backend_of(L)->dev, id)); }
+void hp_do_zero_vector(level_type *L, int id) { hp_coef_written(L, id); BLAS1(hpgmg_hip_fill(&hp_backend_of(L)->dev, id, 0.0)); }
+void init_vector(level_type *L, int id, double s) { hp_coef_written(L, id); BLAS1(hpgmg_hip_fill(&hp_backend_of(L)->dev, id, s)); }
+void hp_do_add_vectors(level_type *L, int c, double sa, int a, double sb, int b) { hp_coef_written(L, c); BLAS1(hpgmg_hip_axpby(&hp_backend_of(L)->dev, c, sa, a, sb, b)); }
+void hp_do_mul_vectors(level_type *L, int c, double s, int a, int b) { hp_coef_written(L, c); BLAS1(hpgmg_hip_mul(&hp_backend_of(L)->dev, c, s, a, b)); }
+void invert_vector(level_type *L, int c, double s, int a) { hp_coef_written(L, c); BLAS1(hpgmg_hip_invert(&hp_backend_of(L)->dev, c, s, a)); }
+void hp_do_scale_vector(level_type *L, int c, double s, int a) { hp_coef_written(L, c); BLAS1(hpgmg_hip_scale(&hp_backend_of(L)->dev, c, s, a)); }
+void shift_vector(level_type *L, int c, int a, double shift) { hp_coef_written(L, c); BLAS1(hpgmg_hip_shift(&hp_backend_of(L)->dev, c, a, shift)); }
+void color_vector(level_type *L, int id, int colors, int ic, int jc, int kc) { hp_coef_written(L, id); BLAS1(hpgmg_hip_color(&hp_backend_of(L)->dev, id, colors, ic, jc, kc)); }
+void random_vector(level_type *L, int id) { hp_coef_written(L, id); BLAS1(hpgmg_hip_random(&hp_backend_of(L)->dev, id)); }
 
 static int attempt_open = 0, attempt_failed = 0;
 static long long brick_failures = 0;
diff --git a/hpgmg_amd/csrc/host/plugin_dense.c b/hpgmg_amd/csrc/host/plugin_dense.c
--- a/hpgmg_amd/csrc/host/plugin_dense.c
+++ b/hpgmg_amd/csrc/host/plugin_dense.c
@@ -31,6 +31,7 @@
   if (layout < HPGMG_DENSE_CELL || layout > HPGMG_DENSE_FACE_K) return -1;
   dense_extents(L, layout, n);
   if (!(src = dense_source(L, id, src, where, n[0] * n[1] * n[2]))) return -1;
+  hp_coef_written(L, id);
   HIP_OK(hpgmg_hip_dense_pack(&hp_backend_of(L)->dev, id, src, (int)n[0], (int)n[1], (int)n[2], check, &status));
   return status;
 }
@@ -78,6 +79,7 @@
   if (mask < 0 || mask > 63 || L->boundary_condition.type != BC_DIRICHLET || L->dim.i != L->dim.j || L->dim.i != L->dim.k) return -1;
   dense_extents(L, layout, n);
   if (!(src = dense_source(L, id, src, where, n[0] * n[1] * n[2]))) return -1;
+  hp_coef_written(L, id);
   HIP_OK(hpgmg_hip_dense_pack_walls(&hp_backend_of(L)->dev, id, src, layout - HPGMG_DENSE_FACE_I, check, mask, wall, &status));
   return status;
 }
@@ -86,6 +88,7 @@
   int status = 0;
   if (!g || L->boundary_condition.type != BC_DIRICHLET || mask < 0 || mask > 63 || (mask && !wall)) return -1;
   if (!(f = dense_source(L, id, f, where, (size_t)L->dim.i * L->dim.j * L->dim.k))) return -1;
+  hp_coef_written(L, id);
   HIP_OK(hpgmg_hip_dense_pack_lifted_robin(&hp_backend_of(L)->dev, id, f, g, bnd_weight(b, L->h), mask, wall, bnd_weight_neumann(b, L->h),
                                            mask ? kappa : NULL, L->h, &status));
   return status;
@@ -115,6 +118,7 @@
 }
 
 void hpgmg_boundary_lift(level_type *L, int id, const double *phi, const double *phi_fine, double sign) {
+  hp_coef_written(L, id);
   HIP_OK(hpgmg_hip_boundary_lift(&hp_backend_of(L)->dev, id, phi, phi_fine, sign));
 }
 
@@ -146,5 +150,6 @@
 }
 void hpgmg_boundary_store_walls(level_type *L, const double *wall, const double *kappa, int mask) {
   if (!mask || !wall) return;
+  hp_dinv_record_clear(L);
   HIP_OK(hpgmg_hip_boundary_store_walls(&hp_backend_of(L)->dev, wall, kappa, L->h, mask));
 }
diff --git a/hpgmg_amd/csrc/host/plugin_ghosts.c b/hpgmg_amd/csrc/host/plugin_ghosts.c
--- a/hpgmg_amd/csrc/host/plugin_ghosts.c
+++ b/hpgmg_amd/csrc/host/plugin_ghosts.c
@@ -11,6 +11,7 @@
 
 void exchange_boundary(level_type *L, int id, int shape) {
   TICK(L, ghostZone_total, "exchange_boundary");
+  hp_coef_written(L, id);
   if (shape >= STENCIL_MAX_SHAPES) shape = STENCIL_SHAPE_BOX;
   communicator_type *C = &L->exchange_ghosts[shape];
   backend_t *B = hp_backend_of(L);
@@ -123,6 +124,7 @@
   if (shape >= STENCIL_MAX_SHAPES) shape = STENCIL_SHAPE_BOX;
   if (L->boundary_condition.type == BC_PERIODIC) return;
   TICK(L, boundary_conditions, "apply_BCs_p1");
+  hp_coef_written(L, x_id);
   backend_t *B = hp_backend_of(L);
   const int n = L->boundary_condition.num_blocks[shape];
   HIP_OK(hpgmg_hip_apply_bc_p1(&B->dev, x_id, hp_mirror(L, L->boundary_condition.blocks[shape], n), n));
@@ -247,6 +249,7 @@
 void extrapolate_betas(level_type *L) {
   if (L->boundary_condition.type == BC_PERIODIC) return;
   TICK(L, boundary_conditions, "extrapolate_betas");
+  hp_dinv_record_clear(L);
   const int n = L->boundary_condition.num_blocks[STENCIL_SHAPE_BOX];
   HIP_OK(hpgmg_hip_extrapolate_betas(&hp_backend_of(L)->dev, hp_mirror(L, L->boundary_condition.blocks[STENCIL_SHAPE_BOX], n), n));
   TOCK();
diff --git a/hpgmg_amd/csrc/host/plugin_internal.h b/hpgmg_amd/csrc/host/plugin_internal.h
--- a/hpgmg_amd/csrc/host/plugin_internal.h
+++ b/hpgmg_amd/csrc/host/plugin_internal.h
@@ -37,6 +37,7 @@
   double *dense_stage; size_t dense_stage_len;
   double *pair_scratch; double **d_pair_base;
   float *coef32; float **d_coef32_base; int coef32_valid;
+  int dinv_rebuilt; double dinv_a, dinv_b, dinv_h2inv;
   int lexicographic;
   int *d_restrict_map;
   struct pair_halo *halo;
@@ -92,7 +93,7 @@
 
 typedef enum { SW_GHOST_FREE = 0, SW_ONE_LAUNCH_GHOSTS, SW_OVERLAP, SW_PAIR_REMOTE, SW_IMAGES, SW_FUSED_SWEEPS, SW_PAIR_MIN_CELLS, SW_FUSED_RESIDUAL, SW_FUSED_TAIL,
                SW_FUSED_FTAIL, SW_FUSED_BOTTOM, SW_SMALL_FUSED, SW_SMALL_VTAIL, SW_SMALL_27PT_GSRB, SW_SMALL_OPS, SW_LAZY, SW_LAZY_REPORT, SW_TEMP_SCRATCH,
-               SW_FV4_NO_EXACT_RB, SW_GRAPH, SW_SMOOTHER_PRECISION, SW_DEFER_NORM, SW_BRICK_VISITS, SW_BRICK_SIZE, SW_BRICK_MIN_DIM, SW_BRICK_FSTEP, SW_BRICK_CHAIN, SW_BRICK_WIDE, SW_BRICK_WIDE_MAX_DIM, SW_BRICK_WIDE_TAIL_DIM, SW_FTAIL_MAX_DIM, SW_COUNT } hp_switch_id;
+               SW_FV4_NO_EXACT_RB, SW_GRAPH, SW_SMOOTHER_PRECISION, SW_DEFER_NORM, SW_BRICK_VISITS, SW_BRICK_SIZE, SW_BRICK_MIN_DIM, SW_BRICK_FSTEP, SW_BRICK_CHAIN, SW_BRICK_WIDE, SW_BRICK_WIDE_MAX_DIM, SW_BRICK_WIDE_TAIL_DIM, SW_FTAIL_MAX_DIM, SW_PAIR_FORM_DINV, SW_COUNT } hp_switch_id;
 HP_INTERNAL long long hp_switch(hp_switch_id id);
 HP_INTERNAL void hp_switch_set(hp_switch_id id, long long value);
 
@@ -132,6 +133,11 @@
 HP_INTERNAL const hpgmg_hip_bc_entry *hp_bc_entries_k(level_type *L, int *n_out, int *all_local_out);
 HP_INTERNAL int hp_vcycle_legs_fused(level_type **levels, int n, int e_id, int R_id, double a, double b, int leg);
 HP_INTERNAL void hp_coef32_invalidate(level_type *L);
+HP_INTERNAL void hp_dinv_record_set(level_type *L, double a, double b, double h2inv);
+HP_INTERNAL void hp_dinv_record_clear(level_type *L);
+HP_INTERNAL void hp_dinv_record_forget(level_type *L);
+HP_INTERNAL void hp_dinv_record_written(const double *dst, size_t n);
+static inline void hp_coef_written(level_type *L, int id) { if (id >= VECTOR_DINV && id <= VECTOR_ALPHA) hp_dinv_record_clear(L); }
 HP_INTERNAL int hp_interp_smooth_fused(level_type *Lf, int e_id, int R_id, level_type *Lc, double a, double b, int exact_state);
 HP_INTERNAL void hp_do_smooth(level_type *L, int x_id, int rhs_id, double a, double b, int temp_dead);
 HP_INTERNAL void hp_do_residual(level_type *L, int res_id, int x_id, int rhs_id, double a, double b);
diff --git a/hpgmg_amd/csrc/host/plugin_problem.c b/hpgmg_amd/csrc/host/plugin_problem.c
--- a/hpgmg_amd/csrc/host/plugin_problem.c
+++ b/hpgmg_amd/csrc/host/plugin_problem.c
@@ -156,4 +156,5 @@
   L->dominant_eigenvalue_of_DinvA = lambda;
   exchange_boundary(L, VECTOR_DINV, STENCIL_SHAPE_BOX);
   if (cfg.helmholtz) exchange_boundary(L, VECTOR_L1INV, STENCIL_SHAPE_BOX);
+  hp_dinv_record_set(L, a, b, 1.0 / (L->h * L->h));
 }
diff --git a/hpgmg_amd/csrc/host/plugin_runtime.c b/hpgmg_amd/csrc/host/plugin_runtime.c
--- a/hpgmg_amd/csrc/host/plugin_runtime.c
+++ b/hpgmg_amd/csrc/host/plugin_runtime.c
@@ -45,8 +45,8 @@
   return p;
 }
 void hpgmg_vector_free(double *p) { hp_lazy_flush(); hpgmg_hip_graph_reset(); hpgmg_hip_free(p); }
-void hpgmg_vector_copy(double *d, const double *s, size_t n) { HIP_OK(hpgmg_hip_memcpy_d2d(d, s, n * sizeof(double))); }
-void hpgmg_vector_upload(double *d, const double *s, size_t n) { HIP_OK(hpgmg_hip_memcpy_h2d(d, s, n * sizeof(double))); }
+void hpgmg_vector_copy(double *d, const double *s, size_t n) { hp_dinv_record_written(d, n); HIP_OK(hpgmg_hip_memcpy_d2d(d, s, n * sizeof(double))); }
+void hpgmg_vector_upload(double *d, const double *s, size_t n) { hp_dinv_record_written(d, n); HIP_OK(hpgmg_hip_memcpy_h2d(d, s, n * sizeof(double))); }
 void hpgmg_vector_download(double *d, const double *s, size_t n) { HIP_OK(hpgmg_hip_memcpy_d2h(d, s, n * sizeof(double))); }
 
 int hpgmg_transport_init_rccl(const char *id128, int rank, int size) {
@@ -175,6 +175,7 @@
   hpgmg_level_ext *X = hpgmg_level_ext_get(L);
   backend_t *B = (backend_t *)X->backend;
   int s;
+  hp_dinv_record_forget(L);
   if (!B) return;
   hpgmg_hip_pair_packed_forget(&B->dev);
   hp_images_release(B);
diff --git a/hpgmg_amd/csrc/host/plugin_smooth.c b/hpgmg_amd/csrc/host/plugin_smooth.c
--- a/hpgmg_amd/csrc/host/plugin_smooth.c
+++ b/hpgmg_amd/csrc/host/plugin_smooth.c
@@ -295,7 +295,40 @@
   if (!B->coef32_valid) { HIP_OK(hpgmg_hip_coef32_refresh(&B->dev, (float *const *)B->d_coef32_base, L->numVectors)); B->coef32_valid = 1; }
   return (const float *const *)B->d_coef32_base;
 }
-void hp_coef32_invalidate(level_type *L) { backend_t *B = hp_backend_of(L); B->coef32_valid = 0; if (B->halo) B->halo->coef_valid = 0; hp_images_invalidate_coefficients(B); hpgmg_hip_pair_packed_invalidate(&B->dev); }
+void hp_coef32_invalidate(level_type *L) { backend_t *B = hp_backend_of(L); B->coef32_valid = 0; hp_dinv_record_clear(L); if (B->halo) B->halo->coef_valid = 0; hp_images_invalidate_coefficients(B); hpgmg_hip_pair_packed_invalidate(&B->dev); }
+
+enum { DINV_RECORDS = 64 };
+static level_type *dinv_recorded[DINV_RECORDS];
+void hp_dinv_record_forget(level_type *L) { int q; for (q = 0; q < DINV_RECORDS; q++) if (dinv_recorded[q] == L) dinv_recorded[q] = NULL; }
+void hp_dinv_record_clear(level_type *L) {
+  hpgmg_level_ext *X = hpgmg_level_ext_get(L);
+  if (X->backend) ((backend_t *)X->backend)->dinv_rebuilt = 0;
+  hp_dinv_record_forget(L);
+}
+void hp_dinv_record_set(level_type *L, double a, double b, double h2inv) {
+  backend_t *B = hp_backend_of(L);
+  int q, slot = -1;
+  for (q = 0; q < DINV_RECORDS; q++) { if (dinv_recorded[q] == L) { slot = q; break; } if (slot < 0 && !dinv_recorded[q]) slot = q; }
+  if (slot < 0) return;
+  dinv_recorded[slot] = L;
+  B->dinv_rebuilt = 1; B->dinv_a = a; B->dinv_b = b; B->dinv_h2inv = h2inv;
+}
+void hp_dinv_record_written(const double *dst, size_t n) {
+  int q, bx;
+  for (q = 0; q < DINV_RECORDS; q++) {
+    level_type *L = dinv_recorded[q];
+    if (!L) continue;
+    for (bx = 0; bx < L->num_my_boxes; bx++) {
+      const double *lo = L->my_boxes[bx].vectors[0] + (size_t)VECTOR_DINV * (size_t)L->box_volume, *hi = L->my_boxes[bx].vectors[0] + (size_t)(VECTOR_ALPHA + 1) * (size_t)L->box_volume;
+      if (dst < hi && dst + n > lo) { hp_dinv_record_clear(L); break; }
+    }
+  }
+}
+void hpgmg_set_pair_form_dinv(int on) { hp_switch_set(SW_PAIR_FORM_DINV, on ? 1 : 0); }
+long long hpgmg_pair_formed_dinv_launches(void) { hp_lazy_flush(); return hpgmg_hip_pair_formed_dinv_launches(); }
+static int dinv_formable(const backend_t *B, double a, double b, double h2inv) {
+  return hp_switch(SW_PAIR_FORM_DINV) && B->dinv_rebuilt && memcmp(&a, &B->dinv_a, sizeof a) == 0 && memcmp(&b, &B->dinv_b, sizeof b) == 0 && memcmp(&h2inv, &B->dinv_h2inv, sizeof h2inv) == 0;
+}
 
 static long long pair_remote_smooths = 0, fp32_pair_smooths = 0;
 long long hpgmg_pair_remote_smooths(void) { return pair_remote_smooths; }
@@ -337,7 +370,7 @@
 long long hpgmg_interp_folded_remote(void) { return interp_folded_remote; }
 static int first_pair_folded(const hpgmg_hip_level *fold_Lc, backend_t *B, int v, int x_id, int rhs_id, double a, double b, double h2inv, const double *c1, const double *c2) {
   hpgmg_hip_pair_fold_interpolation(fold_Lc, x_id, 1.0);
-  return hpgmg_hip_smooth_cheby_pair(&B->dev, v, (double *const *)B->d_pair_base, NULL, 0, x_id, 0, VECTOR_TEMP, 1, 0, 1, 1, rhs_id, a, b, h2inv, c1[0], c2[0], c1[1], c2[1]);
+  return hpgmg_hip_smooth_cheby_pair(&B->dev, v, (double *const *)B->d_pair_base, NULL, 0, x_id, 0, VECTOR_TEMP, 1, 0, 1, 1, rhs_id, a, b, h2inv, c1[0], c2[0], c1[1], c2[1], dinv_formable(B, a, b, h2inv));
 }
 static int smooth_cheby_pairs_fold(level_type *L, int x_id, int rhs_id, double a, double b, const double *c1, const double *c2, int sweeps, int temp_dead, const hpgmg_hip_level *fold_Lc) {
   if (!pair_kernel_ready(L, x_id, rhs_id, sweeps)) return 0;
@@ -355,15 +388,15 @@
   }
   { TICK(L, smooth, "smooth (Chebyshev sweeps 1+2)");
     if (remote && fold_Lc) PAIR_REMOTE_LAUNCH(over, 0, first_pair_folded(fold_Lc, B, v, x_id, rhs_id, a, b, h2inv, c1, c2));
-    else if (remote) PAIR_REMOTE_LAUNCH(over, 0, hpgmg_hip_smooth_cheby_pair(&B->dev, v, (double *const *)B->d_pair_base, c32, 0, x_id, 0, VECTOR_TEMP, 1, 0, 1, 1, rhs_id, a, b, h2inv, c1[0], c2[0], c1[1], c2[1]));
-    else HIP_OK(hpgmg_hip_smooth_cheby_pair(&B->dev, v, (double *const *)B->d_pair_base, c32, 0, x_id, 0, VECTOR_TEMP, 1, 0, 1, 1, rhs_id, a, b, h2inv, c1[0], c2[0], c1[1], c2[1]));
+    else if (remote) PAIR_REMOTE_LAUNCH(over, 0, hpgmg_hip_smooth_cheby_pair(&B->dev, v, (double *const *)B->d_pair_base, c32, 0, x_id, 0, VECTOR_TEMP, 1, 0, 1, 1, rhs_id, a, b, h2inv, c1[0], c2[0], c1[1], c2[1], dinv_formable(B, a, b, h2inv)));
+    else HIP_OK(hpgmg_hip_smooth_cheby_pair(&B->dev, v, (double *const *)B->d_pair_base, c32, 0, x_id, 0, VECTOR_TEMP, 1, 0, 1, 1, rhs_id, a, b, h2inv, c1[0], c2[0], c1[1], c2[1], dinv_formable(B, a, b, h2inv)));
     TOCK(); }
   if (remote) over = hp_pair_halo_begin(L, B, 0, 1, 1, 1, 0, rhs_id);
   { TICK(L, smooth, "smooth (Chebyshev sweeps 3+4)");
-    if (remote) PAIR_REMOTE_LAUNCH(over, temp_dead, hpgmg_hip_smooth_cheby_pair(&B->dev, v, (double *const *)B->d_pair_base, c32, 1, 1, 1, 0, 0, VECTOR_TEMP, 0, x_id, rhs_id, a, b, h2inv, c1[2], c2[2], c1[3], c2[3]));
+    if (remote) PAIR_REMOTE_LAUNCH(over, temp_dead, hpgmg_hip_smooth_cheby_pair(&B->dev, v, (double *const *)B->d_pair_base, c32, 1, 1, 1, 0, 0, VECTOR_TEMP, 0, x_id, rhs_id, a, b, h2inv, c1[2], c2[2], c1[3], c2[3], dinv_formable(B, a, b, h2inv)));
     else {
       if (temp_dead) hpgmg_hip_pair_discard_x1();
-      HIP_OK(hpgmg_hip_smooth_cheby_pair(&B->dev, v, (double *const *)B->d_pair_base, c32, 1, 1, 1, 0, 0, VECTOR_TEMP, 0, x_id, rhs_id, a, b, h2inv, c1[2], c2[2], c1[3], c2[3]));
+      HIP_OK(hpgmg_hip_smooth_cheby_pair(&B->dev, v, (double *const *)B->d_pair_base, c32, 1, 1, 1, 0, 0, VECTOR_TEMP, 0, x_id, rhs_id, a, b, h2inv, c1[2], c2[2], c1[3], c2[3], dinv_formable(B, a, b, h2inv)));
     }
     TOCK(); }
   return 1;
@@ -380,13 +413,13 @@
   int over = 0;
   if (remote) { pair_remote_smooths++; over = hp_pair_halo_begin(L, B, 1, 0, x_id, 0, x_id, rhs_id); }
   { TICK(L, smooth, "smooth (GSRB half sweeps 1+2)");
-    if (remote) PAIR_REMOTE_LAUNCH(over, 0, hpgmg_hip_smooth_gsrb_pair(&B->dev, v, (double *const *)B->d_pair_base, NULL, 0, x_id, 0, 1, 1, rhs_id, a, b, h2inv, 0));
-    else HIP_OK(hpgmg_hip_smooth_gsrb_pair(&B->dev, v, (double *const *)B->d_pair_base, NULL, 0, x_id, 0, 1, 1, rhs_id, a, b, h2inv, 0));
+    if (remote) PAIR_REMOTE_LAUNCH(over, 0, hpgmg_hip_smooth_gsrb_pair(&B->dev, v, (double *const *)B->d_pair_base, NULL, 0, x_id, 0, 1, 1, rhs_id, a, b, h2inv, 0, dinv_formable(B, a, b, h2inv)));
+    else HIP_OK(hpgmg_hip_smooth_gsrb_pair(&B->dev, v, (double *const *)B->d_pair_base, NULL, 0, x_id, 0, 1, 1, rhs_id, a, b, h2inv, 0, dinv_formable(B, a, b, h2inv)));
     TOCK(); }
   if (remote) over = hp_pair_halo_begin(L, B, 0, 1, 1, 1, 1, rhs_id);
   { TICK(L, smooth, "smooth (GSRB half sweeps 3+4)");
-    if (remote) PAIR_REMOTE_LAUNCH(over, 0, hpgmg_hip_smooth_gsrb_pair(&B->dev, v, (double *const *)B->d_pair_base, NULL, 1, 1, 0, 0, x_id, rhs_id, a, b, h2inv, 2));
-    else HIP_OK(hpgmg_hip_smooth_gsrb_pair(&B->dev, v, (double *const *)B->d_pair_base, NULL, 1, 1, 0, 0, x_id, rhs_id, a, b, h2inv, 2));
+    if (remote) PAIR_REMOTE_LAUNCH(over, 0, hpgmg_hip_smooth_gsrb_pair(&B->dev, v, (double *const *)B->d_pair_base, NULL, 1, 1, 0, 0, x_id, rhs_id, a, b, h2inv, 2, dinv_formable(B, a, b, h2inv)));
+    else HIP_OK(hpgmg_hip_smooth_gsrb_pair(&B->dev, v, (double *const *)B->d_pair_base, NULL, 1, 1, 0, 0, x_id, rhs_id, a, b, h2inv, 2, dinv_formable(B, a, b, h2inv)));
     TOCK(); }
   return 1;
 }
diff --git a/hpgmg_amd/csrc/host/plugin_switches.c b/hpgmg_amd/csrc/host/plugin_switches.c
--- a/hpgmg_amd/csrc/host/plugin_switches.c
+++ b/hpgmg_amd/csrc/host/plugin_switches.c
@@ -32,6 +32,7 @@
   [SW_BRICK_WIDE_MAX_DIM] = { "HPGMG_TUNE_BRICK_WIDE_MAX", K_INT, 64, "largest level (cells per side) the 27-pt / fv4 plugins visit as bricks (measured: fv4 `7 64` 29.71 / 29.91 / 30.15 ms with 64 / 32 / 16, 27-pt 12.27 / 12.51 / 12.52)" },
   [SW_BRICK_WIDE_TAIL_DIM] = { "HPGMG_TUNE_BRICK_WIDE_TAIL", K_INT, 1, "27-pt / fv4: the largest one-box level left to the single-workgroup tail (1: the 8^3, 4^3 (and 27-pt: 2^3) levels are visited as ONE brick each and only the bottom solve is left; 2 / 4 / 8: the tail starts there)" },
   [SW_FTAIL_MAX_DIM]    = { "HPGMG_TUNE_FTAIL_MAX", K_INT, 8, "7-pt: the largest level (cells per side) the single-launch F-cycle tail starts from (8: the 16^3 step of the climb is a brick launch each way, eight CUs instead of one: config 1 0.320 vs 0.328 ms with 16, config 2 the same within noise; profiles/r06i_ab_ftail.txt)" },
+  [SW_PAIR_FORM_DINV]    = { "HPGMG_PAIR_FORM_DINV", K_ON, 1, "7-pt sweep pairs (fp64 streams, one rank, variable coefficients, 10 / 12 waves): Dinv is formed in registers from the coefficient streams instead of read, where VECTOR_DINV is known to be rebuild_operator's output for the same a, b; 0: always read" },
   [SW_SMOOTHER_PRECISION]= { "HPGMG_SMOOTHER_PRECISION", K_INT, 64, "32: fp32 coefficient streams in the Chebyshev sweep pairs (BASELINE config 5: within 2e-4 of the fp64 norms, and bit-exact against the CPU oracle's fp32 mode, which rounds the same coefficients); 64: bit-exact" },
 };
 
diff --git a/hpgmg_amd/csrc/kernels/cheby_pair.hpp b/hpgmg_amd/csrc/kernels/cheby_pair.hpp
--- a/hpgmg_amd/csrc/kernels/cheby_pair.hpp
+++ b/hpgmg_amd/csrc/kernels/cheby_pair.hpp
@@ -10,6 +10,7 @@
   int rhs_id;
   double a, b, h2inv, c1a, c2a, c1b, c2b;
   int sweep_a;
+  int form_dinv;
   int keep_x1;
   hpgmg_hip_level Lc; int coarse_id; double prescale;
   double *const *scr_base;
@@ -77,13 +78,27 @@
   return o;
 }
 
+template <int V>
+__device__ __forceinline__ p2 pair_form_dinv(const PlaneCoef<V> &q, double fil, double fih, double fjl, double fjh, double fkl, double fkh, double a, double nbh2) {
+  double d0 = q.bi.x * fil;     double d1 = q.bi.y * (1.0 - 2.0);
+  d0 = d0 + q.bjlo.x * fjl;     d1 = d1 + q.bjlo.y * fjl;
+  d0 = d0 + q.bk0.x * fkl;      d1 = d1 + q.bk0.y * fkl;
+  d0 = d0 + q.bi.y * (1.0 - 2.0); d1 = d1 + q.bir * fih;
+  d0 = d0 + q.bjhi.x * fjh;     d1 = d1 + q.bjhi.y * fjh;
+  d0 = d0 + q.bk1.x * fkh;      d1 = d1 + q.bk1.y * fkh;
+  double A0 = nbh2 * d0, A1 = nbh2 * d1;
+  if (V == HPGMG_HIP_7PT_VC_HELMHOLTZ) { A0 = A0 + a * q.al.x; A1 = A1 + a * q.al.y; }
+  return p2{1.0 / A0, 1.0 / A1};
+}
+
 constexpr int kPairMaxBoxes = 1024;
-template <int V, int NW, bool C32, int SM, bool NARROW, bool INTERP, bool REMOTE = false>
+template <int V, int NW, bool C32, int SM, bool NARROW, bool INTERP, bool REMOTE = false, bool FORM = false>
 __global__ __launch_bounds__(64 * NW) void cheby_pair_kernel(const hpgmg_hip_level L_in, const PairArgs A_in) {
   static_assert(!(REMOTE && C32) && !(REMOTE && NARROW && INTERP), "the multi-rank variant is built for fp64 coefficients; with narrow boxes the interpolation is not folded in");
   constexpr bool kVC = (V != HPGMG_HIP_7PT_CC);
   constexpr bool kHelm = (V == HPGMG_HIP_7PT_VC_HELMHOLTZ);
   constexpr int NR = NW - 2;
+  static_assert(!FORM || (kVC && !C32 && !REMOTE && NW != 16), "no FORM instance of this kind");
   extern __shared__ p2 pair_lds[];
   p2 (*slabX0)[NW][64] = reinterpret_cast<p2 (*)[NW][64]>(pair_lds);
   p2 (*slabX1)[NW][64] = reinterpret_cast<p2 (*)[NW][64]>(pair_lds + 2 * NW * 64);
@@ -221,16 +236,19 @@
     const bool above_in = x0plane(p + 1);
     const bool ghost_plane = REMOTE && (p < 0 || p >= A.Dk);
     if (row_x1) {
-      if (above_in) {
-        const int bn = box_of(bi_, bj_, p + 1), offn = row_off + plane_off(p + 1);
-        x0p = REMOTE ? x0_row(bj_, lj, p + 1) : x0_pair(bn, li, lj, p + 1);
-        if (have_next) {
-          if (kVC) bj_n = CoefStream<C32>(L, A, bn, VECTOR_BETA_J, C32_BETA_J, sh).pair(offn);
-          if (far_lo || far_hi) far_n = far_row(p + 1);
+      auto load_ahead = [&]() {
+        if (above_in) {
+          const int bn = box_of(bi_, bj_, p + 1), offn = row_off + plane_off(p + 1);
+          x0p = REMOTE ? x0_row(bj_, lj, p + 1) : x0_pair(bn, li, lj, p + 1);
+          if (have_next) {
+            if (kVC) bj_n = CoefStream<C32>(L, A, bn, VECTOR_BETA_J, C32_BETA_J, sh).pair(offn);
+            if (far_lo || far_hi) far_n = far_row(p + 1);
+          }
         }
-      }
-      qc.rhs = pld(vec_origin(L, box, A.rhs_id) + sh.lvl + off);
-      qc.dinv = CoefStream<C32>(L, A, box, VECTOR_DINV, C32_DINV, sh).pair(off);
+        qc.rhs = pld(vec_origin(L, box, A.rhs_id) + sh.lvl + off);
+      };
+      if (!FORM) load_ahead();
+      if (!FORM) qc.dinv = CoefStream<C32>(L, A, box, VECTOR_DINV, C32_DINV, sh).pair(off);
       if (kHelm) qc.al = CoefStream<C32>(L, A, box, VECTOR_ALPHA, C32_ALPHA, sh).pair(off);
       if (kVC) {
         const CoefStream<C32> bis(L, A, box, VECTOR_BETA_I, C32_BETA_I, sh), bks(L, A, box, VECTOR_BETA_K, C32_BETA_K, sh);
@@ -245,8 +263,12 @@
         else if (w == NRs + 1 || gj + 1 >= jhi || ((lj + 1) == bd)) qc.bjhi = CoefStream<C32>(L, A, box, VECTOR_BETA_J, C32_BETA_J, sh).pair(off + jS);
         else qc.bjhi = slabBJ[p & 1][w + 1][lane];
       }
+      if (FORM) load_ahead();
       p2 xm1 = x0c;
       if (SM == PAIR_CHEBY && A.c1a != 0.0) xm1 = pld(pair_vec(L, A, A.xm1, box) + shift_of(sh, A.xm1) + off);
+      if (FORM)
+        qc.dinv = pair_form_dinv<V>(qc, (lane == 0 && left_dom) ? -2.0 : -1.0, (lane == 63 && right_dom) ? -2.0 : -1.0, (gj - 1 < 0) ? -2.0 : -1.0, (gj + 1 >= A.Dj) ? -2.0 : -1.0,
+                                    (p - 1 < 0) ? -2.0 : -1.0, (p + 1 >= A.Dk) ? -2.0 : -1.0, A.a, (-A.b) * A.h2inv);
 #ifdef HPGMG_EXP_TIMELINE
       if (probe) { asm volatile("s_waitcnt vmcnt(0)" ::: "memory"); }
       TL_MARK();
diff --git a/hpgmg_amd/csrc/kernels/pair.hip b/hpgmg_amd/csrc/kernels/pair.hip
--- a/hpgmg_amd/csrc/kernels/pair.hip
+++ b/hpgmg_amd/csrc/kernels/pair.hip
@@ -40,6 +40,19 @@
 }
 using namespace hpgmg;
 
+template <int V, int NW, bool C32, int SM, bool NARROW, bool INTERP, bool FORM>
+static int pair_launch_instance(int grid, size_t lds, const hpgmg_hip_level *L, const PairArgs &A) {
+  static bool once = false;
+  if (!once) { HPGMG_CHECK(hipFuncSetAttribute((const void *)cheby_pair_kernel<V, NW, C32, SM, NARROW, INTERP, false, FORM>, hipFuncAttributeMaxDynamicSharedMemorySize, (int)((size_t)NW * 6 * 64 * sizeof(p2)))); once = true; }
+  hipLaunchKernelGGL((cheby_pair_kernel<V, NW, C32, SM, NARROW, INTERP, false, FORM>), dim3(grid), dim3(64, NW), lds, g_stream, *L, A);
+  return 0;
+}
+template <int V, int NW, bool C32, int SM, bool NARROW, bool INTERP>
+static int pair_launch(int grid, size_t lds, const hpgmg_hip_level *L, const PairArgs &A) {
+  if constexpr (V != HPGMG_HIP_7PT_CC && !C32 && NW != 16) { if (A.form_dinv) return pair_launch_instance<V, NW, C32, SM, NARROW, INTERP, true>(grid, lds, L, A); }
+  return pair_launch_instance<V, NW, C32, SM, NARROW, INTERP, false>(grid, lds, L, A);
+}
+
 extern "C" {
 int hpgmg_hip_graph_flush(void);
 
@@ -66,7 +79,7 @@
 static bool g_pair_halo_set = false;
 static int g_pair_rem[6], g_pair_brick[3];
 static const double *g_pair_deep = nullptr, *g_pair_deep_beta = nullptr;
-static long long g_pair_launches = 0, g_pair_remote_launches = 0;
+static long long g_pair_launches = 0, g_pair_remote_launches = 0, g_pair_formed_launches = 0;
 static int g_pair_discard_x1 = 0;
 static const hpgmg_hip_level *g_pair_interp_level = nullptr;
 static int g_pair_interp_id = 0;
@@ -117,7 +130,7 @@
 }
 static int smooth_pair(const hpgmg_hip_level *L, int variant, int gsrb, int sweep_a, double *const *scr_base, const float *const *c32_base,
                        int x0_scr, int x0_id, int xm1_scr, int xm1_id, int out1_scr, int out1_id, int out2_scr, int out2_id,
-                       int rhs_id, double a, double b, double h2inv, double c1a, double c2a, double c1b, double c2b) {
+                       int rhs_id, double a, double b, double h2inv, double c1a, double c2a, double c1b, double c2b, int dinv_is_rebuilt) {
   const bool remote = g_pair_halo_set;
   const int discard_x1 = g_pair_discard_x1;
   const hpgmg_hip_level *const interp_level = g_pair_interp_level;
@@ -153,6 +166,7 @@
   A.rhs_id = rhs_id; A.a = a; A.b = b; A.h2inv = h2inv; A.c1a = c1a; A.c2a = c2a; A.c1b = c1b; A.c2b = c2b;
   A.scr_base = scr_base; A.c32_base = c32_base; A.sweep_a = sweep_a;
   A.keep_x1 = discard_x1 ? 0 : 1;
+  A.form_dinv = (dinv_is_rebuilt && !remote && !c32_base && variant != HPGMG_HIP_7PT_CC && nw != 16) ? 1 : 0;
   const bool interp = (interp_level != nullptr);
   if (interp) {
     const hpgmg_hip_level *C = interp_level;
@@ -196,8 +210,7 @@
   const int prof = profile_begin(whole_cells);
 #define PAIR_NW_SWITCH(...) switch (nw) { case 10: { constexpr int NWC = 10; __VA_ARGS__ } break; case 12: { constexpr int NWC = 12; __VA_ARGS__ } break; default: { constexpr int NWC = 16; __VA_ARGS__ } break; }
 #define PAIR_LAUNCH2(VAR, C32, SM, NARROW, INTERP) PAIR_NW_SWITCH( \
-      static bool once = false; if (!once) { HPGMG_CHECK(hipFuncSetAttribute((const void *)cheby_pair_kernel<VAR, NWC, C32, SM, NARROW, INTERP>, hipFuncAttributeMaxDynamicSharedMemorySize, (int)((size_t)NWC * 6 * 64 * sizeof(p2)))); once = true; } \
-      hipLaunchKernelGGL((cheby_pair_kernel<VAR, NWC, C32, SM, NARROW, INTERP>), dim3(grid), dim3(64, NWC), lds, g_stream, *L, A); )
+      { const int e_ = pair_launch<VAR, NWC, C32, SM, NARROW, INTERP>(grid, lds, L, A); if (e_) return e_; } )
 #define PAIR_LAUNCH_REMOTE_IP(VAR, SM, NRW, IP) { \
       const int ecols = 2 * (A.tiles_i - 1) + (A.rem[0] ? 1 : 0) + (A.rem[1] ? 1 : 0); \
       A.edge_blocks = ((A.Dj + 63) / 64) * A.Dk * ecols; const int egrid_r = grid_for(A.edge_blocks, &A.edge_per_xcd); \
@@ -231,15 +244,15 @@
 #undef PAIR_NW_SWITCH
 #undef PAIR_LAUNCH_REMOTE
 #undef PAIR_LAUNCH_REMOTE_IP
-  if (part != 1) { g_pair_launches++; if (remote) g_pair_remote_launches++; }
+  if (part != 1) { g_pair_launches++; if (remote) g_pair_remote_launches++; if (A.form_dinv) g_pair_formed_launches++; }
   profile_end(prof, 2 * cells, part == 1);
   HPGMG_LAUNCH_CHECK("cheby_pair_kernel");
   return 0;
 }
 int hpgmg_hip_smooth_cheby_pair(const hpgmg_hip_level *L, int variant, double *const *scr_base, const float *const *c32_base,
                                 int x0_scr, int x0_id, int xm1_scr, int xm1_id, int out1_scr, int out1_id, int out2_scr, int out2_id,
-                                int rhs_id, double a, double b, double h2inv, double c1a, double c2a, double c1b, double c2b) {
-  return smooth_pair(L, variant, 0, 0, scr_base, c32_base, x0_scr, x0_id, xm1_scr, xm1_id, out1_scr, out1_id, out2_scr, out2_id, rhs_id, a, b, h2inv, c1a, c2a, c1b, c2b);
+                                int rhs_id, double a, double b, double h2inv, double c1a, double c2a, double c1b, double c2b, int dinv_is_rebuilt) {
+  return smooth_pair(L, variant, 0, 0, scr_base, c32_base, x0_scr, x0_id, xm1_scr, xm1_id, out1_scr, out1_id, out2_scr, out2_id, rhs_id, a, b, h2inv, c1a, c2a, c1b, c2b, dinv_is_rebuilt);
 }
 void hpgmg_hip_pair_fold_interpolation(const hpgmg_hip_level *Lc, int coarse_id, double prescale) {
   g_pair_interp_level = Lc; g_pair_interp_id = coarse_id; g_pair_interp_prescale = prescale;
@@ -254,6 +267,7 @@
 void hpgmg_hip_exp_timeline(void *buf) { g_exp_timeline = (double *)buf; }
 #endif
 void hpgmg_hip_pair_launch_counts(long long out[2]) { out[0] = g_pair_launches; out[1] = g_pair_remote_launches; }
+long long hpgmg_hip_pair_formed_dinv_launches(void) { return g_pair_formed_launches; }
 
 static const hpgmg_hip_level *g_halo_fold_level = nullptr;
 static int g_halo_fold_id = 0;
@@ -284,8 +298,8 @@
 
 int hpgmg_hip_smooth_gsrb_pair(const hpgmg_hip_level *L, int variant, double *const *scr_base, const float *const *c32_base,
                                int x0_scr, int x0_id, int edge_scr_id, int out2_scr, int out2_id, int rhs_id,
-                               double a, double b, double h2inv, int sweep) {
-  return smooth_pair(L, variant, 1, sweep, scr_base, c32_base, x0_scr, x0_id, x0_scr, x0_id, 1, edge_scr_id, out2_scr, out2_id, rhs_id, a, b, h2inv, 0.0, 0.0, 0.0, 0.0);
-}
-
-}
+                               double a, double b, double h2inv, int sweep, int dinv_is_rebuilt) {
+  return smooth_pair(L, variant, 1, sweep, scr_base, c32_base, x0_scr, x0_id, x0_scr, x0_id, 1, edge_scr_id, out2_scr, out2_id, rhs_id, a, b, h2inv, 0.0, 0.0, 0.0, 0.0, dinv_is_rebuilt);
+}
+
+}
diff --git a/include/hpgmg_fv.h b/include/hpgmg_fv.h
--- a/include/hpgmg_fv.h
+++ b/include/hpgmg_fv.h
@@ -105,6 +105,8 @@
 void        hpgmg_set_brick_chains(int on);
 long long   hpgmg_pair_remote_smooths(void);
 long long   hpgmg_fp32_pair_smooths(void);
+void        hpgmg_set_pair_form_dinv(int on);
+long long   hpgmg_pair_formed_dinv_launches(void);
 long long   hpgmg_fused_residuals_remote(void);
 long long   hpgmg_fv4_rb_smooths(void);
 long long   hpgmg_rb27_passes(void);
diff --git a/include/hpgmg_hip.h b/include/hpgmg_hip.h
--- a/include/hpgmg_hip.h
+++ b/include/hpgmg_hip.h
@@ -119,7 +119,8 @@
 int hpgmg_hip_smooth_cheby_pair_supported(const hpgmg_hip_level *L, int variant);
 int hpgmg_hip_smooth_cheby_pair(const hpgmg_hip_level *L, int variant, double *const *scr_base, const float *const *c32_base,
                                 int x0_scr, int x0_id, int xm1_scr, int xm1_id, int out1_scr, int out1_id, int out2_scr, int out2_id,
-                                int rhs_id, double a, double b, double h2inv, double c1a, double c2a, double c1b, double c2b);
+                                int rhs_id, double a, double b, double h2inv, double c1a, double c2a, double c1b, double c2b, int dinv_is_rebuilt);
+long long hpgmg_hip_pair_formed_dinv_launches(void);
 int  hpgmg_hip_smooth_cheby_pair_supported_brick(const hpgmg_hip_level *L, int variant, int nbi, int nbj, int nbk);
 void hpgmg_hip_pair_set_halo(const int brick_boxes[3], const int remote_face[6], const double *deep, const double *deep_beta);
 void hpgmg_hip_pair_discard_x1(void);
@@ -134,7 +135,7 @@
                                 const hpgmg_hip_halo_entry *entries, int n, double *recvbuf, double *deep, double *deep_beta);
 int hpgmg_hip_smooth_gsrb_pair(const hpgmg_hip_level *L, int variant, double *const *scr_base, const float *const *c32_base,
                                int x0_scr, int x0_id, int edge_scr_id, int out2_scr, int out2_id, int rhs_id,
-                               double a, double b, double h2inv, int sweep);
+                               double a, double b, double h2inv, int sweep, int dinv_is_rebuilt);
 void hpgmg_hip_pair_fold_interpolation(const hpgmg_hip_level *Lc, int coarse_id, double prescale);
 int hpgmg_hip_coef32_refresh(const hpgmg_hip_level *L, float *const *c32_base, int num_vectors );
 
```
